# ldyken53/gaussian-splatting-wgpu

Measured on AMD Instinct MI355X. Metric: frames/sec, higher is better.
Workload: dtype f32; 1 GPU; bicycle-like synthetic 6.1M gaussians @1920x1080; gaussians=6100000, width=1920, height=1080, tile_size=16, parallelism=single GPU, visible=2430918, processed=15909895, block_evaluated=6068168, sort_passes=1, depth_ordered_emission=True, tight_binning=True, blend_mode=fused, camera=64-step orbit, moved every frame

## Files before the change

### gaussian-splatting-wgpu_amd/csrc/gs_context.hip

```cpp
#include <atomic>
#include <cmath>
#include <cstdarg>
#include <memory>
#include <new>

#include "gs_runtime.h"

thread_local char g_err[512] = "";
int32_t fail(int32_t code, const char* fmt, ...) {
    va_list ap;
    va_start(ap, fmt);
    vsnprintf(g_err, sizeof(g_err), fmt, ap);
    va_end(ap);
    return code;
}

static uint32_t tiles_f32(uint32_t extent, uint32_t ts) {
    return (uint32_t)std::ceil((float)extent / (float)ts);
}
static uint32_t bits_for(uint64_t v) {
    uint32_t b = 0;
    while (v) { ++b; v >>= 1; }
    return b ? b : 1;
}

GS_EXPORT const char* gs_last_error(void) { return g_err; }
GS_EXPORT int32_t gs_abi_version(void) { return GS_ABI_VERSION; }

int32_t alloc_kv(gs_ctx* c, uint64_t capacity, uint64_t row_cap) {
    if (capacity >= (1ull << 30)) return fail(GS_ERR_CAPACITY, "capacity %llu exceeds 2^30 intersections", (unsigned long long)capacity);
    if (row_cap >= (1ull << 31)) return fail(GS_ERR_CAPACITY, "%llu row items exceed the 2^31 limit", (unsigned long long)row_cap);
    c->gr.valid = false;
    c->keysA.reset(); c->valsA.reset(); c->keysB.reset(); c->valsB.reset(); c->keysU.reset(); c->valsU.reset();
    c->keysG.reset(); c->chunk_table.reset(); c->arena.reset(); c->rows_sorted.reset(); c->M3.reset(); c->ctl_mem.reset();
    c->valsG.reset();
    c->keysG_valid = c->valsG_valid = c->gdataG_valid = false;
    capacity = std::max<uint64_t>(capacity, 4096);
    row_cap = (std::max<uint64_t>(row_cap, 4096) + 15) & ~(uint64_t)15;
    const size_t kb = (size_t)capacity * 4;
    HIP_TRY(hipMalloc(c->keysA.out(), kb));
    HIP_TRY(hipMalloc(c->valsA.out(), kb));
    HIP_TRY(hipMalloc(c->keysB.out(), kb));
    HIP_TRY(hipMalloc(c->valsB.out(), kb));
    c->sort_index = GsSort{{c->keysA, c->valsA}, {c->keysB, c->valsB}, c->passes, 8, 0, false, false};
    c->sort_tile = GsSort{{c->keysA, c->valsA}, {c->keysB, c->valsB}, c->tile_passes, c->tile_bits, c->tile16 ? 0u : 1u, c->tile16, true};
    HIP_TRY(hipMalloc(c->chunk_table.out(), (size_t)gs_emit_chunks(std::max(capacity, row_cap)) * 4));
    if (c->tight_ok) {
        HIP_TRY(hipMalloc(c->arena.out(), (size_t)row_cap * 12));
        HIP_TRY(hipMalloc(c->rows_sorted.out(), (size_t)row_cap * 12));
        HIP_TRY(hipMalloc(c->M3.out(), (size_t)gs_rows_chunks(row_cap) * 256 * 4));
    }
    const size_t ctl_sz = (sizeof(GsControl) + 255) & ~(size_t)255;
    const size_t scan_sz = (((size_t)gs_scan_blocks(c->n ? c->n : 1) + 1) * 8 + 255) & ~(size_t)255;
    const size_t sort_sz = (size_t)std::max(c->passes, c->tile_passes) * gs_sort_tiles(capacity) * 256 * 4;
    const size_t rows_sz = c->tight_ok ? (size_t)gs_rows_sort_tiles(row_cap) * 256 * 4 : 0;
    const size_t depth_sz = ((size_t)c->T * 4 + 255) & ~(size_t)255;
    c->ctl_bytes = ctl_sz + depth_sz + rows_sz + scan_sz + sort_sz;
    c->ctl_bytes_tight = ctl_sz + depth_sz + rows_sz;
    HIP_TRY(hipMalloc(c->ctl_mem.out(), c->ctl_bytes));
    char* const base = (char*)c->ctl_mem.get();
    c->ctl = (GsControl*)base;
    c->tile_depth = (uint32_t*)(base + ctl_sz);
    c->rows_status = (uint32_t*)(base + ctl_sz + depth_sz);
    c->scan_status = (unsigned long long*)(base + ctl_sz + depth_sz + rows_sz);
    c->sort_status = (uint32_t*)(base + ctl_sz + depth_sz + rows_sz + scan_sz);
    c->capacity = capacity;
    c->row_cap = row_cap;
    c->frame.capacity = (uint32_t)capacity;
    c->frame.row_cap = (uint32_t)row_cap;
    return GS_OK;
}

GS_EXPORT int32_t gs_create(const gs_config* cfg, gs_ctx** out) {
    if (!cfg || !out) return fail(GS_ERR_INVALID_ARGUMENT, "gs_create: null argument");
    if (cfg->struct_size != sizeof(gs_config)) return fail(GS_ERR_INVALID_ARGUMENT, "gs_create: struct_size %u != %zu", cfg->struct_size, sizeof(gs_config));
    if (cfg->width == 0 || cfg->height == 0) return fail(GS_ERR_INVALID_ARGUMENT, "gs_create: empty canvas");
    if (cfg->tile_size != 8 && cfg->tile_size != 16 && cfg->tile_size != 32)
        return fail(GS_ERR_INVALID_ARGUMENT, "gs_create: tile_size must be 8, 16 or 32 (got %u)", cfg->tile_size);
    int ndev = 0;
    if (hipGetDeviceCount(&ndev) != hipSuccess || ndev == 0) return fail(GS_ERR_NO_DEVICE, "gs_create: no HIP device");
    if (cfg->device < 0 || cfg->device >= ndev) return fail(GS_ERR_INVALID_ARGUMENT, "gs_create: device %d of %d", cfg->device, ndev);
    HIP_TRY(hipSetDevice(cfg->device));

    std::unique_ptr<gs_ctx> c(new (std::nothrow) gs_ctx());
    if (!c) return fail(GS_ERR_OUT_OF_MEMORY, "gs_create: host allocation failed");
    c->cfg = *cfg;
    GsFrame& f = c->frame;
    f.width = cfg->width; f.height = cfg->height; f.tile_size = cfg->tile_size;
    f.ntx = tiles_f32(cfg->width, cfg->tile_size);
    f.nty = tiles_f32(cfg->height, cfg->tile_size);
    if (f.ntx >= 32768 || f.nty >= 65536) return fail(GS_ERR_INVALID_ARGUMENT, "gs_create: canvas too large");
    f.col0 = cfg->col_begin;
    f.col1 = cfg->col_end;
    if (f.col0 == 0 && f.col1 == 0) f.col1 = f.ntx;
    if (f.col1 > f.ntx || f.col0 >= f.col1) return fail(GS_ERR_INVALID_ARGUMENT, "gs_create: bad tile-column slab [%u,%u) of %u", f.col0, f.col1, f.ntx);
    f.full = (f.col0 == 0 && f.col1 == f.ntx) ? 1u : 0u;
    f.px0 = f.col0 * f.tile_size;
    f.slab_w = std::min(f.width, f.col1 * f.tile_size) - f.px0;
    c->T = f.ntx * f.nty;
    const uint64_t max_key = ((uint64_t)f.nty * f.ntx + f.ntx) * 1000ull + 999ull;
    if (max_key > 0xFFFFFFFFull) return fail(GS_ERR_INVALID_ARGUMENT, "gs_create: tile ids overflow the 32-bit key (write_tile_ids.wgsl:29)");
    c->key_bits = bits_for(max_key);
    c->passes = (c->key_bits + 7) / 8;
    const uint32_t tbits = bits_for((uint64_t)f.nty * f.ntx + f.ntx);
    c->tile_passes = (tbits + 7) / 8;
    c->tile_bits = (tbits + c->tile_passes - 1) / c->tile_passes;
    c->tile16 = ((uint64_t)f.nty * f.ntx + f.ntx) < 0xFFFFull;
    if ((uint64_t)(f.ntx + 1) * (f.nty + 1) > GS_COUNT_MASK) return fail(GS_ERR_INVALID_ARGUMENT, "gs_create: canvas has too many tiles");
    c->tight_ok = f.ntx <= 255u && f.nty <= 255u;

    hipDeviceProp_t prop;
    HIP_TRY(hipGetDeviceProperties(&prop, cfg->device));
    c->opt.grid_persist = (uint32_t)prop.multiProcessorCount * 4;
    if (cfg->stream) c->stream = (hipStream_t)cfg->stream;
    else { HIP_TRY(hipStreamCreateWithFlags(c->own_stream.out(), hipStreamNonBlocking)); c->stream = c->own_stream; }

    HIP_TRY(hipMalloc(c->ranges.out(), (size_t)c->T * 4));
    HIP_TRY(hipMemset(c->ranges, 0, (size_t)c->T * 4));
    const size_t px = (size_t)f.slab_w * f.height;
    HIP_TRY(hipMalloc(c->rgba8.out(), px * 4));
    HIP_TRY(hipMemset(c->rgba8, 0, px * 4));
    if (cfg->flags & GS_FLAG_F32_TAP) HIP_TRY(hipMalloc(c->rgbf.out(), px * 12));
    if (cfg->flags & GS_FLAG_AUX_OUTPUTS) {
        HIP_TRY(hipMalloc(c->alpha.out(), px * 4));
        HIP_TRY(hipMalloc(c->depth.out(), px * 4));
        HIP_TRY(hipMemset(c->alpha, 0, px * 4));
        HIP_TRY(hipMemset(c->depth, 0, px * 4));
    }
    HIP_TRY(hipHostMalloc(c->h_ctl.out(), sizeof(GsControl), hipHostMallocDefault));
    memset(c->h_ctl, 0, sizeof(GsControl));
    HIP_TRY(hipMalloc(c->d_pxb.out(), 65 * 4));
    HIP_TRY(hipMalloc(c->tileoff.out(), 256 * 256 * 4));
    HIP_TRY(hipMalloc(c->rowtot.out(), 256 * 4));
    HIP_TRY(hipMalloc(c->sticky.out(), 4 * 4));
    HIP_TRY(hipMemset(c->sticky, 0, 4 * 4));
    HIP_TRY(hipHostMalloc(c->h_rep.out(), sizeof(GsReport), hipHostMallocDefault));
    memset(c->h_rep, 0, sizeof(GsReport));
    if (cfg->flags & GS_FLAG_TIMING) {
        for (auto& row : c->ev)
            for (auto& e : row) HIP_TRY(hipEventCreate(e.out()));
        c->have_events = true;
    }
    c->fif = (c->own_stream && f.full) ? 3u : 1u;
    *out = c.release();
    return GS_OK;
}

gs_ctx::~gs_ctx() { drop_graph(this); }

GS_EXPORT int32_t gs_destroy(gs_ctx* c) {
    if (!c) return GS_OK;
    hipSetDevice(c->cfg.device);
    drop_shadows(c);
    if (c->stream) hipStreamSynchronize(c->stream);
    delete c;
    return GS_OK;
}

static int32_t alloc_per_gaussian(gs_ctx* c, uint64_t n, uint64_t min_capacity = 0, uint64_t min_rows = 0) {
    c->gr.valid = false;
    c->scene_own.reset();
    c->scene_mem = nullptr;
    c->n = (uint32_t)n;
    c->frame.n = (uint32_t)n;
    c->have_frame = false;
    c->cov.reset();
    c->ng = gs_ctx::Neigh{};
    c->cl = gs_ctx::Cluster{};
    c->counts.reset(); c->offsets.reset(); c->grec.reset(); c->rowptr.reset(); c->gsort_scratch.reset(); c->gdata.reset(); c->gdataG.reset();
    c->unit_off.reset(); c->unit_n.reset();
    const size_t np = ((size_t)n + 63) & ~(size_t)63;
    const size_t ne = (size_t)gs_gsort_tiles((uint32_t)(n ? n : 1)) * 2048, nu = ne / 1024 + 2;
    HIP_TRY(hipMalloc(c->counts.out(), ne * 4));
    HIP_TRY(hipMalloc(c->offsets.out(), std::max<size_t>(np * 4, 256)));
    HIP_TRY(hipMalloc(c->grec.out(), std::max<size_t>(np * 16, 256)));
    HIP_TRY(hipMalloc(c->rowptr.out(), ne * 4));
    HIP_TRY(hipMalloc(c->unit_off.out(), ne * 2));
    HIP_TRY(hipMalloc(c->unit_n.out(), nu * 4));
    HIP_TRY(hipMemsetAsync(c->unit_n, 0, nu * 4, c->stream));
    HIP_TRY(hipMalloc(c->gsort_scratch.out(), gs_gsort_scratch_bytes((uint32_t)n)));
    HIP_TRY(hipMalloc(c->gdata.out(), ((size_t)n + GS_RECORD_SLACK) * 64));
    HIP_TRY(hipMemsetAsync(c->gdata, 0, ((size_t)n + GS_RECORD_SLACK) * 64, c->stream));
    uint64_t cap = c->cfg.max_intersections ? c->cfg.max_intersections : std::max<uint64_t>(4 * n, 1u << 22);
    cap = std::max<uint64_t>(cap, min_capacity);
    cap = std::min<uint64_t>(cap, (1ull << 30) - 1);
    const uint64_t rows = std::max<uint64_t>(std::max<uint64_t>(2 * n, 1u << 20), min_rows);
    return alloc_kv(c, cap, rows);
}

GsSceneLayout scene_layout(void* base, uint64_t n, bool state) {
    GsSceneLayout L;
    const size_t np = ((size_t)n + 63) & ~(size_t)63;
    const size_t sh_end = np * 4 * 4 + np * 32 + (size_t)n * 192, state_at = (sh_end + 255) & ~(size_t)255;
    L.np = np;
    L.state_at = state_at;
    L.bytes = state ? state_at + np : sh_end;
    char* p = (char*)base;
    GsScene& s = L.scene;
    s.px = (float*)p; p += np * 4; s.py = (float*)p; p += np * 4; s.pz = (float*)p; p += np * 4;
    s.smax = (float*)p; p += np * 4;
    s.geo = (float4*)p; p += np * 32;
    s.sh = (float4*)p;
    s.state = state ? (const uint8_t*)base + state_at : nullptr;
    return L;
}
static void scene_views(gs_ctx* c, uint64_t n) {
    const GsSceneLayout L = scene_layout(c->scene_own.get(), n, has_state(c));
    c->scene_mem = c->scene_own;
    c->scene_bytes = L.bytes;
    c->scene = L.scene;
}

uint64_t scene_new_serial() {
    static std::atomic<uint64_t> next{1};
    return next.fetch_add(1, std::memory_order_relaxed);
}
int32_t scene_alloc(gs_ctx* c, uint64_t n, uint64_t min_capacity, uint64_t min_rows) {
    c->scene_serial = scene_new_serial();
    int32_t rc = alloc_per_gaussian(c, n, min_capacity, min_rows);
    if (rc != GS_OK) return rc;
    const GsSceneLayout L = scene_layout(nullptr, n, has_state(c));
    HIP_TRY(hipMalloc(c->scene_own.out(), std::max<size_t>(L.bytes, 256)));
    scene_views(c, n);
    if (has_state(c))
        HIP_TRY(hipMemsetAsync((char*)c->scene_mem + L.state_at, 0, std::max<size_t>(L.np, 4), c->stream));
    return GS_OK;
}

int32_t scene_install(gs_ctx* c, DevBuf<>&& mem, uint64_t n, uint64_t min_capacity, uint64_t min_rows) {
    const int32_t rc = alloc_per_gaussian(c, n, min_capacity, min_rows);
    if (rc != GS_OK) {
        c->scene = GsScene{};
        c->n = c->frame.n = 0;
        return rc;
    }
    c->scene_own = std::move(mem);
    scene_views(c, n);
    return GS_OK;
}

static int32_t upload_common(gs_ctx* c, const void* d_aos, uint64_t n) {
    int32_t rc = scene_alloc(c, n);
    if (rc != GS_OK) return rc;
    if (n) gs_launch_repack(d_aos, (uint32_t)n, 0, c->scene, c->stream);
    HIP_TRY(hipGetLastError());
    HIP_TRY(hipStreamSynchronize(c->stream));
    return GS_OK;
}

void drop_shadows(gs_ctx* c) {
    for (gs_ctx* s : c->shadows) gs_destroy(s);
    c->shadows.clear();
    c->last = c;
    c->rr = 0;
    c->cap_hint = 0;
    c->row_hint = 0;
}
GS_EXPORT int32_t gs_share_splats(gs_ctx* c, gs_ctx* owner) {
    if (!c || !owner || c == owner) return fail(GS_ERR_INVALID_ARGUMENT, "gs_share_splats: needs two distinct contexts");
    if (c->cfg.device != owner->cfg.device) return fail(GS_ERR_INVALID_ARGUMENT, "gs_share_splats: contexts are on different devices");
    if (!c->is_shadow) drop_shadows(c);
    if (!owner->scene_mem) return fail(GS_ERR_NO_SCENE, "gs_share_splats: the owner holds no splats");
    if (has_state(c) && !has_state(owner))
        return fail(GS_ERR_INVALID_ARGUMENT, "gs_share_splats: this context has GS_FLAG_SPLAT_STATE, the owner keeps no state plane");
    HIP_TRY(hipSetDevice(c->cfg.device));
    if (c->pending) { int32_t rc = wait_one(c); if (rc != GS_OK) return rc; }
    int32_t rc = alloc_per_gaussian(c, owner->n, c->cfg.max_intersections ? 0 : owner->capacity, owner->row_cap);
    if (rc != GS_OK) return rc;
    c->scene_mem = owner->scene_mem;
    c->scene_bytes = owner->scene_bytes;
    c->scene = owner->scene;
    c->scene_serial = scene_new_serial();
    HIP_TRY(hipStreamSynchronize(c->stream));
    return GS_OK;
}

GS_EXPORT int32_t gs_upload_splats_device(gs_ctx* c, const void* d_aos, uint64_t n) {
    if (!c || (!d_aos && n)) return fail(GS_ERR_INVALID_ARGUMENT, "gs_upload_splats_device: null argument");
    if (n >= (1ull << 31)) return fail(GS_ERR_INVALID_ARGUMENT, "gs_upload_splats: too many gaussians");
    HIP_TRY(hipSetDevice(c->cfg.device));
    drop_shadows(c);
    return upload_common(c, d_aos, n);
}

GS_EXPORT int32_t gs_upload_splats(gs_ctx* c, const void* aos, uint64_t n) {
    if (!c || (!aos && n)) return fail(GS_ERR_INVALID_ARGUMENT, "gs_upload_splats: null argument");
    if (n >= (1ull << 31)) return fail(GS_ERR_INVALID_ARGUMENT, "gs_upload_splats: too many gaussians");
    HIP_TRY(hipSetDevice(c->cfg.device));
    drop_shadows(c);
    DevBuf<> d;
    const size_t bytes = (size_t)n * GS_SPLAT_RECORD_BYTES;
    HIP_TRY(hipMalloc(d.out(), std::max<size_t>(bytes, 256)));
    if (bytes) {
        hipError_t e = hipMemcpy(d, aos, bytes, hipMemcpyHostToDevice);
        if (e != hipSuccess) return fail(GS_ERR_HIP, "upload memcpy: %s", hipGetErrorString(e));
    }
    return upload_common(c, d, n);
}

GS_EXPORT int32_t gs_host_alloc(uint64_t bytes, void** out) {
    if (!out) return fail(GS_ERR_INVALID_ARGUMENT, "gs_host_alloc: null argument");
    *out = nullptr;
    HIP_TRY(hipHostMalloc(out, std::max<size_t>((size_t)bytes, 256), hipHostMallocDefault));
    return GS_OK;
}
GS_EXPORT void gs_host_free(void* p) { if (p) hipHostFree(p); }

GS_EXPORT int32_t gs_slab_width(gs_ctx* c, uint32_t* px_begin, uint32_t* px_width) {
    if (!c) return fail(GS_ERR_INVALID_ARGUMENT, "gs_slab_width: null ctx");
    if (px_begin) *px_begin = c->frame.px0;
    if (px_width) *px_width = c->frame.slab_w;
    return GS_OK;
}

static int32_t set_option_one(gs_ctx* c, int32_t key, int64_t value) {
    c->gr.valid = false;
    GsOptions& o = c->opt;
    switch (key) {
    case GS_OPT_FRAME_GRAPH: o.frame_graph = (value != 0); return GS_OK;
    case GS_OPT_BLEND_ABLATION: o.blend_ablation = (uint32_t)value & 0x3FFFFu; return GS_OK;
    case GS_OPT_PERSISTENT_GRID: if (value <= 0) break; o.grid_persist = (uint32_t)value; return GS_OK;
    case GS_OPT_RESET_TIMING: c->timed_from = c->frames; c->max_I_seen = 0; c->truncated_frames = 0; return GS_OK;
    case GS_OPT_EMIT_ORDER: if (value < 0 || value > 2) break; o.emit_order = (int)value; return GS_OK;
    case GS_OPT_UNFUSED: return GS_OK;
    case GS_OPT_DEBUG_VIEW: if (value < 0 || value > 4) break; o.debug_view = (uint32_t)value; return GS_OK;
    case GS_OPT_TILE_CULL: o.tile_cull = (value != 0); return GS_OK;
    case GS_OPT_PROJ_CHUNKS: if (value != 0 && value != 2 && value != 4 && value != 8) break; o.tight_nb = (uint32_t)value; return GS_OK;
    case GS_OPT_SELECT_TINT:
        if (!has_state(c)) return fail(GS_ERR_INVALID_ARGUMENT, "gs_set_option: GS_OPT_SELECT_TINT needs GS_FLAG_SPLAT_STATE");
        if (value < 0 || value > 0xFFFFFFFFll) break;
        o.select_tint = (uint32_t)value;
        return GS_OK;
    default: break;
    }
    return fail(GS_ERR_INVALID_ARGUMENT, "gs_set_option: bad key/value %d/%lld", key, (long long)value);
}
GS_EXPORT int32_t gs_set_option(gs_ctx* c, int32_t key, int64_t value) {
    if (!c) return fail(GS_ERR_INVALID_ARGUMENT, "gs_set_option: null ctx");
    if (key == GS_OPT_FRAMES_IN_FLIGHT) {
        if (value < 1 || value > 4) return fail(GS_ERR_INVALID_ARGUMENT, "gs_set_option: frames in flight must be 1..4");
        if (!c->own_stream || !c->frame.full) value = 1;
        int32_t rc = gs_wait(c);
        if (rc != GS_OK && rc != GS_ERR_TRUNCATED) return rc;
        while (c->shadows.size() + 1 > (size_t)value) {
            if (c->last == c->shadows.back()) { c->last = c; }
            gs_destroy(c->shadows.back());
            c->shadows.pop_back();
        }
        c->fif = (uint32_t)value;
        c->rr = 0;
        return GS_OK;
    }
    int32_t rc = set_option_one(c, key, value);
    for (gs_ctx* s : c->shadows) if (rc == GS_OK) rc = set_option_one(s, key, value);
    return rc;
}
```

### gaussian-splatting-wgpu_amd/csrc/gs_device.h

```cpp
#pragma once
#include <hip/hip_runtime.h>
#include <stdint.h>

#define GS_WAVE 64

struct GsFrame {
    uint32_t n;
    uint32_t width, height, tile_size;
    uint32_t ntx, nty;
    uint32_t col0, col1;
    uint32_t px0, slab_w;
    uint32_t capacity;
    uint32_t full;
    uint32_t row_cap;
};

#define GS_COUNT_BITS 22
#define GS_COUNT_MASK 0x3FFFFFu

struct GsControl {
    uint32_t scan_ticket[2];
    uint32_t sort_ticket[4];
    uint32_t rows_ticket;
    uint32_t num_slots;
    uint32_t num_items;
    uint32_t fault;
    uint32_t overflow;
    uint32_t num_intersections;
    uint32_t num_visible;
    uint32_t pad0;
    uint32_t row_cursor[16];
    uint32_t rec_cursor[16];
    unsigned long long num_processed[64];
    unsigned long long num_evaluated[64];
    uint32_t hist[4][256];
    uint32_t rowhist[8][256];
};
__device__ __forceinline__ uint32_t gs_rowhist(const GsControl* ctl, uint32_t r) {
    uint32_t s = 0;
#pragma unroll
    for (int k = 0; k < 8; ++k) s += ctl->rowhist[k][r];
    return s;
}

struct GsReport {
    uint32_t fault, overflow, num_intersections, num_visible, num_slots, num_items, pad0, pad1;
    uint32_t row_cursor[16];
    uint32_t sticky[4];
};
__device__ __forceinline__ void gs_frame_report(const GsControl* ctl, uint32_t I, uint32_t num_items, uint32_t capacity, uint32_t* sticky,
                                                GsReport* rep) {
    uint32_t need = 0;
    for (int k = 0; k < 16; ++k) need = ctl->row_cursor[k] > need ? ctl->row_cursor[k] : need;
    need = need > 0x07FFFFFFu ? 0x7FFFFFFFu : need * 16u;
    const uint32_t over = (I > capacity || ctl->overflow) ? 1u : 0u;
    uint32_t s0 = 0, s1 = 0, s2 = 0, s3 = 0;
    if (sticky) {
        s0 = atomicAdd(&sticky[0], over) + over;
        s1 = atomicOr(&sticky[1], ctl->fault ? 1u : 0u) | (ctl->fault ? 1u : 0u);
        s2 = atomicMax(&sticky[2], I); s2 = s2 > I ? s2 : I;
        s3 = atomicMax(&sticky[3], need); s3 = s3 > need ? s3 : need;
    }
    if (rep) {
        rep->fault = ctl->fault; rep->overflow = over; rep->num_intersections = I; rep->num_visible = ctl->num_visible;
        rep->num_slots = ctl->num_slots; rep->num_items = num_items;
        for (int k = 0; k < 16; ++k) rep->row_cursor[k] = ctl->row_cursor[k];
        rep->sticky[0] = s0; rep->sticky[1] = s1; rep->sticky[2] = s2; rep->sticky[3] = s3;
    }
}

struct GsTightOut {
    uint32_t* arena; uint32_t* rowptr; GsControl* ctl;
    unsigned short* unit_off; uint32_t* unit_n;
    uint32_t rec_shard_cap;
};
#define GS_RECORD_SLACK (16u * 512u * 8u)

struct GsScene {
    const float* px; const float* py; const float* pz;
    const float* smax;
    const float4* geo;
    const float4* sh;
    const uint8_t* state;
};

#define GS_ST_HIDDEN 1u
#define GS_ST_SELECTED 2u
struct GsTint { float t[3]; float k; };
__device__ __forceinline__ uint32_t gs_state_apply(uint32_t s, uint32_t op, uint32_t bits) {
    return op == 1u ? (s | bits) : op == 2u ? (s & ~bits) : op == 3u ? (s ^ bits) : bits;
}
struct GsStateQuad { uint32_t w, valid; };
__device__ __forceinline__ GsStateQuad gs_state_quad(const uint8_t* __restrict__ state, uint32_t n, uint32_t q) {
    const uint64_t first = (uint64_t)q * 4u;
    uint32_t w = 0u, valid = 0u;
    if (first + 4u <= n) {
        valid = 4u;
        if (state) w = reinterpret_cast<const uint32_t*>(state)[q];
    } else if (first < n) {
        valid = (uint32_t)(n - first);
        if (state)
            for (uint32_t k = 0; k < valid; ++k) w |= (uint32_t)state[first + k] << (8u * k);
    }
    return GsStateQuad{w, valid};
}

struct GsPlyTable {
    uint32_t stride, nsrc, all_float;
    uint16_t soff[11 + 48];
    uint8_t stype[11 + 48], slot[11 + 48];
};

struct GsUniforms {
    float view[16];
    float proj[16];
    float cam[3];
    float tan_fovx, tan_fovy, focal_x, focal_y, scale_modifier;
};

__device__ __forceinline__ float wg_max(float a, float b) { return (a < b) ? b : a; }
__device__ __forceinline__ float wg_min(float a, float b) { return (b < a) ? b : a; }
__device__ __forceinline__ int wg_maxi(int a, int b) { return (a < b) ? b : a; }
__device__ __forceinline__ int wg_mini(int a, int b) { return (b < a) ? b : a; }

__device__ __forceinline__ int f2i_sat(float x) {
    if (x != x) return 0;
    if (x >= 2147483648.0f) return 2147483647;
    if (x <= -2147483648.0f) return (-2147483647 - 1);
    return (int)x;
}
__device__ __forceinline__ uint32_t f2u_sat(float x) {
    if (x != x) return 0u;
    if (x >= 4294967296.0f) return 0xFFFFFFFFu;
    if (x <= 0.0f) return 0u;
    return (uint32_t)x;
}

__device__ __forceinline__ float gs_exp(float x) {
    if (x != x) return x;
    if (x > 88.72283935546875f) return __builtin_inff();
    if (x < -103.97208404541015625f) return 0.0f;
    const float nf = __builtin_rintf(x * 1.44269502162933349609375f);
    float r = __builtin_fmaf(-nf, 0.693145751953125f, x);
    r = __builtin_fmaf(-nf, 1.42860677465796470642e-06f, r);
    float p = 1.9875691500e-4f;
    p = __builtin_fmaf(p, r, 1.3981999507e-3f);
    p = __builtin_fmaf(p, r, 8.3334519073e-3f);
    p = __builtin_fmaf(p, r, 4.1665795894e-2f);
    p = __builtin_fmaf(p, r, 1.6666665459e-1f);
    p = __builtin_fmaf(p, r, 5.0000001201e-1f);
    const float z = r * r;
    float y = __builtin_fmaf(p, z, r);
    y = y + 1.0f;
    const int n = (int)nf;
    const int a = n >> 1;
    const int b = n - a;
    const float sa = __uint_as_float((uint32_t)(a + 127) << 23);
    const float sb = __uint_as_float((uint32_t)(b + 127) << 23);
    return (y * sa) * sb;
}

__device__ __forceinline__ float gs_blend_power(float cx, float cy, float cz, float dx, float dy) {
    const float t1 = cx * dx * dx, t2 = cz * dy * dy, t3 = cy * dx * dy;
    return -0.5f * (t1 + t2) - t3;
}
__device__ __forceinline__ float gs_blend_alpha(float op, float power) { return wg_min(0.99f, op * gs_exp(power)); }
struct GsPixel { float T, cr, cg, cb, cd; };
template <bool AUX>
__device__ __forceinline__ GsPixel gs_blend_exact(GsPixel p, float4 p1, float4 p2, float dx, float dy) {
    const float power = gs_blend_power(p1.x, p1.y, p1.z, dx, dy);
    const float alpha = gs_blend_alpha(p2.w, power);
    const float test = p.T * (1.0f - alpha);
    const float cond = (power <= 0.0f && alpha >= (float)(1.0 / 255.0) && test >= 0.0001f) ? 1.0f : 0.0f;
    p.cr += cond * p2.x * alpha * p.T;
    p.cg += cond * p2.y * alpha * p.T;
    p.cb += cond * p2.z * alpha * p.T;
    if constexpr (AUX) p.cd += cond * p1.w * alpha * p.T;
    p.T = cond * test + (1.0f - cond) * p.T;
    return p;
}
template <bool EXACT>
__device__ __forceinline__ bool gs_pixel_final(float T) {
    const float c255 = (float)(1.0 / 255.0);
    return (EXACT ? T * (1.0f - c255) : __builtin_fmaf(-T, c255, T)) < 0.0001f;
}

__device__ __forceinline__ float block_qmin(float cx, float cy, float cz, float dxlo, float dxhi, float dylo, float dyhi,
                                            float& mag) {
    const float X = __builtin_fminf(__builtin_fmaxf(0.0f, dxlo), dxhi);
    const float Y = __builtin_fminf(__builtin_fmaxf(0.0f, dylo), dyhi);
    float q = 3.0e38f;
    mag = 0.0f;
    if (X == 0.0f && Y == 0.0f) return 0.0f;
    if (X != 0.0f) {
        const float dy = __builtin_fminf(__builtin_fmaxf(-cy * X * __builtin_amdgcn_rcpf(cz), dylo), dyhi);
        const float a = 0.5f * cx * X * X, b = 0.5f * cz * dy * dy, c = cy * X * dy;
        q = a + b + c;
        mag = __builtin_fabsf(a) + __builtin_fabsf(b) + __builtin_fabsf(c);
    }
    if (Y != 0.0f) {
        const float dx = __builtin_fminf(__builtin_fmaxf(-cy * Y * __builtin_amdgcn_rcpf(cx), dxlo), dxhi);
        const float a = 0.5f * cx * dx * dx, b = 0.5f * cz * Y * Y, c = cy * dx * Y;
        const float q2 = a + b + c;
        if (q2 < q) { q = q2; mag = __builtin_fabsf(a) + __builtin_fabsf(b) + __builtin_fabsf(c); }
    }
    return q;
}

__device__ __forceinline__ bool blend_tmax_cull(float cx, float cy, float cz, float op, float dxlo, float dxhi, float dylo, float dyhi, float Tmax) {
    const float ax0 = (0.5f * cx) * dxlo * dxlo, ax1 = (0.5f * cx) * dxhi * dxhi, by0 = (0.5f * cz) * dylo * dylo, by1 = (0.5f * cz) * dyhi * dyhi;
    const float c00 = cy * dxlo * dylo, c01 = cy * dxlo * dyhi, c10 = cy * dxhi * dylo, c11 = cy * dxhi * dyhi;
    const float qmax = __builtin_fmaxf(__builtin_fmaxf(ax0 + by0 + c00, ax0 + by1 + c01), __builtin_fmaxf(ax1 + by0 + c10, ax1 + by1 + c11));
    const float qmag = __builtin_fmaxf(ax0, ax1) + __builtin_fmaxf(by0, by1) +
                       __builtin_fmaxf(__builtin_fmaxf(__builtin_fabsf(c00), __builtin_fabsf(c01)), __builtin_fmaxf(__builtin_fabsf(c10), __builtin_fabsf(c11)));
    const float alo = 0.99f * __builtin_fminf(0.99f, op * __builtin_amdgcn_exp2f(-1.44269502162933349609375f * (qmax + 1.0e-5f * qmag)));
    return Tmax * (1.0f - alo) < 0.0000999f;
}

struct GsLiveBox { float c0, c1, r0, r1; };
template <bool EMPTY_OK>
__device__ __forceinline__ GsLiveBox gs_live_box(unsigned long long lv) {
    uint32_t lcm = (uint32_t)lv | (uint32_t)(lv >> 32);
    lcm |= lcm >> 16; lcm |= lcm >> 8; lcm &= 0xFFu;
    const unsigned long long lo = EMPTY_OK ? lv | (1ull << 63) : lv, hi = EMPTY_OK ? lv | 1ull : lv;
    return GsLiveBox{(float)__builtin_ctz(lcm | 0x100u), (float)(31 - __builtin_clz(lcm | 1u)), (float)(__builtin_ctzll(lo) >> 3),
                     (float)((63 - __builtin_clzll(hi)) >> 3)};
}

__device__ __forceinline__ uint2 gs_tile_range(const uint32_t* __restrict__ ranges, uint32_t tile, uint32_t capacity) {
    const uint32_t start = tile > 0 ? ranges[tile - 1] : 0u;
    uint32_t end = ranges[tile];
    if (end > capacity) end = capacity;
    return make_uint2(start, end);
}

struct GsListRec {
    float ux, uy, cx, cy, cz, z, op;
    uint32_t id;
    bool live;
};
__device__ __forceinline__ GsListRec gs_list_fetch(const uint4* __restrict__ gdata, const uint32_t* __restrict__ values, uint32_t i, uint32_t end,
                                                   uint32_t id_mask, uint32_t want, uint32_t nrec, uint32_t n) {
    GsListRec r;
    r.ux = r.uy = r.cx = r.cy = r.cz = r.z = r.op = 0.0f;
    r.id = 0u;
    r.live = false;
    if (i < end) {
        const uint32_t v = values[i];
        const uint32_t g = v & id_mask;
        if (g < nrec && (want == 0u || (v & want) != 0u)) {
            const uint4 p0 = gdata[(uint64_t)g * 4 + 0];
            const uint4 p1 = gdata[(uint64_t)g * 4 + 1];
            r.op = __uint_as_float(((const uint32_t*)gdata)[(uint64_t)g * 16 + 11]);
            r.ux = __uint_as_float(p0.x); r.uy = __uint_as_float(p0.y);
            r.cx = __uint_as_float(p1.x); r.cy = __uint_as_float(p1.y); r.cz = __uint_as_float(p1.z); r.z = __uint_as_float(p1.w);
            r.id = p0.z;
            r.live = p0.z < n;
        }
    }
    return r;
}
__device__ __forceinline__ uint32_t gs_bcast(uint32_t v, int l) { return (uint32_t)__builtin_amdgcn_readlane((int)v, l); }
__device__ __forceinline__ float gs_bcast(float v, int l) { return __uint_as_float((uint32_t)__builtin_amdgcn_readlane((int)__float_as_uint(v), l)); }

__device__ __forceinline__ void slab_cols(uint32_t rx0, uint32_t rx1, const GsFrame& f, uint32_t& xa, uint32_t& wmain,
                                          uint32_t& alias) {
    const uint32_t hi = rx1 < f.ntx ? rx1 : f.ntx;
    xa = rx0 > f.col0 ? rx0 : f.col0;
    const uint32_t xb = hi < f.col1 ? hi : f.col1;
    wmain = xb > xa ? xb - xa : 0u;
    alias = (rx1 == f.ntx + 1u && f.col0 == 0u) ? 1u : 0u;
}

__device__ __forceinline__ uint32_t lane_id() { return __builtin_amdgcn_mbcnt_hi(~0u, __builtin_amdgcn_mbcnt_lo(~0u, 0u)); }

#define GS_DPP(v, ctrl, rm) (uint32_t)__builtin_amdgcn_update_dpp(0, (int)(v), (ctrl), (rm), 0xf, false)
__device__ __forceinline__ uint32_t wave_incl_scan(uint32_t v, uint32_t) {
    v += GS_DPP(v, 0x111, 0xf);
    v += GS_DPP(v, 0x112, 0xf);
    v += GS_DPP(v, 0x114, 0xf);
    v += GS_DPP(v, 0x118, 0xf);
    v += GS_DPP(v, 0x142, 0xa);
    v += GS_DPP(v, 0x143, 0xc);
    return v;
}
__device__ __forceinline__ unsigned long long wave_incl_scan64(unsigned long long v, uint32_t lane) {
#pragma unroll
    for (int d = 1; d < 64; d <<= 1) {
        const uint32_t lo = __shfl_up((uint32_t)v, d, 64), hi = __shfl_up((uint32_t)(v >> 32), d, 64);
        if ((int)lane >= d) v += ((unsigned long long)hi << 32) | lo;
    }
    return v;
}
__device__ __forceinline__ uint32_t wave_incl_max(uint32_t v) {
    uint32_t t;
    t = GS_DPP(v, 0x111, 0xf); v = (t > v) ? t : v;
    t = GS_DPP(v, 0x112, 0xf); v = (t > v) ? t : v;
    t = GS_DPP(v, 0x114, 0xf); v = (t > v) ? t : v;
    t = GS_DPP(v, 0x118, 0xf); v = (t > v) ? t : v;
    t = GS_DPP(v, 0x142, 0xa); v = (t > v) ? t : v;
    t = GS_DPP(v, 0x143, 0xc); v = (t > v) ? t : v;
    return v;
}
__device__ __forceinline__ uint32_t wave_sum(uint32_t v) {
    return (uint32_t)__builtin_amdgcn_readlane((int)wave_incl_scan(v, 0u), 63);
}

__device__ __forceinline__ void st_agent(uint32_t* p, uint32_t v) {
    __hip_atomic_store(p, v, __ATOMIC_RELAXED, __HIP_MEMORY_SCOPE_AGENT);
}
__device__ __forceinline__ uint32_t ld_agent(const uint32_t* p) {
    return __hip_atomic_load(p, __ATOMIC_RELAXED, __HIP_MEMORY_SCOPE_AGENT);
}
__device__ __forceinline__ void st_agent64(unsigned long long* p, unsigned long long v) {
    __hip_atomic_store(p, v, __ATOMIC_RELAXED, __HIP_MEMORY_SCOPE_AGENT);
}
__device__ __forceinline__ unsigned long long ld_agent64(const unsigned long long* p) {
    return __hip_atomic_load(p, __ATOMIC_RELAXED, __HIP_MEMORY_SCOPE_AGENT);
}

#define GS_SPIN_LIMIT (1u << 22)
```

### gaussian-splatting-wgpu_amd/csrc/gs_frame.hip

```cpp
#include <dlfcn.h>

#include "gs_runtime.h"
#include "gs_tight.h"

namespace {
struct Roctx {
    int (*push)(const char*) = nullptr;
    int (*pop)() = nullptr;
    Roctx() {
        void* h = dlopen("librocprofiler-sdk-roctx.so.1", RTLD_LAZY | RTLD_LOCAL);
        if (!h) h = dlopen("libroctx64.so.4", RTLD_LAZY | RTLD_LOCAL);
        if (h) {
            push = (int (*)(const char*))dlsym(h, "roctxRangePushA");
            pop = (int (*)())dlsym(h, "roctxRangePop");
            if (!push || !pop) push = nullptr, pop = nullptr;
        }
    }
};
Roctx& roctx() { static Roctx r; return r; }
const char* const kStageRange[] = {"gsplat:process_gaussians", "gsplat:exclusive_scan", "gsplat:write_tile_ids", "gsplat:radix_sort",
                                   "gsplat:compute_ranges", "gsplat:compute_tiles"};
}

static inline void mark(gs_ctx* c, int i) {
    if (!c->have_events) return;
    hipEventRecord(c->ev[c->frames % GS_EV_RING][i], c->stream);
    Roctx& r = roctx();
    if (r.push) {
        if (i > 0) r.pop();
        if (i < GS_STAGE_COUNT) r.push(kStageRange[i]);
    }
}

static void mark_cb(void* p, int i) { mark((gs_ctx*)p, i); }

GsLists frame_lists(const gs_ctx* c) {
    return GsLists{c->gdata, c->notes.valsS, c->ranges, c->frame, c->notes.last_tight ? GS_ID_MASK : 0xFFFFFFFFu,
                   c->notes.last_tight ? c->n + GS_RECORD_SLACK : c->n};
}

static void prepare_projection(gs_ctx* c, const GsUniforms& u, bool tight) {
    gs_preprocess_prepare(c->pre, c->scene, u, c->frame, c->gdata, c->counts, tight, c->arena, c->rowptr, c->unit_off, c->unit_n, c->ctl, c->opt.tight_nb,
                          has_state(c), tint_of(c->opt.select_tint));
}


static FrameNotes bin_tight(gs_ctx* c) {
    hipStream_t st = c->stream;
    gs_launch_gsort(c->counts, c->rowptr, c->unit_off, c->unit_n, c->n, c->gsort_scratch, c->grec, c->chunk_table,
                    (uint32_t)gs_emit_chunks(std::max(c->capacity, c->row_cap)), &c->ctl->num_visible, &c->ctl->num_slots, c->opt.grid_persist, st);
    mark(c, 2);
    gs_launch_rows(c->arena, c->grec, c->chunk_table, c->rows_sorted, c->ctl, c->rows_status, (uint32_t)c->row_cap, c->M3, c->tileoff, c->rowtot, c->frame,
                   c->valsA, c->ranges, c->opt.grid_persist / 4u, c->sticky, c->h_rep, st, mark_cb, c);
    mark(c, 4);
    return FrameNotes{nullptr, c->valsA,  1u,  1u,  false,  false,  true};
}

static FrameNotes sort_to_ranges(gs_ctx* c, const GsSort& plan, bool by_index) {
    hipStream_t st = c->stream;
    mark(c, 3);
    const GsSortPair sorted = gs_launch_sort(plan, c->ctl, c->sort_status, (uint32_t)c->capacity, c->opt.grid_persist, st);
    mark(c, 4);
    const uint32_t grid = c->opt.grid_persist * 2;
    if (plan.keys16) gs_launch_ranges16((const uint16_t*)sorted.keys, c->ctl, (uint32_t)c->capacity, c->T, c->ranges, grid, c->sticky, c->h_rep, st);
    else gs_launch_ranges(sorted.keys, c->ctl, (uint32_t)c->capacity, c->T, c->ranges, grid, c->sticky, c->h_rep, st);
    return FrameNotes{sorted.keys, sorted.vals, plan.passes,  1u, by_index, plan.keys16,  false};
}

static int32_t bin_by_index(gs_ctx* c, bool debug, FrameNotes& nt) {
    hipStream_t st = c->stream;
    gs_launch_scan(c->counts, c->n, c->offsets, c->scan_status, &c->ctl->scan_ticket[0], c->ctl, st);
    mark(c, 2);
    gs_launch_emit(c->gdata, c->counts, c->offsets, c->frame, c->keysA, c->valsA, c->ctl, st);
    if (debug) {
        const size_t kb = (size_t)c->capacity * 4;
        if (!c->keysU) {
            HIP_TRY(hipMalloc(c->keysU.out(), kb));
            HIP_TRY(hipMalloc(c->valsU.out(), kb));
        }
        HIP_TRY(hipMemcpyAsync(c->keysU, c->keysA, kb, hipMemcpyDeviceToDevice, st));
        HIP_TRY(hipMemcpyAsync(c->valsU, c->valsA, kb, hipMemcpyDeviceToDevice, st));
    }
    nt = sort_to_ranges(c, c->sort_index, true);
    return GS_OK;
}

static FrameNotes bin_by_depth(gs_ctx* c) {
    gs_launch_gsort(c->counts, nullptr, nullptr, nullptr, c->n, c->gsort_scratch, c->grec, c->chunk_table, (uint32_t)gs_emit_chunks(std::max(c->capacity, c->row_cap)),
                    &c->ctl->num_visible, &c->ctl->num_intersections, c->opt.grid_persist, c->stream);
    mark(c, 2);
    gs_launch_emit_balanced(c->gdata, c->grec, c->chunk_table, c->frame, c->keysA, c->valsA, c->ctl, c->opt.grid_persist * 2, c->tile_bits, c->tile_passes,
                            c->tile16, c->stream);
    return sort_to_ranges(c, c->sort_tile, false);
}

static int32_t record_frame(gs_ctx* c, const GsUniforms& u, bool debug, void* ext_rgba8, bool tight, bool index_order) {
    hipStream_t st = c->stream;
    const GsOptions& o = c->opt;
    gs_launch_zero(c->ctl_mem, tight ? c->ctl_bytes_tight : c->ctl_bytes, st);
    c->h_ctl_valid = false;
    if (debug) HIP_TRY(hipMemsetAsync(c->gdata, 0, std::max<size_t>((size_t)c->n * 64, 256), st));
    mark(c, 0);
    prepare_projection(c, u, tight);
    gs_launch_preprocess(c->pre, st);
    mark(c, 1);
    FrameNotes& nt = c->notes;
    if (tight) nt = bin_tight(c);
    else if (!debug && !index_order) nt = bin_by_depth(c);
    else if (const int32_t rc = bin_by_index(c, debug, nt); rc != GS_OK) return rc;
    mark(c, 5);
    uint32_t* target = ext_rgba8 ? (uint32_t*)ext_rgba8 : c->rgba8.get();
    const bool prof = (o.blend_ablation & 0x10000u) != 0;
    if (prof && !c->blend_prof) HIP_TRY(hipMalloc(c->blend_prof.out(), (size_t)(1u << 20) * 16));
    const bool aux = (c->cfg.flags & GS_FLAG_AUX_OUTPUTS) != 0;
    const int walkers = gs_launch_blend(frame_lists(c), target, c->rgbf, aux, c->alpha, c->depth, c->ctl, c->tile_depth, (c->cfg.flags & GS_FLAG_EXACT_BLEND) != 0,
                                        o.blend_ablation & 0xFFFFu, st, prof ? c->blend_prof.get() : nullptr, &c->blend_prof_blocks);
    if (walkers == -2) return fail(GS_ERR_INVALID_ARGUMENT, "blend: GS_FLAG_AUX_OUTPUTS without its alpha / depth planes");
    if (walkers < 0) return fail(GS_ERR_INVALID_ARGUMENT, "unsupported tile size %u", c->frame.tile_size);
    nt.blend_walkers = (uint32_t)walkers;
    mark(c, 6);
    if (o.debug_view) gs_launch_debug_view(c->ranges, c->frame, o.debug_view, target, st);
    return GS_OK;
}

void drop_graph(gs_ctx* c) {
    if (c->gr.exec) hipGraphExecDestroy(c->gr.exec);
    if (c->gr.graph) hipGraphDestroy(c->gr.graph);
    c->gr.exec = nullptr; c->gr.graph = nullptr; c->gr.pre_node = nullptr;
    c->gr.valid = false;
}

static int32_t enqueue_frame(gs_ctx* c, const GsUniforms& u, bool debug, void* ext_rgba8) {
    hipStream_t st = c->stream;
    bool index_order = (c->opt.emit_order == 1);
    if (c->opt.emit_order == 2) {
        const uint64_t saved = c->passes > c->tile_passes ? c->passes - c->tile_passes : 0;
        index_order = !(c->have_frame && saved * (uint64_t)c->h_rep->num_intersections >= 1000000ull);
    }
    const bool tight = !debug && c->opt.tile_cull && c->tight_ok && (uint64_t)c->n + GS_RECORD_SLACK <= (1ull << GS_ID_BITS);
    const bool graphable = c->opt.frame_graph && !debug && !c->have_events && !(c->opt.blend_ablation & 0x10000u) && c->n;
    if (graphable) {
        const GraphKey key{index_order, tight, ext_rgba8, c->alpha, c->depth};
        if (!c->gr.exec || !c->gr.valid || !(c->gr.key == key)) {
            if (c->gr.exec) HIP_TRY(hipStreamSynchronize(st));
            drop_graph(c);
            HIP_TRY(hipStreamBeginCapture(st, hipStreamCaptureModeRelaxed));
            const int32_t rc = record_frame(c, u, debug, ext_rgba8, tight, index_order);
            const hipError_t e = hipStreamEndCapture(st, &c->gr.graph);
            if (rc != GS_OK) { drop_graph(c); return rc; }
            if (e != hipSuccess || !c->gr.graph) return fail(GS_ERR_HIP, "frame graph capture: %s", hipGetErrorString(e));
            hipGraph_t g = c->gr.graph;
            HIP_TRY(hipGraphInstantiate(&c->gr.exec, g, nullptr, nullptr, 0));
            size_t nn = 0;
            HIP_TRY(hipGraphGetNodes(g, nullptr, &nn));
            std::vector<hipGraphNode_t> nodes(nn);
            HIP_TRY(hipGraphGetNodes(g, nodes.data(), &nn));
            uint32_t found = 0;
            for (hipGraphNode_t nd : nodes) {
                hipGraphNodeType ty;
                if (hipGraphNodeGetType(nd, &ty) != hipSuccess || ty != hipGraphNodeTypeKernel) continue;
                hipKernelNodeParams kp;
                if (hipGraphKernelNodeGetParams(nd, &kp) == hipSuccess && kp.func == c->pre.func) { c->gr.pre_node = nd; ++found; }
            }
            if (found != 1) {
                c->opt.frame_graph = false;
                c->gr.pre_node = nullptr;
            }
            c->gr.key = key;
            c->gr.notes = c->notes;
            c->gr.valid = true;
        } else {
            c->notes = c->gr.notes;
            prepare_projection(c, u, tight);
            hipKernelNodeParams kp{};
            kp.func = const_cast<void*>(c->pre.func);
            kp.gridDim = dim3(c->pre.blocks); kp.blockDim = dim3(256); kp.sharedMemBytes = 0;
            kp.kernelParams = c->pre.args; kp.extra = nullptr;
            HIP_TRY(hipGraphExecKernelNodeSetParams(c->gr.exec, c->gr.pre_node, &kp));
        }
        HIP_TRY(hipGraphLaunch(c->gr.exec, st));
        c->gr.frames++;
    } else {
        const int32_t rc = record_frame(c, u, debug, ext_rgba8, tight, index_order);
        if (rc != GS_OK) return rc;
    }
    c->keysG_valid = c->valsG_valid = c->gdataG_valid = false;
    c->h_ctl_valid = false;
    HIP_TRY(hipGetLastError());
    c->pending = true;
    c->have_frame = true;
    c->last_debug = debug;
    c->last_ext = ext_rgba8;
    c->last_u = u;
    c->frames++;
    return GS_OK;
}

static int32_t render_common(gs_ctx* c, const void* uniforms, bool debug, void* ext) {
    if (!c || !uniforms) return fail(GS_ERR_INVALID_ARGUMENT, "gs_render: null argument");
    if (!c->scene_mem) return fail(GS_ERR_NO_SCENE, "gs_render: no splats uploaded");
    HIP_TRY(hipSetDevice(c->cfg.device));
    GsUniforms u;
    static_assert(sizeof(GsUniforms) == GS_UNIFORM_BYTES, "uniform block must be 160 bytes");
    memcpy(&u, uniforms, sizeof(u));
    return enqueue_frame(c, u, debug, ext);
}

int32_t wait_one(gs_ctx* c) {
    if (!c) return fail(GS_ERR_INVALID_ARGUMENT, "gs_wait: null ctx");
    HIP_TRY(hipSetDevice(c->cfg.device));
    uint32_t dropped = 0;
    for (int attempt = 0; attempt < 8; ++attempt) {
        HIP_TRY(hipStreamSynchronize(c->stream));
        c->pending = false;
        if (!c->have_frame) return GS_OK;
        const uint32_t over_frames = c->h_rep->sticky[0], fault_any = c->h_rep->sticky[1];
        const uint64_t max_I = c->h_rep->sticky[2], max_rows = c->h_rep->sticky[3];
        if (over_frames || fault_any || max_I || max_rows) HIP_TRY(hipMemset(c->sticky, 0, 4 * 4));
        c->h_rep->sticky[0] = c->h_rep->sticky[1] = c->h_rep->sticky[2] = c->h_rep->sticky[3] = 0;
        if (max_I > c->max_I_seen) c->max_I_seen = max_I;
        if (fault_any || c->h_rep->fault) return fail(GS_ERR_DEVICE_FAULT, "a look-back spin exceeded its bound (fault word set)");
        const uint64_t I = c->h_rep->num_intersections;
        uint64_t rows_last = 0;
        if (c->notes.last_tight)
            for (int k = 0; k < 16; ++k) rows_last = std::max<uint64_t>(rows_last, (uint64_t)c->h_rep->row_cursor[k] * 16);
        const bool last_over = I > c->capacity || c->h_rep->overflow;
        if (attempt == 0 && over_frames > (last_over ? 1u : 0u)) dropped = over_frames - (last_over ? 1u : 0u);
        const uint64_t need = std::max<uint64_t>(I, max_I), need_rows = std::max<uint64_t>(rows_last, max_rows);
        if (!last_over && need <= c->capacity && need_rows <= c->row_cap) break;
        if (need >= (1ull << 30)) return fail(GS_ERR_CAPACITY, "%llu intersections exceed the 2^30 limit", (unsigned long long)need);
        uint64_t want = c->capacity, want_rows = c->row_cap;
        if (need > c->capacity) want = std::min<uint64_t>(std::max<uint64_t>(need + need / 4, c->capacity * 2), (1ull << 30) - 1);
        if (need_rows > c->row_cap) want_rows = std::max<uint64_t>(need_rows + need_rows / 4, c->row_cap * 2);
        if (want == c->capacity && want_rows == c->row_cap) {
            if (last_over) return fail(GS_ERR_CAPACITY, "the frame reports an overflow that growing cannot fix (capacity %llu, rows %llu)",
                                       (unsigned long long)c->capacity, (unsigned long long)c->row_cap);
            break;
        }
        int32_t rc = alloc_kv(c, want, want_rows);
        if (rc != GS_OK) return rc;
        if (!last_over) break;
        if (attempt == 7) return fail(GS_ERR_CAPACITY, "capacity did not converge");
        c->frames--;
        rc = enqueue_frame(c, c->last_u, c->last_debug, c->last_ext);
        if (rc != GS_OK) return rc;
    }
    if (dropped) {
        c->truncated_frames += dropped;
        return fail(GS_ERR_TRUNCATED, "%u frame(s) enqueued before the last one overflowed the (key,value) capacity and were rendered from "
                    "truncated lists; the capacity has been grown to %llu -- wait after every frame, or pass gs_config.max_intersections",
                    dropped, (unsigned long long)c->capacity);
    }
    return GS_OK;
}

GS_EXPORT int32_t gs_wait(gs_ctx* c) {
    if (!c) return fail(GS_ERR_INVALID_ARGUMENT, "gs_wait: null ctx");
    int32_t first = wait_one(c);
    char msg[sizeof(g_err)];
    if (first != GS_OK) memcpy(msg, g_err, sizeof(msg));
    for (gs_ctx* s : c->shadows) {
        const int32_t rc = wait_one(s);
        if (rc != GS_OK && first == GS_OK) { first = rc; memcpy(msg, g_err, sizeof(msg)); }
    }
    c->cap_hint = std::max(c->cap_hint, over_ring(c, [](const gs_ctx* m) { return m->capacity; }, true));
    c->row_hint = std::max(c->row_hint, over_ring(c, [](const gs_ctx* m) { return m->row_cap; }, true));
    if (first != GS_OK) memcpy(g_err, msg, sizeof(msg));
    return first;
}

static int32_t add_shadow(gs_ctx* c) {
    gs_config cfg = c->cfg;
    cfg.stream = nullptr;
    cfg.max_intersections = 0;
    gs_ctx* s = nullptr;
    int32_t rc = gs_create(&cfg, &s);
    if (rc != GS_OK) return rc;
    s->fif = 1;
    s->is_shadow = true;
    rc = gs_share_splats(s, c);
    if (rc != GS_OK) { gs_destroy(s); return rc; }
    s->opt = c->opt;
    c->shadows.push_back(s);
    return GS_OK;
}

GS_EXPORT int32_t gs_render(gs_ctx* c, const void* uniforms) {
    if (!c || !uniforms) return fail(GS_ERR_INVALID_ARGUMENT, "gs_render: null argument");
    gs_ctx* t = c;
    if (c->fif > 1 && c->scene_mem) {
        if (c->pending && c->shadows.size() + 1 < c->fif) {
            int32_t rc = add_shadow(c);
            if (rc != GS_OK) return rc;
            c->rr = (uint32_t)c->shadows.size();
        }
        if (!c->shadows.empty()) {
            const uint32_t slot = c->rr++ % (uint32_t)(c->shadows.size() + 1);
            t = slot ? c->shadows[slot - 1] : c;
        }
        if (t->capacity < c->cap_hint || t->row_cap < c->row_hint) {
            HIP_TRY(hipSetDevice(t->cfg.device));
            if (t->pending) { int32_t rc = wait_one(t); if (rc != GS_OK && rc != GS_ERR_TRUNCATED) return rc; }
            int32_t rc = alloc_kv(t, std::max(t->capacity, c->cap_hint), std::max(t->row_cap, c->row_hint));
            if (rc != GS_OK) return rc;
            t->have_frame = false;
        }
    }
    const int32_t rc = render_common(t, uniforms, false, nullptr);
    if (rc == GS_OK) c->last = t;
    return rc;
}
GS_EXPORT int32_t gs_render_debug(gs_ctx* c, const void* uniforms) {
    const int32_t rc = render_common(c, uniforms, true, nullptr);
    if (rc == GS_OK && c) c->last = c;
    return rc;
}
GS_EXPORT int32_t gs_render_to(gs_ctx* c, const void* uniforms, void* d_rgba8) {
    if (!d_rgba8) return fail(GS_ERR_INVALID_ARGUMENT, "gs_render_to: null output");
    const int32_t rc = render_common(c, uniforms, false, d_rgba8);
    if (rc == GS_OK && c) c->last = c;
    return rc;
}

GS_EXPORT int32_t gs_render_host(gs_ctx* c, const void* uniforms, void* host_dst, uint64_t size, uint64_t* ticket) {
    if (!c || !uniforms || !host_dst || !ticket) return fail(GS_ERR_INVALID_ARGUMENT, "gs_render_host: null argument");
    const uint64_t bytes = (uint64_t)c->frame.slab_w * c->frame.height * 4;
    if (size < bytes) return fail(GS_ERR_INVALID_ARGUMENT, "gs_render_host: need %llu bytes, got %llu", (unsigned long long)bytes, (unsigned long long)size);
    int32_t rc = gs_render(c, uniforms);
    if (rc != GS_OK) return rc;
    gs_ctx* t = last_of(c);
    if (!t->ev_done) HIP_TRY(hipEventCreateWithFlags(t->ev_done.out(), hipEventDisableTiming));
    HIP_TRY(hipMemcpyAsync(host_dst, t->rgba8, bytes, hipMemcpyDeviceToHost, t->stream));
    std::lock_guard<std::mutex> lk(c->ticket_mu);
    HIP_TRY(hipEventRecord(t->ev_done, t->stream));
    const uint64_t k = c->next_ticket++;
    c->tickets[k & 63u].ticket = k;
    c->tickets[k & 63u].member = t;
    *ticket = k;
    return GS_OK;
}

GS_EXPORT int32_t gs_wait_ticket(gs_ctx* c, uint64_t ticket) {
    if (!c) return fail(GS_ERR_INVALID_ARGUMENT, "gs_wait_ticket: null ctx");
    gs_ctx* t = nullptr;
    {
        std::lock_guard<std::mutex> lk(c->ticket_mu);
        if (ticket == 0 || ticket >= c->next_ticket) return fail(GS_ERR_INVALID_ARGUMENT, "gs_wait_ticket: unknown ticket %llu", (unsigned long long)ticket);
        if (c->next_ticket - ticket > 64 || c->tickets[ticket & 63u].ticket != ticket) return GS_OK;
        t = c->tickets[ticket & 63u].member;
    }
    HIP_TRY(hipSetDevice(c->cfg.device));
    HIP_TRY(hipEventSynchronize(t->ev_done));
    return GS_OK;
}
```

### gaussian-splatting-wgpu_amd/csrc/gs_kernels.h

```cpp
#pragma once
#include "gs_device.h"

void gs_launch_repack(const void* d_aos, uint32_t n, uint32_t first, const GsScene& s, hipStream_t st);
void gs_launch_ply_chunk(const void* d_raw, uint32_t m, uint32_t first, const GsPlyTable& t, const GsScene& s, hipStream_t st);
struct GsPreprocessLaunch {
    const void* func;
    uint32_t blocks;
    GsScene s; GsUniforms u; GsFrame f;
    void* gdata; uint32_t* counts; GsTightOut to; GsTint tint;
    float w2;
    void* args[8];
};
float gs_view_norm2(const GsUniforms& u);
void gs_preprocess_prepare(GsPreprocessLaunch& L, const GsScene& s, const GsUniforms& u, const GsFrame& f, void* gdata, uint32_t* counts,
                           bool tight, uint32_t* arena, uint32_t* rowptr, unsigned short* unit_off, uint32_t* unit_n, GsControl* ctl,
                           uint32_t tight_nb = 0, bool state = false, GsTint tint = GsTint{});
void gs_launch_preprocess(GsPreprocessLaunch& L, hipStream_t st);
void gs_launch_zero(void* p, uint64_t bytes, hipStream_t st);
uint32_t gs_scan_blocks(uint32_t n);
void gs_launch_scan(const uint32_t* counts, uint32_t n, uint32_t* offsets, unsigned long long* status, uint32_t* ticket, GsControl* ctl,
                    hipStream_t st);
uint64_t gs_emit_chunks(uint64_t capacity);
void gs_launch_emit_balanced(const void* gdata, const void* grec, const uint32_t* chunk_table, const GsFrame& f, uint32_t* keys, uint32_t* values,
                             GsControl* ctl, uint32_t grid, uint32_t hist_bits, uint32_t hist_passes, bool keys16, hipStream_t st);
void gs_launch_emit(const void* gdata, const uint32_t* counts, const uint32_t* offsets, const GsFrame& f, uint32_t* keys, uint32_t* values,
                    GsControl* ctl, hipStream_t st);
void gs_launch_ranges16(const uint16_t* tiles, const GsControl* ctl, uint32_t capacity, uint32_t T, uint32_t* ranges, uint32_t grid,
                        uint32_t* sticky, GsReport* rep, hipStream_t st);
void gs_launch_rebuild_keys(const uint16_t* tiles, const uint32_t* vals, const uint32_t* counts, uint32_t count, uint32_t n, uint32_t* keys,
                            hipStream_t st);
void gs_launch_ranges(const uint32_t* keys, const GsControl* ctl, uint32_t capacity, uint32_t T, uint32_t* ranges, uint32_t grid,
                      uint32_t* sticky, GsReport* rep, hipStream_t st);
uint32_t gs_sort_tiles(uint64_t capacity);
struct GsSortPair { uint32_t *keys, *vals; };
struct GsSort {
    GsSortPair in, alt;
    uint32_t passes, bits, by_tile;
    bool keys16, have_hist;
};
GsSortPair gs_launch_sort(const GsSort& s, GsControl* ctl, uint32_t* status, uint32_t capacity, uint32_t grid, hipStream_t st);
struct GsLists {
    const void* gdata;
    const uint32_t* values;
    const uint32_t* ranges;
    GsFrame f;
    uint32_t id_mask;
    uint32_t nrec;
};
int gs_launch_blend(const GsLists& L, uint32_t* rgba8, float* rgbf, bool aux, float* alpha, float* depth, GsControl* ctl, uint32_t* tile_depth,
                    bool exact, uint32_t ablation, hipStream_t st, uint32_t* prof = nullptr, uint32_t* prof_blocks = nullptr);
void gs_launch_debug_view(const uint32_t* ranges, const GsFrame& f, uint32_t view, uint32_t* rgba8, hipStream_t st);
void gs_launch_assemble(const void* slabs, void* image, uint32_t width, uint32_t height, const uint32_t* d_px_bounds, uint32_t n_slabs,
                        uint64_t slab_stride_px, hipStream_t st);
uint32_t gs_gsort_tiles(uint32_t n);
uint64_t gs_gsort_scratch_bytes(uint32_t n);
void gs_launch_gsort(const uint32_t* words, const uint32_t* aux_in, const unsigned short* unit_off, const uint32_t* unit_n, uint32_t n, void* scratch,
                     void* grec, uint32_t* chunk_table, uint32_t chunk_cap, uint32_t* tot_visible, uint32_t* tot_quantity, uint32_t grid, hipStream_t st);
uint32_t gs_rows_sort_tiles(uint64_t row_cap);
uint32_t gs_rows_chunks(uint64_t row_cap);
void gs_launch_rows(const uint32_t* arena, const void* grec, const uint32_t* chunk_table, uint32_t* rows_sorted, GsControl* ctl, uint32_t* sort_status, uint32_t row_cap,
                    uint32_t* M3, uint32_t* tileoff, uint32_t* rowtot, const GsFrame& f, uint32_t* values, uint32_t* ranges, uint32_t cus,
                    uint32_t* sticky, GsReport* rep, hipStream_t st, void (*mark)(void*, int), void* mark_arg);
void gs_launch_rows_rebuild_keys(const uint32_t* ranges, uint32_t T, const uint32_t* vals, const void* gdata, uint32_t nrec, uint32_t count, uint32_t n,
                                 uint32_t* keys, hipStream_t st);
void gs_launch_rows_rebuild_taps(const uint32_t* vals, const void* gdata, uint32_t nrec, uint32_t count, uint32_t n, uint32_t* ids_out, void* gdata_out,
                                 hipStream_t st);
struct GsRegionDev {
    float a[3], b[3];
    float x0, y0, x1, y1;
    float W, H;
    uint32_t wi, hi;
    float proj[16];
    float viewz[4];
    const uint8_t* mask;
};
#define GS_STATE_SLOTS 32
#define GS_STATE_SLOT_STRIDE 32
void gs_launch_state_region(uint32_t kind, uint8_t* state, const GsScene& s, uint32_t n, const GsRegionDev& r, uint32_t op, uint32_t bits,
                            uint32_t where_mask, uint32_t where_value, unsigned long long* matched, hipStream_t st);
void gs_launch_state_ids(uint8_t* state, const uint32_t* ids, uint64_t n, uint32_t op, uint32_t bits, hipStream_t st);
void gs_launch_state_count(const uint8_t* state, uint32_t n, uint32_t mask, uint32_t value, unsigned long long* count, hipStream_t st);
void gs_launch_state_coverage(uint8_t* state, const void* planes, uint32_t n, uint32_t min_hits, float min_weight, uint32_t covered, uint32_t op,
                              uint32_t bits, uint32_t where_mask, uint32_t where_value, unsigned long long* matched, hipStream_t st);
struct GsAttrDev { float p[4]; };
void gs_launch_attr_state(uint32_t kind, uint8_t* state, const GsScene& s, const void* cov, uint32_t n, const GsAttrDev& a, float lo, float hi,
                          uint32_t inside, uint32_t op, uint32_t bits, uint32_t where_mask, uint32_t where_value, unsigned long long* matched,
                          hipStream_t st);
struct GsAttrSlot { unsigned long long matched, nan; uint32_t kmin, kmax; };
void gs_launch_attr_summary(uint32_t kind, const uint8_t* state, const GsScene& s, const void* cov, uint32_t n, const GsAttrDev& a, uint32_t mask,
                            uint32_t value, unsigned long long* slots, hipStream_t st);
void gs_launch_attr_histogram(uint32_t kind, const uint8_t* state, const GsScene& s, const void* cov, uint32_t n, const GsAttrDev& a, uint32_t mask,
                              uint32_t value, float lo, float hi, float scale, uint32_t bins, unsigned long long* counts, uint32_t grid, hipStream_t st);
void gs_launch_attr_values(uint32_t kind, const GsScene& s, const void* cov, uint32_t n, const GsAttrDev& a, const uint32_t* ids, uint32_t first,
                           uint32_t m, float* out, hipStream_t st);
struct GsNeighGrid { float lo[3]; float inv_h; uint32_t g[3]; uint32_t bx, bxy, shift, blocks, none; };
void gs_launch_neigh_bounds(const uint8_t* state, const GsScene& s, uint32_t n, uint32_t smask, uint32_t svalue, uint32_t qmask, uint32_t qvalue,
                            uint32_t* out, hipStream_t st);
void gs_launch_neigh_keys(const uint8_t* state, const GsScene& s, uint32_t n, uint32_t mask, uint32_t value, const GsNeighGrid& g, uint32_t* keys,
                          uint32_t* vals, hipStream_t st);
void gs_launch_neigh_records(const uint32_t* keys, const uint32_t* vals, uint32_t n, const GsNeighGrid& g, const GsScene& s, void* rec, uint32_t* skeys,
                             void* table, hipStream_t st);
void gs_launch_neigh_cands(const void* qrec, uint32_t nq, const void* srec, const uint32_t* skeys, const void* table, uint32_t nrec, const GsNeighGrid& g,
                           unsigned long long* sums, hipStream_t st);
void gs_launch_neigh_query(const void* qrec, uint32_t nq, uint32_t first_block, uint32_t blocks, const void* srec, const uint32_t* skeys, const void* table,
                           uint32_t nrec, const GsNeighGrid& g, float r2, uint32_t limit, uint32_t n, uint32_t* plane, hipStream_t st);
void gs_launch_state_neigh(uint8_t* state, const uint32_t* plane, uint32_t n, uint32_t min_count, uint32_t max_count, uint32_t inside, uint32_t op,
                           uint32_t bits, uint32_t where_mask, uint32_t where_value, unsigned long long* matched, hipStream_t st);
void gs_launch_cluster_init(const uint8_t* state, const GsScene& s, uint32_t n, uint32_t mask, uint32_t value, uint32_t* parent, uint32_t* count,
                            hipStream_t st);
void gs_launch_cluster_edges(const void* rec, uint32_t nrec, uint32_t first_block, uint32_t blocks, const uint32_t* skeys, const void* table,
                             const GsNeighGrid& g, float r2, uint32_t n, uint32_t* parent, uint32_t* changed, hipStream_t st);
void gs_launch_cluster_flatten(const void* rec, uint32_t nrec, uint32_t n, uint32_t* parent, hipStream_t st);
void gs_launch_cluster_sizes(const void* rec, uint32_t nrec, uint32_t n, const uint32_t* parent, uint32_t* count, bool fold, hipStream_t st);
void gs_launch_cluster_commit(const uint32_t* parent, const uint32_t* count, uint32_t n, uint32_t* labels, uint32_t* sizes, unsigned long long* slots,
                              hipStream_t st);
void gs_launch_cluster_seeds(const uint8_t* state, const uint32_t* labels, uint32_t n, uint32_t mask, uint32_t value, uint32_t* flag, hipStream_t st);
void gs_launch_state_cluster_linked(uint8_t* state, const uint32_t* labels, uint32_t n, const uint32_t* flag, uint32_t op, uint32_t bits, uint32_t where_mask,
                                    uint32_t where_value, unsigned long long* matched, hipStream_t st);
uint32_t gs_select_blocks(uint32_t n);
void gs_launch_select_count(const uint8_t* state, uint32_t n, uint32_t mask, uint32_t value, uint32_t* counts, hipStream_t st);
void gs_launch_select_scatter(const uint8_t* state, uint32_t n, uint32_t mask, uint32_t value, const uint32_t* offsets, uint32_t* ids, uint32_t cap,
                              hipStream_t st);
void gs_launch_unpack(const GsScene& s, uint32_t n, const uint32_t* ids, uint32_t first, uint32_t m, void* d_aos, uint32_t* out_ids, hipStream_t st);
void gs_launch_compact_planes(const GsScene& o, uint32_t n_old, const uint32_t* ids, uint32_t m, const GsScene& d, hipStream_t st, uint32_t first = 0,
                              bool with_state = true);
void gs_launch_grow(const GsScene& o, uint32_t n_old, const GsScene& d, uint32_t n_new, uint32_t new_state, uint32_t grid, hipStream_t st);
struct GsSnapshotDev {
    const uint32_t* ids;
    float *x, *y, *z;
    float4 *geo, *sh;
    uint32_t* state;
};
void gs_launch_snapshot(uint32_t mode, const GsScene& sc, uint32_t n, const GsSnapshotDev& s, uint32_t m, uint32_t parts, hipStream_t st);
void gs_launch_write(const void* d_aos, const uint8_t* d_states, uint32_t m, const uint32_t* ids, const GsScene& s, uint32_t n, uint32_t parts,
                     hipStream_t st);
void gs_launch_ids_ascending(const uint32_t* ids, uint64_t m, uint32_t n, unsigned long long* first_bad, hipStream_t st);
struct gs_xform;
void gs_launch_xform(const GsScene& s, uint32_t n, const uint32_t* ids, uint32_t m, const gs_xform& x, hipStream_t st);
struct gs_grade;
void gs_launch_grade(const GsScene& s, uint32_t n, const uint32_t* ids, uint32_t m, const gs_grade& x, hipStream_t st);
void gs_launch_pick(const GsLists& L, const void* d_queries, uint32_t n, void* d_results, uint32_t max_contrib, void* d_contrib, hipStream_t st);
struct GsCoverDev {
    uint32_t x0, y0, x1, y1;
    const uint8_t* mask;
};
void gs_launch_coverage(const GsLists& L, uint32_t bx0, uint32_t by0, uint32_t nbx, uint32_t nby, const GsCoverDev& r, void* planes, hipStream_t st);
```

### gaussian-splatting-wgpu_amd/csrc/gs_runtime.h

```cpp
#pragma once
#include <hip/hip_runtime.h>

#include <algorithm>
#include <cstdint>
#include <cstdio>
#include <cstring>
#include <mutex>
#include <vector>

#include "../../include/gsplat/gs_abi.h"
#include "gs_kernels.h"

#define GS_EXPORT extern "C" __attribute__((visibility("default")))

extern thread_local char g_err[512];
int32_t fail(int32_t code, const char* fmt, ...) __attribute__((format(printf, 2, 3)));
#define HIP_TRY(expr)                                                                                       \
    do {                                                                                                    \
        hipError_t e_ = (expr);                                                                             \
        if (e_ != hipSuccess)                                                                               \
            return fail(e_ == hipErrorOutOfMemory ? GS_ERR_OUT_OF_MEMORY : GS_ERR_HIP, "%s: %s", #expr,      \
                        hipGetErrorString(e_));                                                             \
    } while (0)

template <class P, auto Destroy>
struct Owned {
    P p = nullptr;
    Owned() = default;
    explicit Owned(P q) : p(q) {}
    Owned(const Owned&) = delete;
    Owned& operator=(const Owned&) = delete;
    Owned(Owned&& o) noexcept : p(o.p) { o.p = nullptr; }
    Owned& operator=(Owned&& o) noexcept { if (this != &o) { reset(); p = o.p; o.p = nullptr; } return *this; }
    ~Owned() { reset(); }
    void reset() { if (p) { (void)Destroy(p); p = nullptr; } }
    P* out() { reset(); return &p; }
    P get() const { return p; }
    operator P() const { return p; }
    P operator->() const { return p; }
};
template <class T = void> using DevBuf = Owned<T*, hipFree>;
template <class T = void> using PinnedBuf = Owned<T*, hipHostFree>;
template <class T>
struct Scratch : DevBuf<T> {
    uint64_t cap = 0;
    int32_t reserve(uint64_t count) {
        if (count <= cap) return GS_OK;
        cap = 0;
        HIP_TRY(hipMalloc(this->out(), (size_t)count * sizeof(T)));
        cap = count;
        return GS_OK;
    }
};
using Event = Owned<hipEvent_t, hipEventDestroy>;
using Stream = Owned<hipStream_t, hipStreamDestroy>;
using File = Owned<FILE*, fclose>;

struct FrameNotes {
    uint32_t *keysS = nullptr, *valsS = nullptr;
    uint32_t last_passes = 0;
    uint32_t blend_walkers = 1;
    bool last_by_index = true;
    bool last_keys16 = false;
    bool last_tight = false;
};

struct GraphKey {
    bool index = false, tight = false;
    void* ext = nullptr;
    float *alpha = nullptr, *depth = nullptr;
    bool operator==(const GraphKey& o) const { return index == o.index && tight == o.tight && ext == o.ext && alpha == o.alpha && depth == o.depth; }
};

struct GsOptions {
    int emit_order = 2;
    uint32_t debug_view = 0;
    bool tile_cull = true;
    uint32_t tight_nb = 0;
    uint32_t blend_ablation = 0;
    uint32_t select_tint = 0x80FFFF00u;
    uint32_t grid_persist = 0;
    bool frame_graph = false;
};

#define GS_EV_RING 256
struct gs_ctx {
    ~gs_ctx();
    gs_config cfg{};
    Stream own_stream;
    hipStream_t stream = nullptr;
    GsFrame frame{};
    uint32_t T = 0, passes = 0, key_bits = 0;
    uint32_t tile_passes = 0, tile_bits = 0;
    bool tile16 = false;
    bool tight_ok = false;
    GsOptions opt;
    DevBuf<uint32_t> blend_prof;
    uint32_t blend_prof_blocks = 0;
    uint32_t fif = 1;
    std::vector<gs_ctx*> shadows;
    bool is_shadow = false;
    gs_ctx* last = nullptr;
    uint32_t rr = 0;
    uint64_t cap_hint = 0, row_hint = 0;
    Event ev_done;
    uint64_t next_ticket = 1;
    struct { uint64_t ticket; gs_ctx* member; } tickets[64] = {};
    std::mutex ticket_mu;
    DevBuf<> scene_own;
    void* scene_mem = nullptr;
    size_t scene_bytes = 0;
    GsScene scene{};
    uint32_t n = 0;
    uint64_t scene_serial = 0;
    DevBuf<uint32_t> counts, offsets, rowptr;
    DevBuf<unsigned short> unit_off;
    DevBuf<uint32_t> unit_n;
    DevBuf<> gdata;
    DevBuf<> grec;
    DevBuf<> gsort_scratch;
    uint64_t capacity = 0;
    DevBuf<uint32_t> keysA, valsA, keysB, valsB;
    GsSort sort_index{}, sort_tile{};
    DevBuf<uint32_t> keysU, valsU;
    DevBuf<uint32_t> keysG;
    bool keysG_valid = false;
    DevBuf<uint32_t> valsG;
    DevBuf<> gdataG;
    bool valsG_valid = false, gdataG_valid = false;
    DevBuf<uint32_t> chunk_table;
    uint64_t row_cap = 0;
    DevBuf<uint32_t> arena, rows_sorted, M3;
    DevBuf<uint32_t> tileoff, rowtot;
    DevBuf<> ctl_mem;
    size_t ctl_bytes = 0;
    size_t ctl_bytes_tight = 0;
    GsControl* ctl = nullptr;
    uint32_t* tile_depth = nullptr;
    uint32_t* rows_status = nullptr;
    unsigned long long* scan_status = nullptr;
    uint32_t* sort_status = nullptr;
    PinnedBuf<GsControl> h_ctl;
    bool h_ctl_valid = false;
    PinnedBuf<GsReport> h_rep;
    DevBuf<uint32_t> sticky;
    uint64_t max_I_seen = 0;
    uint64_t truncated_frames = 0;
    DevBuf<uint32_t> ranges, rgba8;
    DevBuf<float> rgbf;
    DevBuf<float> alpha, depth;
    DevBuf<uint32_t> d_pxb;
    uint32_t pxb_host[65] = {};
    uint32_t pxb_n = 0;
    struct { DevBuf<> q, r; Scratch<uint8_t> c; } pick;
    struct { DevBuf<unsigned long long> counter; Scratch<uint32_t> ids; Scratch<uint8_t> mask; } st;
    struct { Scratch<uint32_t> counts, ids; } ex;
    struct { DevBuf<unsigned long long> slots; Scratch<unsigned long long> hist; Scratch<float> vals; } at;
    DevBuf<> cov;
    struct Neigh {
        DevBuf<uint32_t> plane;
        Scratch<uint32_t> keysA, valsA, keysB, valsB, skeys, bounds;
        Scratch<uint8_t> ctl, src, qry, table;
        Scratch<unsigned long long> sums;
        uint32_t n32 = 0;
    } ng;
    struct Cluster { DevBuf<uint32_t> label, size; } cl;
    Event ev[GS_EV_RING][GS_STAGE_COUNT + 1];
    bool have_events = false;
    uint64_t timed_from = 0;
    struct {
        bool valid = false;
        hipGraph_t graph = nullptr;
        hipGraphExec_t exec = nullptr;
        hipGraphNode_t pre_node = nullptr;
        GraphKey key;
        FrameNotes notes;
        uint64_t frames = 0;
    } gr;
    GsPreprocessLaunch pre{};
    FrameNotes notes;
    bool have_frame = false, pending = false, last_debug = false;
    void* last_ext = nullptr;
    GsUniforms last_u{};
    uint64_t frames = 0;
};

int32_t alloc_kv(gs_ctx* c, uint64_t capacity, uint64_t row_cap);
int32_t scene_alloc(gs_ctx* c, uint64_t n, uint64_t min_capacity = 0, uint64_t min_rows = 0);
struct GsSceneLayout {
    GsScene scene{};
    size_t np = 0, state_at = 0, bytes = 0;
};
GsSceneLayout scene_layout(void* base, uint64_t n, bool state);
int32_t scene_install(gs_ctx* c, DevBuf<>&& mem, uint64_t n, uint64_t min_capacity, uint64_t min_rows);
uint64_t scene_new_serial();
void drop_shadows(gs_ctx* c);
void drop_graph(gs_ctx* c);
int32_t wait_one(gs_ctx* c);
GsLists frame_lists(const gs_ctx* c);
template <class Get>
uint64_t over_ring(const gs_ctx* root, Get get, bool maximum = false) {
    uint64_t v = get(root);
    for (const gs_ctx* s : root->shadows) v = maximum ? std::max<uint64_t>(v, get(s)) : v + get(s);
    return v;
}
enum class Plane {
    none,
    filtered,
    always
};
int32_t resident_check(gs_ctx* c, const char* who, Plane need, uint32_t mask = 0, uint32_t value = 0);
int32_t resident_drain(gs_ctx* c, bool counter = false);
inline int32_t resident_begin(gs_ctx* c, const char* who, Plane need, uint32_t mask = 0, uint32_t value = 0) {
    const int32_t rc = resident_check(c, who, need, mask, value);
    return rc != GS_OK ? rc : resident_drain(c);
}
int32_t stage_mask(gs_ctx* root, const uint8_t* mask, hipStream_t st, const uint8_t** dev);
int32_t last_frame(gs_ctx* root, const char* who, gs_ctx** c);
int32_t cover_planes(gs_ctx* root, hipStream_t st);
int32_t neigh_plane(gs_ctx* c, hipStream_t st);
size_t plane_bytes(const gs_ctx* c);
struct NeighBuilt {
    GsNeighGrid g{};
    const uint8_t* state = nullptr;
    uint64_t sources = 0, queried = 0;
    uint32_t nsrc = 0, nqry = 0;
    bool grid = false;
    float cell_edge = 0.0f;
    const void* qrec = nullptr;
    std::vector<unsigned long long> sums;
    uint64_t candidates = 0;
};
int32_t neigh_check_radius(const char* who, float radius, float* r2);
int32_t neigh_build(gs_ctx* c, const char* who, float radius, uint32_t smask, uint32_t svalue, uint32_t qmask, uint32_t qvalue, NeighBuilt* b);
int32_t neigh_budget(const char* who, uint64_t candidates, uint64_t max_candidates, float radius);
template <class Launch>
void neigh_slices(const std::vector<unsigned long long>& sums, Launch launch) {
    const uint32_t nblocks = (uint32_t)sums.size();
    for (uint32_t b0 = 0; b0 < nblocks;) {
        uint64_t sum = sums[b0];
        uint32_t b1 = b0 + 1u;
        while (b1 < nblocks && sum + sums[b1] <= GS_NEIGH_SLICE_CANDIDATES) sum += sums[b1++];
        launch(b0, b1 - b0);
        b0 = b1;
    }
}
int32_t cluster_planes(gs_ctx* c, hipStream_t st);
int32_t edit_select(gs_ctx* c, uint32_t mask, uint32_t value, bool want_ids, uint64_t* total);
static constexpr uint64_t kBounceRecords = 1ull << 20;
struct PlyLayout {
    uint64_t data_off = 0, vertex_count = 0;
    uint32_t stride = 0;
    int degree = 0, nsrc = 0;
    uint32_t soff[11 + 48], stype[11 + 48], slot[11 + 48];
    bool all_float = true;
};
struct PlySource { File fp; PlyLayout L; };
int32_t ply_open(const char* who, const char* path, PlySource* src);
int32_t ply_stream(const char* who, gs_ctx* c, PlySource& src, const GsScene& dst, uint64_t first);
int32_t attr_check(const char* who, const gs_attr* a, GsAttrDev* dev);
inline bool attr_needs_cover(const gs_attr* a) { return a->kind >= GS_ATTR_COVER_HITS; }
inline gs_ctx* last_of(gs_ctx* c) { return (c && c->last) ? c->last : c; }
inline bool has_state(const gs_ctx* c) { return (c->cfg.flags & GS_FLAG_SPLAT_STATE) != 0; }
inline GsTint tint_of(uint32_t argb) {
    return GsTint{{(float)((argb >> 16) & 255u) / 255.0f, (float)((argb >> 8) & 255u) / 255.0f, (float)(argb & 255u) / 255.0f},
                  (float)(argb >> 24) / 255.0f};
}
```

### gaussian-splatting-wgpu_amd/csrc/k_gsort.hip

```cpp
#include "gs_binning.h"

#define GC_ITEMS 8
#define GC_THREADS 256
#define GC (GC_THREADS * GC_ITEMS)
#define GBINS 1024
#ifndef GS_GSORT_RUNS_Q
#define GS_GSORT_RUNS_Q 4
#endif
__device__ __forceinline__ uint64_t m_index(uint32_t b, uint32_t col, uint32_t ncol) { return ((uint64_t)(b >> 3) * ncol + col) * 8u + (b & 7u); }

#define GU (GC / 2)
__device__ __forceinline__ uint2 unit_pair(const uint2* __restrict__ unit_n, uint32_t c) {
    const uint2 v = unit_n[c];
    return make_uint2(v.x < GU ? v.x : GU, v.y < GU ? v.y : GU);
}
template <bool DENSE>
__global__ __launch_bounds__(GC_THREADS) void gs_gsort_hist_kernel(const uint32_t* __restrict__ words, const uint2* __restrict__ unit_n, uint32_t n,
                                                                   uint2* __restrict__ M, uint32_t ncol, uint32_t cpr, uint32_t NT) {
    __shared__ uint32_t s_cnt[GBINS];
    __shared__ unsigned long long s_sum[GBINS];
    const uint32_t run = blockIdx.x, tid = threadIdx.x;
    const uint32_t c0 = run * cpr, c1 = c0 + cpr < NT ? c0 + cpr : NT;
    for (uint32_t b = tid; b < GBINS; b += GC_THREADS) { s_cnt[b] = 0u; s_sum[b] = 0ull; }
    uint32_t wv[GC_ITEMS];
    uint2 un = make_uint2(0u, 0u);
    auto load = [&](uint32_t c, uint32_t (&o)[GC_ITEMS]) {
#pragma unroll
        for (int j = 0; j < GC_ITEMS; ++j) {
            if (DENSE) {
                const uint32_t e = (uint32_t)(j & 3) * GC_THREADS + tid;
                o[j] = (e < (j < 4 ? un.x : un.y)) ? words[c * GC + (uint32_t)(j >> 2) * GU + e] : 0u;
            } else {
                const uint32_t k = c * GC + j * GC_THREADS + tid;
                o[j] = (k < n) ? words[k] : 0u;
            }
        }
    };
    if (DENSE) un = unit_pair(unit_n, c0);
    load(c0, wv);
    if (DENSE) un = c0 + 1u < c1 ? unit_pair(unit_n, c0 + 1u) : make_uint2(0u, 0u);
    __syncthreads();
    for (uint32_t c = c0; c < c1; ++c) {
        uint32_t nx[GC_ITEMS];
        if (c + 1u < c1) load(c + 1u, nx);
        else {
#pragma unroll
            for (int j = 0; j < GC_ITEMS; ++j) nx[j] = 0u;
        }
        if (DENSE) un = c + 2u < c1 ? unit_pair(unit_n, c + 2u) : make_uint2(0u, 0u);
#pragma unroll
        for (int j = 0; j < GC_ITEMS; ++j) {
            const uint32_t w = wv[j];
            if (w & GS_COUNT_MASK) {
                const uint32_t b = w >> GS_COUNT_BITS;
                atomicAdd(&s_cnt[b], 1u);
                atomicAdd(&s_sum[b], (unsigned long long)(w & GS_COUNT_MASK));
            }
        }
#pragma unroll
        for (int j = 0; j < GC_ITEMS; ++j) wv[j] = nx[j];
    }
    __syncthreads();
#pragma unroll
    for (uint32_t i = 0; i < GBINS / GC_THREADS; ++i) {
        const uint32_t b = tid * (GBINS / GC_THREADS) + i;
        M[m_index(b, run, ncol)] = make_uint2(s_cnt[b], sat32(s_sum[b]));
    }
}

#define GR_THREADS 1024
__device__ __forceinline__ void scan_stride8(uint32_t& x, unsigned long long& y, uint32_t lane) {
#pragma unroll
    for (int d = 8; d < 64; d <<= 1) {
        const uint32_t ox = __shfl_up(x, d, 64), lo = __shfl_up((uint32_t)y, d, 64), hi = __shfl_up((uint32_t)(y >> 32), d, 64);
        if ((int)lane >= d) { x += ox; y += ((unsigned long long)hi << 32) | lo; }
    }
}
__global__ __launch_bounds__(GR_THREADS) void gs_gsort_rowscan_kernel(uint2* __restrict__ M, uint32_t ncol, uint2* __restrict__ rowtot) {
    __shared__ uint32_t s_x[GR_THREADS / 64][8];
    __shared__ unsigned long long s_y[GR_THREADS / 64][8];
    const uint32_t nt = ncol, tid = threadIdx.x, lane = tid & 63, w = tid >> 6, cl = tid >> 3, sub = tid & 7u;
    const uint32_t per = (nt + GR_THREADS / 8 - 1u) / (GR_THREADS / 8);
    const uint32_t c0 = cl * per < nt ? cl * per : nt, c1 = (cl + 1u) * per < nt ? (cl + 1u) * per : nt;
    uint2* row = M + (uint64_t)blockIdx.x * ncol * 8u + sub;
    uint32_t ax = 0;
    unsigned long long ay = 0;
    for (uint32_t c = c0; c < c1; c += 8u) {
        uint2 v[8];
#pragma unroll
        for (int k = 0; k < 8; ++k) v[k] = (c + k < c1) ? row[(uint64_t)(c + k) * 8u] : make_uint2(0u, 0u);
#pragma unroll
        for (int k = 0; k < 8; ++k) { ax += v[k].x; ay += v[k].y; }
    }
    uint32_t ix = ax;
    unsigned long long iy = ay;
    scan_stride8(ix, iy, lane);
    if (lane >= 56u) { s_x[w][sub] = ix; s_y[w][sub] = iy; }
    __syncthreads();
    uint32_t rx = ix - ax, tx = 0;
    unsigned long long ry = iy - ay, ty = 0;
#pragma unroll
    for (uint32_t k = 0; k < GR_THREADS / 64; ++k) {
        const uint32_t vx = s_x[k][sub];
        const unsigned long long vy = s_y[k][sub];
        if (k < w) { rx += vx; ry += vy; }
        tx += vx; ty += vy;
    }
    for (uint32_t c = c0; c < c1; c += 8u) {
        uint2 v[8];
#pragma unroll
        for (int k = 0; k < 8; ++k) v[k] = (c + k < c1) ? row[(uint64_t)(c + k) * 8u] : make_uint2(0u, 0u);
#pragma unroll
        for (int k = 0; k < 8; ++k) {
            if (c + k < c1) row[(uint64_t)(c + k) * 8u] = make_uint2(rx, sat32(ry));
            rx += v[k].x; ry += v[k].y;
        }
    }
    if (tid < 8u) rowtot[blockIdx.x * 8u + sub] = make_uint2(tx, sat32(ty));
}

struct alignas(16) GsortShared {
    uint2 base[GBINS];
    unsigned short binstart[GBINS];
    union {
        unsigned short whist[GC_THREADS / 64][GBINS];
        uint32_t P[GC];
        uint4 zero[GC / 4];
    } u;
    unsigned short id[GC];
    uint32_t word[GC], aux[GC];
    GsPair w2[GC_THREADS / 64];
    uint32_t w1[GC_THREADS / 64];
    uint32_t ptot;
};
static_assert(sizeof(unsigned short) * (GC_THREADS / 64) * GBINS == sizeof(uint32_t) * GC, "the ranking counters and the prefix share their storage");
static_assert(sizeof(GsortShared) <= 40 * 1024, "four workgroups per CU");

template <bool DENSE>
__global__ __launch_bounds__(GC_THREADS) void gs_gsort_scatter_kernel(const uint32_t* __restrict__ words, const uint32_t* __restrict__ aux_in,
                                                                      const unsigned short* __restrict__ unit_off, const uint2* __restrict__ unit_n, uint32_t n,
                                                                      const uint2* __restrict__ M, uint32_t ncol, uint32_t cpr, uint32_t NT,
                                                                      const uint2* __restrict__ rowtot, uint4* __restrict__ grec,
                                                                      uint32_t* __restrict__ chunk_table, uint32_t chunk_cap,
                                                                      uint32_t* __restrict__ tot_visible, uint32_t* __restrict__ tot_quantity) {
    __shared__ GsortShared S;
    const uint32_t run_id = blockIdx.x;
    const uint32_t chunk0 = run_id * cpr, chunk1 = chunk0 + cpr < NT ? chunk0 + cpr : NT;
    const uint32_t tid = threadIdx.x, lane = tid & 63, w = tid >> 6;
    const unsigned long long lt_mask = (1ull << lane) - 1ull;
    constexpr uint32_t BPT = GBINS / GC_THREADS;

    uint32_t nwv[GC_ITEMS], nav[GC_ITEMS];
    uint32_t nid[GC_ITEMS];
    uint2 un = make_uint2(0u, 0u);
    uint2 unx = make_uint2(0u, 0u);
#pragma unroll
    for (int j = 0; j < GC_ITEMS; ++j) nwv[j] = nav[j] = nid[j] = 0u;
    const uint32_t whole = n / GC;
    auto load_chunk = [&](uint32_t c) {
        if (DENSE) {
            const uint32_t T = un.x + un.y;
            const uint32_t R = (T + 255u) >> 8;
            const uint32_t p0 = w * (R << 6) + lane;
#pragma unroll
            for (int j = 0; j < GC_ITEMS; ++j) {
                if ((uint32_t)j < R) {
                    const uint32_t p = p0 + j * 64 < T ? p0 + j * 64 : 0u;
                    const uint32_t e = c * GC + (p >= un.x ? GU + (p - un.x) : p);
                    nwv[j] = words[e];
                    nav[j] = aux_in[e];
                    nid[j] = (uint32_t)unit_off[e];
                }
            }
            unx = un;
            return;
        }
        const uint32_t k0 = c * GC + w * (64 * GC_ITEMS) + lane;
        if (c < whole) {
#pragma unroll
            for (int j = 0; j < GC_ITEMS; ++j) nwv[j] = words[k0 + j * 64];
#pragma unroll
            for (int j = 0; j < GC_ITEMS; ++j) nav[j] = aux_in ? aux_in[k0 + j * 64] : 0u;
        } else {
#pragma unroll
            for (int j = 0; j < GC_ITEMS; ++j) {
                const uint32_t k = k0 + j * 64;
                nwv[j] = (k < n) ? words[k] : 0u;
                nav[j] = (aux_in && k < n) ? aux_in[k] : 0u;
            }
        }
    };
    if (DENSE) un = unit_pair(unit_n, chunk0);
    load_chunk(chunk0);
    if (DENSE) un = chunk0 + 1u < chunk1 ? unit_pair(unit_n, chunk0 + 1u) : make_uint2(0u, 0u);
    {
        uint2 t[BPT], mm[BPT];
#pragma unroll
        for (uint32_t i = 0; i < BPT; ++i) { t[i] = rowtot[tid * BPT + i]; mm[i] = M[m_index(tid * BPT + i, run_id, ncol)]; }

        GsPair acc; acc.x = 0u; acc.y = 0ull;
#pragma unroll
        for (uint32_t i = 0; i < BPT; ++i) { acc.x += t[i].x; acc.y += t[i].y; }
        GsPair total;
        GsPair run = block_excl2<GC_THREADS / 64>(acc, tid, S.w2, total);
#pragma unroll
        for (uint32_t i = 0; i < BPT; ++i) {
            S.base[tid * BPT + i] = make_uint2(run.x + mm[i].x, sat32(run.y + mm[i].y));
            run.x += t[i].x; run.y += t[i].y;
        }
        if (run_id == 0 && tid == 0) { *tot_visible = total.x; *tot_quantity = sat32(total.y); }
    }

    for (uint32_t chunk = chunk0; chunk < chunk1; ++chunk) {
        uint32_t wv[GC_ITEMS], av[GC_ITEMS];
#pragma unroll
        for (int j = 0; j < GC_ITEMS; ++j) { wv[j] = nwv[j]; av[j] = nav[j]; }
        uint32_t idv[GC_ITEMS];
#pragma unroll
        for (int j = 0; j < GC_ITEMS; ++j) idv[j] = 0u;
        if (DENSE) {
            const uint32_t T = unx.x + unx.y, R = (T + 255u) >> 8, p0 = w * (R << 6) + lane;
#pragma unroll
            for (int j = 0; j < GC_ITEMS; ++j) {
                const uint32_t p = p0 + j * 64;
                if (!((uint32_t)j < R && p < T)) wv[j] = 0u;
                idv[j] = (p >= unx.x ? GU : 0u) + nid[j];
            }
        }
        if (chunk + 1u < chunk1) load_chunk(chunk + 1u);
        if (DENSE) un = chunk + 2u < chunk1 ? unit_pair(unit_n, chunk + 2u) : make_uint2(0u, 0u);
        {
            S.u.zero[w * (GBINS / 8) + lane] = make_uint4(0u, 0u, 0u, 0u);
            S.u.zero[w * (GBINS / 8) + 64 + lane] = make_uint4(0u, 0u, 0u, 0u);
        }
        uint32_t rank2[GC_ITEMS / 2];
#pragma unroll
        for (int j = 0; j < GC_ITEMS; ++j) {
            if (!(wv[j] & GS_COUNT_MASK)) wv[j] = 0u;
            const unsigned long long vis = __ballot(wv[j] != 0u);
            uint32_t r = 0;
            if (vis) {
                const uint32_t d = wv[j] >> GS_COUNT_BITS;
                uint32_t plo = (uint32_t)vis, phi = (uint32_t)(vis >> 32);
#pragma unroll
                for (int b = 0; b < 10; ++b) {
                    const uint32_t bit = (d >> b) & 1u;
                    const unsigned long long bal = __ballot(bit != 0u);
                    const uint32_t inv = bit - 1u;
                    plo &= (uint32_t)bal ^ inv;
                    phi &= (uint32_t)(bal >> 32) ^ inv;
                }
                r = wave_rank_peers(S.u.whist[w], d, plo, phi, wv[j] != 0u, lt_mask);
            }
            rank2_put(rank2, j, r);
        }
        __syncthreads();
        uint32_t nc;
        {
            uint32_t tot[BPT], acc = 0;
#pragma unroll
            for (uint32_t i = 0; i < BPT; ++i) {
                const uint32_t b = tid * BPT + i;
                uint32_t run = 0;
#pragma unroll
                for (int k = 0; k < GC_THREADS / 64; ++k) { const uint32_t c = S.u.whist[k][b]; S.u.whist[k][b] = (unsigned short)run; run += c; }
                tot[i] = run;
                acc += run;
            }
            uint32_t run = block_excl_u32<GC_THREADS / 64, uint32_t>(acc, tid, S.w1, nc);
#pragma unroll
            for (uint32_t i = 0; i < BPT; ++i) { S.binstart[tid * BPT + i] = (unsigned short)run; run += tot[i]; }
        }
        if (nc == 0) continue;
        __syncthreads();
#pragma unroll
        for (int j = 0; j < GC_ITEMS; ++j) {
            if (wv[j]) {
                const uint32_t d = wv[j] >> GS_COUNT_BITS;
                const uint32_t r = rank2_get(rank2, j);
                const uint32_t pos = (uint32_t)S.binstart[d] + (uint32_t)S.u.whist[w][d] + r;
                S.id[pos] = (unsigned short)(DENSE ? idv[j] : w * (64 * GC_ITEMS) + j * 64 + lane);
                S.word[pos] = wv[j];
                S.aux[pos] = av[j];
            }
        }
        __syncthreads();
        {
            uint32_t c[GC_ITEMS], acc = 0;
#pragma unroll
            for (int j = 0; j < GC_ITEMS; ++j) {
                const uint32_t p = tid * GC_ITEMS + j;
                c[j] = (p < nc) ? (S.word[p] & GS_COUNT_MASK) : 0u;
                acc += c[j];
            }
            unsigned long long total;
            unsigned long long run = block_excl_u32<GC_THREADS / 64, unsigned long long>(acc, tid, S.w1, total);
#pragma unroll
            for (int j = 0; j < GC_ITEMS; ++j) { S.u.P[tid * GC_ITEMS + j] = sat32(run); run += c[j]; }
            if (tid == 0) S.ptot = sat32(total);
        }
        __syncthreads();
#pragma unroll
        for (int j = 0; j < GC_ITEMS; ++j) {
            const uint32_t pos = j * GC_THREADS + tid;
            if (pos >= nc) continue;
            const uint32_t x = S.word[pos];
            const uint32_t b = x >> GS_COUNT_BITS, first = S.binstart[b];
            const uint2 base = S.base[b];
            const uint32_t g = base.x + (pos - first);
            const unsigned long long off64 = (unsigned long long)base.y + (S.u.P[pos] - S.u.P[first]);
            const uint32_t off = sat32(off64);
            grec[g] = make_uint4(chunk * GC + (uint32_t)S.id[pos], x, off, S.aux[pos]);
            const uint32_t cnt = x & GS_COUNT_MASK;
            if (off != 0xFFFFFFFFu) {
                const unsigned long long lastq = (off64 + cnt - 1ull) >> GS_EMIT_CHUNK_SHIFT;
                const uint32_t last = lastq > 0xFFFFFFFFull ? 0xFFFFFFFFu : (uint32_t)lastq;
                for (uint32_t c = (uint32_t)((off64 + (1u << GS_EMIT_CHUNK_SHIFT) - 1ull) >> GS_EMIT_CHUNK_SHIFT); c <= last && c < chunk_cap; ++c) chunk_table[c] = g;
            }
        }
        if (chunk + 1u < chunk1) {
            uint32_t dx[BPT], py[BPT + 1];
            uint32_t s = S.binstart[tid * BPT];
            py[0] = s < GC ? S.u.P[s] : S.ptot;
#pragma unroll
            for (uint32_t i = 0; i < BPT; ++i) {
                const uint32_t b = tid * BPT + i;
                const uint32_t e = (b + 1u < GBINS) ? (uint32_t)S.binstart[b + 1u] : nc;
                dx[i] = e - s;
                py[i + 1] = e < GC ? S.u.P[e] : S.ptot;
                s = e;
            }
            __syncthreads();
#pragma unroll
            for (uint32_t i = 0; i < BPT; ++i) {
                uint2 v = S.base[tid * BPT + i];
                v.x += dx[i];
                v.y = py[i + 1] == 0xFFFFFFFFu ? 0xFFFFFFFFu : sat32((unsigned long long)v.y + (py[i + 1] - py[i]));
                S.base[tid * BPT + i] = v;
            }
        }
    }
}

uint32_t gs_gsort_tiles(uint32_t n) { return (n + GC - 1) / GC; }
uint64_t gs_gsort_scratch_bytes(uint32_t n) { return ((uint64_t)GBINS * gs_gsort_tiles(n ? n : 1) + GBINS) * sizeof(uint2); }
void gs_launch_gsort(const uint32_t* words, const uint32_t* aux_in, const unsigned short* unit_off, const uint32_t* unit_n, uint32_t n, void* scratch,
                     void* grec, uint32_t* chunk_table, uint32_t chunk_cap, uint32_t* tot_visible, uint32_t* tot_quantity, uint32_t grid, hipStream_t st) {
    if (!n) return;
    const uint32_t NT = gs_gsort_tiles(n);
    uint64_t want = (uint64_t)grid * GS_GSORT_RUNS_Q / 4u;
    if (!want) want = 1;
    const uint32_t cpr = (uint32_t)((NT + want - 1) / want);
    const uint32_t G = (NT + cpr - 1) / cpr;
    uint2* M = (uint2*)scratch;
    uint2* rowtot = M + (uint64_t)GBINS * G;
    const uint2* un = (const uint2*)unit_n;
    if (un) hipLaunchKernelGGL(gs_gsort_hist_kernel<true>, dim3(G), dim3(GC_THREADS), 0, st, words, un, n, M, G, cpr, NT);
    else hipLaunchKernelGGL(gs_gsort_hist_kernel<false>, dim3(G), dim3(GC_THREADS), 0, st, words, un, n, M, G, cpr, NT);
    hipLaunchKernelGGL(gs_gsort_rowscan_kernel, dim3(GBINS / 8), dim3(GR_THREADS), 0, st, M, G, rowtot);
    if (un) hipLaunchKernelGGL(gs_gsort_scatter_kernel<true>, dim3(G), dim3(GC_THREADS), 0, st, words, aux_in, unit_off, un, n, (const uint2*)M, G, cpr, NT,
                               (const uint2*)rowtot, (uint4*)grec, chunk_table, chunk_cap, tot_visible, tot_quantity);
    else hipLaunchKernelGGL(gs_gsort_scatter_kernel<false>, dim3(G), dim3(GC_THREADS), 0, st, words, aux_in, unit_off, un, n, (const uint2*)M, G, cpr, NT,
                            (const uint2*)rowtot, (uint4*)grec, chunk_table, chunk_cap, tot_visible, tot_quantity);
}
```

### gaussian-splatting-wgpu_amd/csrc/k_preprocess.hip

```cpp
#include "gs_device.h"
#include "gs_kernels.h"
#include "gs_tight.h"

__global__ __launch_bounds__(256) void gs_repack_kernel(const float4* __restrict__ aos, uint32_t n, uint32_t first, float* px, float* py,
                                                         float* pz, float* smax, float* geo, float* sh) {
    const uint64_t t = (uint64_t)blockIdx.x * 256 + threadIdx.x;
    const uint64_t total = (uint64_t)n * 20;
    if (t >= total) return;
    const uint32_t g = first + (uint32_t)(t / 20), c = (uint32_t)(t % 20);
    const float4 v = aos[t];
    float* r = geo + (uint64_t)g * 8;
    if (c == 0) { px[g] = v.x; py[g] = v.y; pz[g] = v.z; }
    else if (c == 1) { r[0] = v.x; r[1] = v.y; r[2] = v.z; smax[g] = __builtin_fmaxf(v.x, __builtin_fmaxf(v.y, v.z)); }
    else if (c == 2) { r[4] = v.x; r[5] = v.y; r[6] = v.z; r[7] = v.w; }
    else if (c == 3) { r[3] = v.x; }
    else {
        const uint32_t k = c - 4;
        float* q = sh + (uint64_t)g * 48 + 3 * k;
        q[0] = v.x;
        q[1] = v.y;
        q[2] = v.z;
    }
}

__global__ __launch_bounds__(256) void gs_ply_chunk_kernel(const unsigned char* __restrict__ raw, uint32_t m, uint32_t first, GsPlyTable t,
                                                            float* px, float* py, float* pz, float* smax, float* geo, float* sh) {
    const uint64_t id = (uint64_t)blockIdx.x * 256 + threadIdx.x;
    if (id >= (uint64_t)m * t.nsrc) return;
    const uint32_t v = (uint32_t)(id / t.nsrc), k = (uint32_t)(id % t.nsrc);
    const unsigned char* src = raw + (uint64_t)v * t.stride;
    auto rd = [&](uint32_t kk) {
        const unsigned char* q = src + t.soff[kk];
        if (t.stype[kk] == 1u) {
            uint32_t w;
            if (t.all_float) w = *reinterpret_cast<const uint32_t*>(q);
            else w = (uint32_t)q[0] | ((uint32_t)q[1] << 8) | ((uint32_t)q[2] << 16) | ((uint32_t)q[3] << 24);
            return __uint_as_float(w);
        }
        if (t.stype[kk] == 2u) return (float)((double)q[0] / 255.0);
        return 0.0f;
    };
    const uint64_t g = (uint64_t)first + v;
    const uint32_t slot = t.slot[k];
    const float val = rd(k);
    if (slot == 0u) px[g] = val;
    else if (slot == 1u) py[g] = val;
    else if (slot == 2u) pz[g] = val;
    else if (slot >= 4u && slot <= 6u) {
        geo[g * 8 + (slot - 4u)] = val;
        if (slot == 4u) smax[g] = __builtin_fmaxf(val, __builtin_fmaxf(rd(4), rd(5)));
    } else if (slot >= 8u && slot <= 11u) geo[g * 8 + 4u + (slot - 8u)] = val;
    else if (slot == 12u) geo[g * 8 + 3u] = val;
    else {
        const uint32_t kk = (slot - 16u) >> 2, ch = (slot - 16u) & 3u;
        sh[g * 48 + 3u * kk + ch] = val;
    }
}
void gs_launch_ply_chunk(const void* d_raw, uint32_t m, uint32_t first, const GsPlyTable& t, const GsScene& s, hipStream_t st) {
    const uint64_t total = (uint64_t)m * t.nsrc;
    if (!total) return;
    hipLaunchKernelGGL(gs_ply_chunk_kernel, dim3((uint32_t)((total + 255) / 256)), dim3(256), 0, st, (const unsigned char*)d_raw, m, first, t,
                       (float*)s.px, (float*)s.py, (float*)s.pz, (float*)s.smax, (float*)s.geo, (float*)s.sh);
}

struct M3 { float m[3][3]; };
__device__ __forceinline__ M3 m3_mul(const M3& A, const M3& B) {
    M3 o;
#pragma unroll
    for (int c = 0; c < 3; ++c)
#pragma unroll
        for (int r = 0; r < 3; ++r) o.m[c][r] = (A.m[0][r] * B.m[c][0] + A.m[1][r] * B.m[c][1]) + A.m[2][r] * B.m[c][2];
    return o;
}
__device__ __forceinline__ M3 m3_t(const M3& A) {
    M3 o;
#pragma unroll
    for (int c = 0; c < 3; ++c)
#pragma unroll
        for (int r = 0; r < 3; ++r) o.m[c][r] = A.m[r][c];
    return o;
}
__device__ __forceinline__ void m4_mulv(const float* m, float x, float y, float z, float* o) {
#pragma unroll
    for (int r = 0; r < 4; ++r) o[r] = ((m[0 + r] * x + m[4 + r] * y) + m[8 + r] * z) + m[12 + r] * 1.0f;
}

__device__ __forceinline__ float sigmoid_ref(float o) {
    const float ez = gs_exp(o);
    const float cond = (o >= 0.0f) ? 1.0f : 0.0f;
    return (cond * (1.0f / (1.0f + gs_exp(-o)))) + ((1.0f - cond) * (ez / (1.0f + ez)));
}

__device__ __forceinline__ void sh_colour(const float4* __restrict__ sh, float x, float y, float z, const GsUniforms& u, float col[3]) {
    const float dx = x - u.cam[0], dy = y - u.cam[1], dz = z - u.cam[2];
    const float dl = __builtin_sqrtf((dx * dx + dy * dy) + dz * dz);
    const float X = dx / dl, Y = dy / dl, Z = dz / dl;
    const float xx = X * X, yy = Y * Y, zz = Z * Z, xy = X * Y, xz = X * Z, yz = Y * Z;
    float k[16];
    k[4] = 1.0925484305920792f * xy;
    k[5] = -1.0925484305920792f * yz;
    k[6] = 0.31539156525252005f * ((2.f * zz - xx) - yy);
    k[7] = -1.0925484305920792f * xz;
    k[8] = 0.5462742152960396f * (xx - yy);
    k[9] = (-0.5900435899266435f * Y) * (3.f * xx - yy);
    k[10] = (2.890611442640554f * xy) * Z;
    k[11] = (-0.4570457994644658f * Y) * ((4.f * zz - xx) - yy);
    k[12] = (0.3731763325901154f * Z) * ((2.f * zz - 3.f * xx) - 3.f * yy);
    k[13] = (-0.4570457994644658f * X) * ((4.f * zz - xx) - yy);
    k[14] = (1.445305721320277f * Z) * (xx - yy);
    k[15] = (-0.5900435899266435f * X) * (xx - 3.f * yy);
    float shv[48];
#pragma unroll
    for (int p = 0; p < 12; ++p) {
#ifdef PRE_ABLATE_SH
        const float4 vv = make_float4(X, Y, Z, 0.5f);
#else
        const float4 vv = sh[p];
#endif
        shv[4 * p + 0] = vv.x; shv[4 * p + 1] = vv.y; shv[4 * p + 2] = vv.z; shv[4 * p + 3] = vv.w;
    }
#pragma unroll
    for (int c = 0; c < 3; ++c) {
        float res = 0.28209479177387814f * shv[c];
        res = res + 0.4886025119029199f * ((((-Y) * shv[3 + c]) + Z * shv[6 + c]) - X * shv[9 + c]);
#pragma unroll
        for (int j = 4; j < 16; ++j) res = res + k[j] * shv[3 * j + c];
        res = res + 0.5f;
        col[c] = wg_max(res, 0.0f);
    }
}

__device__ __forceinline__ bool in_frustum_slab(const GsUniforms& u, const GsFrame& f, float w2, float x, float y, float z, float smax_log) {
    float ph[4], pv[4];
    m4_mulv(u.proj, x, y, z, ph);
    const float pw = 1.0f / (ph[3] + 0.0000001f);
    const float ndx = ph[0] * pw, ndy = ph[1] * pw;
    m4_mulv(u.view, x, y, z, pv);
    if ((pv[2] <= 0.2f) || (ndx <= -1.1f || ndx >= 1.1f || ndy <= -1.1f || ndy >= 1.1f)) return false;
    if (f.full) return true;
    const float sm = __expf(smax_log) * u.scale_modifier * 1.001f;
    const float limx = 1.3f * u.tan_fovx, limy = 1.3f * u.tan_fovy;
    const float iz = 1.0f / pv[2];
    const float jf2 = ((u.focal_x * iz) * (u.focal_x * iz) * (1.0f + limx * limx) + (u.focal_y * iz) * (u.focal_y * iz) * (1.0f + limy * limy)) * w2;
    const float rb = 3.0f * __builtin_sqrtf(2.0f * jf2 * sm * sm + 0.92f) * 1.001f + 2.0f;
    const float pxs = ((ndx * 0.5f) + 0.5f) * (float)f.width;
    const float ts = (float)f.tile_size;
    const float lo = pxs - rb, hi = pxs + rb;
    const bool reach = (lo < (float)f.col1 * ts) && (f.col0 == 0u || hi >= (float)f.col0 * ts);
    const bool alias = (f.col0 == 0u) && (hi >= (float)f.ntx * ts);
    return (reach || alias) || !(rb == rb);
}

#ifdef GS_PROFILING
__device__ unsigned long long gs_pre_prof[256][16];
extern "C" __attribute__((visibility("default"))) int gs_prof_preprocess(unsigned long long* out8, int reset) {
    static unsigned long long h[256][16];
    if (out8) {
        if (hipMemcpyFromSymbol(h, HIP_SYMBOL(gs_pre_prof), sizeof(h)) != hipSuccess) return -1;
        for (int k = 0; k < 8; ++k) { out8[k] = 0; for (int c = 0; c < 256; ++c) out8[k] += h[c][k]; }
    }
    if (reset) { for (auto& r : h) for (auto& v : r) v = 0; if (hipMemcpyToSymbol(HIP_SYMBOL(gs_pre_prof), h, sizeof(h)) != hipSuccess) return -1; }
    return 0;
}
#define PRE_STAMP(k) do { const uint32_t t_ = (uint32_t)__builtin_amdgcn_readfirstlane((int)(uint32_t)__builtin_amdgcn_s_memtime()); \
                          pacc[k] = (uint32_t)__builtin_amdgcn_readfirstlane((int)(pacc[k] + (t_ - tprev))); tprev = t_; } while (0)
#else
#define PRE_STAMP(k) do { } while (0)
#endif
#define PRE_G 512
#ifndef PRE_WAVES
#define PRE_WAVES 4
#endif
typedef uint32_t gs_row_u32x3 __attribute__((ext_vector_type(3), aligned(4)));


template <bool TIGHT, int NB, bool STATE>
__global__ __launch_bounds__(256, PRE_WAVES) void gs_preprocess_kernel(GsScene s, GsUniforms u, GsFrame f, uint4* __restrict__ gdata,
                                                             uint32_t* __restrict__ tile_counts, GsTightOut to, GsTint tint, float w2) {
    __shared__ uint32_t s_ids[PRE_G * NB];
    constexpr bool KEEP_POS = NB == 2;
    __shared__ float s_pos[3][KEEP_POS ? PRE_G * NB : 1];
    __shared__ uint32_t s_cnt[2][4];
    __shared__ uint32_t s_misc[8];
    __shared__ alignas(16) uint32_t s_rc[TIGHT ? 2 * NB : 1][4];
    __shared__ uint32_t s_ust[TIGHT ? 4 : 1];
    __shared__ float4 s_tA[TIGHT ? 256 : 1], s_tB[TIGHT ? 256 : 1], s_tC[TIGHT ? 256 : 1];
    __shared__ uint32_t s_mark[TIGHT ? 256 : 1], s_tcnt[TIGHT ? 256 : 1], s_tgid[TIGHT ? 256 : 1];
    __shared__ uint32_t s_tw[4];
    __shared__ uint32_t s_rowhist[TIGHT ? 256 : 1];
    const uint32_t tid = threadIdx.x, lane = tid & 63, w = tid >> 6;
    const uint32_t bid = blockIdx.x;
    const uint32_t base = bid * (PRE_G * NB);
    if (TIGHT) s_rowhist[tid] = 0u;
#ifdef GS_PROFILING
    uint32_t pacc[5] = {0, 0, 0, 0, 0};
    uint32_t tprev = (uint32_t)__builtin_amdgcn_readfirstlane((int)(uint32_t)__builtin_amdgcn_s_memtime());
#endif

    uint32_t nvis = 0;
    if (NB > 1) {
        if (!TIGHT) {
            if (tid == 0) s_misc[1] = 0u;
            __syncthreads();
        }
        uint32_t carried = 0;
        constexpr int GRP = 2 * NB < 8 ? 2 * NB : 8;
#pragma unroll 1
        for (int h = 0; h < 2 * NB / GRP; ++h) {
            float X[GRP], Y[GRP], Z[GRP], S[GRP];
            uint32_t B[GRP];
#pragma unroll
            for (int k = 0; k < GRP; ++k) {
                const uint32_t i = base + (uint32_t)(h * GRP + k) * 256u + tid;
                const uint32_t ic = i < f.n ? i : f.n - 1u;
                X[k] = s.px[ic]; Y[k] = s.py[ic]; Z[k] = s.pz[ic];
                S[k] = 0.0f;
                B[k] = STATE ? (uint32_t)s.state[ic] : 0u;
            }
            if (!f.full) {
#pragma unroll
                for (int k = 0; k < GRP; ++k) {
                    const uint32_t i = base + (uint32_t)(h * GRP + k) * 256u + tid;
                    S[k] = s.smax[i < f.n ? i : f.n - 1u];
                }
            }
            __builtin_amdgcn_sched_barrier(0);
            if (TIGHT) {
                uint32_t vm = 0;
#pragma unroll
                for (int k = 0; k < GRP; ++k) {
                    const uint32_t i = base + (uint32_t)(h * GRP + k) * 256u + tid;
                    bool v = false;
                    if (i < f.n) {
                        v = in_frustum_slab(u, f, w2, X[k], Y[k], Z[k], S[k]);
                        if (STATE && (B[k] & GS_ST_HIDDEN)) v = false;
                    }
                    vm |= (v ? 1u : 0u) << k;
                    const uint32_t c = (uint32_t)__popcll(__ballot(v));
                    if (lane == 0) s_rc[h * GRP + k][w] = c;
                }
                __syncthreads();
#pragma unroll
                for (int k = 0; k < GRP; ++k) {
                    const uint4 c = make_uint4(s_rc[h * GRP + k][0], s_rc[h * GRP + k][1], s_rc[h * GRP + k][2], s_rc[h * GRP + k][3]);
                    const bool v = (vm >> k) & 1u;
                    const unsigned long long b = __ballot(v);
                    if (v) {
                        const uint32_t off = (uint32_t)(h * GRP + k) * 256u + tid;
                        const uint32_t slot = carried + (w > 0 ? c.x : 0u) + (w > 1 ? c.y : 0u) + (w > 2 ? c.z : 0u) + (uint32_t)__popcll(b & ((1ull << lane) - 1ull));
                        s_ids[slot] = STATE ? (off | (B[k] << 16)) : off;
                        if (KEEP_POS) { s_pos[0][slot] = X[k]; s_pos[1][slot] = Y[k]; s_pos[2][slot] = Z[k]; }
                    }
                    carried += (c.x + c.y) + (c.z + c.w);
                }
                continue;
            }
#pragma unroll
            for (int k = 0; k < GRP; ++k) {
                const uint32_t off = (uint32_t)(h * GRP + k) * 256u + tid;
                const uint32_t i = base + off;
                bool v = false;
                if (i < f.n) {
                    v = in_frustum_slab(u, f, w2, X[k], Y[k], Z[k], S[k]);
                    if (STATE && (B[k] & GS_ST_HIDDEN)) v = false;
                    if (!v) tile_counts[i] = 0u;
                }
                const unsigned long long b = __ballot(v);
                if (b) {
                    uint32_t at = 0;
                    if (lane == (uint32_t)__builtin_ctzll(b)) at = atomicAdd(&s_misc[1], (uint32_t)__popcll(b));
                    at = (uint32_t)__builtin_amdgcn_readlane((int)at, __builtin_ctzll(b));
                    if (v) {
                        const uint32_t slot = at + (uint32_t)__popcll(b & ((1ull << lane) - 1ull));
                        s_ids[slot] = STATE ? (off | (B[k] << 16)) : off;
                        if (KEEP_POS) { s_pos[0][slot] = X[k]; s_pos[1][slot] = Y[k]; s_pos[2][slot] = Z[k]; }
                    }
                }
            }
        }
        if (TIGHT && tid < NB / 2) {
            uint32_t first = 0, cnt = 0;
#pragma unroll
            for (int r = 0; r < 2 * NB; ++r) {
                const uint4 c = make_uint4(s_rc[r][0], s_rc[r][1], s_rc[r][2], s_rc[r][3]);
                const uint32_t t = (c.x + c.y) + (c.z + c.w);
                if (r < 4 * (int)tid) first += t;
                else if (r < 4 * (int)tid + 4) cnt += t;
            }
            s_ust[tid] = first;
            const uint32_t un = bid * (NB / 2) + tid;
            if (un < ((f.n + 1023u) >> 10)) to.unit_n[un] = cnt;
        }
        __syncthreads();
        nvis = TIGHT ? carried : s_misc[1];
    } else {
        bool vis[2];
        uint32_t sb[2] = {0u, 0u};
        unsigned long long bal[2];
#pragma unroll
        for (int k = 0; k < 2; ++k) {
            const uint32_t i = base + k * 256 + tid;
            vis[k] = false;
            if (i < f.n) {
                vis[k] = in_frustum_slab(u, f, w2, s.px[i], s.py[i], s.pz[i], f.full ? 0.0f : s.smax[i]);
                if (STATE) {
                    sb[k] = (uint32_t)s.state[i];
                    if (sb[k] & GS_ST_HIDDEN) vis[k] = false;
                }
                if (!vis[k]) tile_counts[i] = 0u;
            }
            bal[k] = __ballot(vis[k]);
            if (lane == 0) s_cnt[k][w] = (uint32_t)__popcll(bal[k]);
        }
        __syncthreads();
#pragma unroll
        for (int k = 0; k < 2; ++k) {
            uint32_t before = 0;
#pragma unroll
            for (int ww = 0; ww < 4; ++ww) {
                const uint32_t c = s_cnt[k][ww];
                if (ww < (int)w) before += c;
                nvis += c;
            }
            if (k == 1) before += s_cnt[0][0] + s_cnt[0][1] + s_cnt[0][2] + s_cnt[0][3];
            if (vis[k]) s_ids[before + (uint32_t)__popcll(bal[k] & ((1ull << lane) - 1ull))] = (k * 256 + tid) | (STATE ? sb[k] << 16 : 0u);
        }
        __syncthreads();
    }

    PRE_STAMP(0);
    const uint32_t trips = (nvis + 255u) / 256u;
    const uint32_t ts_ = f.tile_size, sub = ts_ >= 16u ? ts_ / 2u : ts_, ns = ts_ / sub;
    const float inv_ts = 1.0f / (float)ts_, inv_sub = 1.0f / (float)sub;
    const uint32_t shard = bid & 15u, shard_cap = f.row_cap >> 4;
    for (uint32_t v = tid, trip = 0; TIGHT ? trip < trips : v < nvis; v += 256, ++trip) {
        const bool active = v < nvis;
        const uint32_t sid = s_ids[active ? v : nvis - 1u];
        const uint32_t i = base + (STATE ? (sid & 0xFFFFu) : sid);
        const float4* geo = s.geo + (uint64_t)i * 2;
        const float x = KEEP_POS ? s_pos[0][v < nvis ? v : nvis - 1u] : s.px[i], y = KEEP_POS ? s_pos[1][v < nvis ? v : nvis - 1u] : s.py[i],
                    z = KEEP_POS ? s_pos[2][v < nvis ? v : nvis - 1u] : s.pz[i];
        float ph[4], pv[4];
        m4_mulv(u.proj, x, y, z, ph);
        const float pw = 1.0f / (ph[3] + 0.0000001f);
        const float ndx = ph[0] * pw, ndy = ph[1] * pw;
        m4_mulv(u.view, x, y, z, pv);
        const float uvx = (ndx * 0.5f) + 0.5f, uvy = (ndy * 0.5f) + 0.5f;
        const float4 so = geo[0];
        const float4 q = geo[1];
        const float mod = u.scale_modifier;
        const float sc[3] = {gs_exp(so.x) * mod, gs_exp(so.y) * mod, gs_exp(so.z) * mod};
        const float len = __builtin_sqrtf(((q.x * q.x + q.y * q.y) + q.z * q.z) + q.w * q.w);
        const float qr = q.x / len, qx = q.y / len, qy = q.z / len, qz = q.w / len;
        M3 R;
        R.m[0][0] = 1.f - 2.f * (qy * qy + qz * qz); R.m[0][1] = 2.f * (qx * qy - qr * qz); R.m[0][2] = 2.f * (qx * qz + qr * qy);
        R.m[1][0] = 2.f * (qx * qy + qr * qz); R.m[1][1] = 1.f - 2.f * (qx * qx + qz * qz); R.m[1][2] = 2.f * (qy * qz - qr * qx);
        R.m[2][0] = 2.f * (qx * qz - qr * qy); R.m[2][1] = 2.f * (qy * qz + qr * qx); R.m[2][2] = 1.f - 2.f * (qx * qx + qy * qy);
        M3 M;
#pragma unroll
        for (int c = 0; c < 3; ++c)
#pragma unroll
            for (int r = 0; r < 3; ++r) M.m[c][r] = sc[r] * R.m[c][r];
        const M3 Sig = m3_mul(m3_t(M), M);
        float t0 = pv[0], t1 = pv[1];
        const float t2 = pv[2];
        const float limx = 1.3f * u.tan_fovx, limy = 1.3f * u.tan_fovy;
        t0 = wg_min(limx, wg_max(-limx, t0 / t2)) * t2;
        t1 = wg_min(limy, wg_max(-limy, t1 / t2)) * t2;
        M3 J;
        J.m[0][0] = u.focal_x / t2; J.m[0][1] = 0.f; J.m[0][2] = -(u.focal_x * t0) / (t2 * t2);
        J.m[1][0] = 0.f; J.m[1][1] = u.focal_y / t2; J.m[1][2] = -(u.focal_y * t1) / (t2 * t2);
        J.m[2][0] = 0.f; J.m[2][1] = 0.f; J.m[2][2] = 0.f;
        M3 Wm;
#pragma unroll
        for (int c = 0; c < 3; ++c)
#pragma unroll
            for (int r = 0; r < 3; ++r) Wm.m[c][r] = u.view[r * 4 + c];
        const M3 Tm = m3_mul(Wm, J);
        M3 Vrk;
        Vrk.m[0][0] = Sig.m[0][0]; Vrk.m[0][1] = Sig.m[0][1]; Vrk.m[0][2] = Sig.m[0][2];
        Vrk.m[1][0] = Sig.m[0][1]; Vrk.m[1][1] = Sig.m[1][1]; Vrk.m[1][2] = Sig.m[1][2];
        Vrk.m[2][0] = Sig.m[0][2]; Vrk.m[2][1] = Sig.m[1][2]; Vrk.m[2][2] = Sig.m[2][2];
        const M3 cov = m3_mul(m3_mul(m3_t(Tm), m3_t(Vrk)), Tm);
        const float ca = cov.m[0][0] + 0.3f, cb = cov.m[0][1], cc = cov.m[1][1] + 0.3f;
        const float det = ca * cc - cb * cb;
        uint32_t count = 0;
        uint32_t rminx = 0, rminy = 0, rmaxx = 0, rmaxy = 0;
        uint32_t t_xa = 0, t_wmain = 0, t_alias = 0;
        float conx = 0.f, cony = 0.f, conz = 0.f, opacity = 0.f;
        if (det != 0.0f) {
            const float det_inv = 1.0f / det;
            conx = cc * det_inv; cony = (-cb) * det_inv; conz = ca * det_inv;
            const float mid = 0.5f * (ca + cc);
            const float sq = __builtin_sqrtf(wg_max(0.1f, mid * mid - det));
            const float l1 = mid + sq, l2 = mid - sq;
            const float radius = __builtin_ceilf(3.f * __builtin_sqrtf(wg_max(l1, l2)));
            const float pxs = uvx * (float)f.width, pys = uvy * (float)f.height;
            const int ts = (int)f.tile_size, ntx = (int)f.ntx, nty = (int)f.nty;
            rminx = (uint32_t)wg_mini(ntx, wg_maxi(0, f2i_sat(pxs - radius) / ts));
            rminy = (uint32_t)wg_mini(nty, wg_maxi(0, f2i_sat(pys - radius) / ts));
            rmaxx = (uint32_t)(wg_mini(ntx, wg_maxi(0, f2i_sat(pxs + radius) / ts)) + 1);
            rmaxy = (uint32_t)(wg_mini(nty, wg_maxi(0, f2i_sat(pys + radius) / ts)) + 1);
            uint32_t xa, wmain, alias;
            slab_cols(rminx, rmaxx, f, xa, wmain, alias);
            count = f.full ? (rmaxy - rminy) * (rmaxx - rminx)  : (rmaxy - rminy) * (wmain + alias);
            if (TIGHT) { t_xa = xa; t_wmain = wmain; t_alias = alias; }
        }
        uint32_t nslots = 0, rowptr = 0;
        if (TIGHT) {
            uint32_t ra = 0, nrows = 0;
            if (active && count) {
                opacity = sigmoid_ref(so.w);
                const TightG tg = tight_setup(uvx, uvy, conx, cony, conz, opacity, (float)f.width, (float)f.height);
                if (tg.mode == 0u) count = 0u;
                else {
                    uint32_t rb;
                    tight_rows(tg, rminy, rmaxy, f.tile_size, inv_ts, f.nty, t_alias, ra, rb);
                    nrows = rb - ra;
                    nslots = nrows * (1u + t_alias);
                    if (!nslots) count = 0u;
                    s_tA[tid] = make_float4(tg.gx, tg.gy, tg.kc, tg.qa);
                    s_tB[tid] = make_float4(tg.qb, tg.rcx, tg.xmax, tg.dyR);
                    s_tC[tid] = make_float4(tg.eR, __uint_as_float(tg.mode), __uint_as_float(ra | (nrows << 16)),
                                            __uint_as_float(t_xa | (t_wmain << 16) | (t_alias << 31)));
                }
            } else {
                count = 0u;
            }
            s_tcnt[tid] = 0u;
            PRE_STAMP(1);
            const uint32_t rincl = wave_incl_scan(nslots, lane);
            const uint32_t Rw = (uint32_t)__builtin_amdgcn_readlane((int)rincl, 63);
            const uint32_t myrp = rincl - nslots;
            const unsigned long long recb = __ballot(nslots != 0u);
            const uint32_t recrank = (uint32_t)__popcll(recb & ((1ull << lane) - 1ull));
            if (lane == 63) s_tw[w] = rincl | ((uint32_t)__popcll(recb) << 16);
            __syncthreads();
            uint32_t wbase = 0, R = 0, cbase = 0, C = 0;
#pragma unroll
            for (int k = 0; k < 4; ++k) {
                const uint32_t t = s_tw[k];
                if (k < (int)w) { wbase += t & 0xFFFFu; cbase += t >> 16; }
                R += t & 0xFFFFu; C += t >> 16;
            }
            if (tid == 0) {
                uint32_t at = 0, rat = 0, ok = 1u;
                if (R) {
                    at = atomicAdd(&to.ctl->row_cursor[shard], R);
                    rat = atomicAdd(&to.ctl->rec_cursor[shard], C);
                    if (at > shard_cap || R > shard_cap - at) { ok = 0u; to.ctl->overflow = 1u; }
                }
                s_misc[2] = at; s_misc[3] = ok; s_misc[4] = rat;
            }
            __syncthreads();
            const uint32_t abase = shard * shard_cap + s_misc[2] + wbase;
            const bool ok = s_misc[3] != 0u;
            if (nslots) s_tgid[tid] = shard * to.rec_shard_cap + s_misc[4] + cbase + recrank;
            PRE_STAMP(2);
            uint32_t jcarry = 0u;
            for (uint32_t rb0 = 0; rb0 < Rw; rb0 += 64u) {
                s_mark[tid] = 0u;
                __builtin_amdgcn_fence(__ATOMIC_RELEASE, "wavefront");
                if (nslots && myrp >= rb0 && myrp < rb0 + 64u) s_mark[(w << 6) + (myrp - rb0)] = lane + 1u;
                __builtin_amdgcn_fence(__ATOMIC_RELEASE, "wavefront");
                __builtin_amdgcn_fence(__ATOMIC_ACQUIRE, "wavefront");
                uint32_t m = wave_incl_max(s_mark[tid]);
                m = m > jcarry ? m : jcarry;
                jcarry = (uint32_t)__builtin_amdgcn_readlane((int)m, 63);
                const uint32_t ri = rb0 + lane;
                const uint32_t rpj = (uint32_t)__shfl((int)myrp, (int)(m ? m - 1u : 0u), 64);
                if (ri < Rw) {
                    const uint32_t j = (w << 6) + (m - 1u);
                    const float4 a = s_tA[j], b = s_tB[j], c4 = s_tC[j];
                    TightG g;
                    g.gx = a.x; g.gy = a.y; g.kc = a.z; g.qa = a.w; g.qb = b.x; g.rcx = b.y; g.xmax = b.z; g.dyR = b.w;
                    g.eR = c4.x; g.mode = __float_as_uint(c4.y);
                    g.cx = g.cy = g.cz = g.cxz = g.lim2 = g.ymax = 0.0f;
                    const uint32_t rw = __float_as_uint(c4.z), cw = __float_as_uint(c4.w);
                    uint32_t w1, w2;
                    const uint32_t ilen = tight_slot_item(g, ri - rpj, rw & 0xFFFFu, rw >> 16, f.tile_size, inv_ts, sub, inv_sub, ns, f.nty, cw & 0xFFFFu,
                                                          (cw >> 16) & 0x7FFFu, cw >> 31, w1, w2);
                    if (ilen) {
                        atomicAdd(&s_tcnt[j], ilen);
                        atomicAdd(&s_rowhist[w1 & 0xFFu], 1u);
                    }
                    if (ok) {
                        gs_row_u32x3 it;
                        it.x = ilen ? s_tgid[j] : GS_ROW_HOLE; it.y = w1; it.z = w2;
                        *reinterpret_cast<gs_row_u32x3*>(to.arena + (uint64_t)(abase + ri) * 3u) = it;
                    }
                }
            }
            __builtin_amdgcn_fence(__ATOMIC_RELEASE, "wavefront");
            __builtin_amdgcn_fence(__ATOMIC_ACQUIRE, "wavefront");
            if (count) count = ok ? s_tcnt[tid] : 0u;
            rowptr = abase + myrp;
            PRE_STAMP(3);
            if (!active) continue;
        }
        const uint32_t bucket = f2u_sat(wg_min(50.0f * pv[2], 999.0f));
        const uint32_t word = count ? ((TIGHT ? nslots : count) | (bucket << GS_COUNT_BITS)) : 0u;
        if (TIGHT) {
            const uint32_t off = STATE ? (sid & 0xFFFFu) : sid, uk = off >> 10;
            const uint32_t e = ((bid * (NB / 2) + uk) << 10) + (v - (NB == 2 ? 0u : s_ust[uk]));
            tile_counts[e] = word;
            to.rowptr[e] = rowptr;
            to.unit_off[e] = (unsigned short)(off & 1023u);
        } else tile_counts[i] = word;
        if (count == 0) continue;

        float col[3];
        sh_colour(s.sh + (uint64_t)i * 12, x, y, z, u, col);
        if (STATE && ((sid >> 16) & GS_ST_SELECTED) && tint.k != 0.0f) {
#pragma unroll
            for (int c = 0; c < 3; ++c) col[c] = col[c] + tint.k * (tint.t[c] - col[c]);
        }
        if (!TIGHT) opacity = sigmoid_ref(so.w);
        uint4* o4 = gdata + (uint64_t)(TIGHT ? s_tgid[tid] : i) * 4;
        o4[0] = make_uint4(__float_as_uint(uvx), __float_as_uint(uvy), i, 0u);
        o4[1] = make_uint4(__float_as_uint(conx), __float_as_uint(cony), __float_as_uint(conz), __float_as_uint(pv[2]));
        o4[2] = make_uint4(__float_as_uint(col[0]), __float_as_uint(col[1]), __float_as_uint(col[2]), __float_as_uint(opacity));
        o4[3] = make_uint4(rminx, rminy, rmaxx, rmaxy);
    }
    PRE_STAMP(4);
#ifdef GS_PROFILING
    if (TIGHT && lane == 0) {
        unsigned long long* pp = gs_pre_prof[(bid * 4u + w) & 255u];
        for (int k = 0; k < 5; ++k) atomicAdd(&pp[k], (unsigned long long)pacc[k]);
        atomicAdd(&pp[5], 1ull);
    }
#endif
    if (TIGHT) {
        __syncthreads();
        const uint32_t c = s_rowhist[tid];
        if (c) atomicAdd(&to.ctl->rowhist[bid & 7u][tid], c);
    }
}

void gs_launch_repack(const void* d_aos, uint32_t n, uint32_t first, const GsScene& s, hipStream_t st) {
    const uint64_t total = (uint64_t)n * 20;
    const uint32_t blocks = (uint32_t)((total + 255) / 256);
    if (!blocks) return;
    hipLaunchKernelGGL(gs_repack_kernel, dim3(blocks), dim3(256), 0, st, (const float4*)d_aos, n, first, (float*)s.px, (float*)s.py,
                       (float*)s.pz, (float*)s.smax, (float*)s.geo, (float*)s.sh);
}
float gs_view_norm2(const GsUniforms& u) {
    double A[3][3];
    for (int i = 0; i < 3; ++i)
        for (int j = 0; j < 3; ++j) {
            A[i][j] = 0.0;
            for (int r = 0; r < 3; ++r) A[i][j] += (double)u.view[4 * i + r] * (double)u.view[4 * j + r];
        }
    const double q = (A[0][0] + A[1][1] + A[2][2]) / 3.0;
    const double d0 = A[0][0] - q, d1 = A[1][1] - q, d2 = A[2][2] - q;
    const double p2 = (d0 * d0 + d1 * d1 + d2 * d2 + 2.0 * (A[0][1] * A[0][1] + A[0][2] * A[0][2] + A[1][2] * A[1][2])) / 6.0;
    const double p = sqrt(p2);
    double lam = q;
    if (!(p <= 1e-14 * fabs(q))) {
        const double b01 = A[0][1] / p, b02 = A[0][2] / p, b12 = A[1][2] / p, b0 = d0 / p, b1 = d1 / p, b2 = d2 / p;
        double r = 0.5 * (b0 * (b1 * b2 - b12 * b12) - b01 * (b01 * b2 - b12 * b02) + b02 * (b01 * b12 - b1 * b02));
        r = r < -1.0 ? -1.0 : (r > 1.0 ? 1.0 : r);
        lam = q + 2.0 * p * cos(acos(r) / 3.0);
    }
    return (float)(lam * (1.0 + 1e-7));
}
void gs_preprocess_prepare(GsPreprocessLaunch& L, const GsScene& s, const GsUniforms& u, const GsFrame& f, void* gdata, uint32_t* counts,
                           bool tight, uint32_t* arena, uint32_t* rowptr, unsigned short* unit_off, uint32_t* unit_n, GsControl* ctl,
                           uint32_t tight_nb, bool state, GsTint tint) {
    const uint32_t wcols = f.col1 - f.col0;
    uint32_t nb = f.full || wcols * 4u > f.ntx * 3u ? 1u : (wcols * 10u > f.ntx * 3u ? 4u : 8u);
    if (tight) nb = tight_nb ? tight_nb : (nb == 1u ? 2u : nb);
    L.blocks = (f.n + PRE_G * nb - 1) / (PRE_G * nb);
    if (state) {
        if (tight) L.func = nb == 8u ? (const void*)&gs_preprocess_kernel<true, 8, true> : nb == 4u ? (const void*)&gs_preprocess_kernel<true, 4, true>
                                                                                                     : (const void*)&gs_preprocess_kernel<true, 2, true>;
        else L.func = nb == 8u ? (const void*)&gs_preprocess_kernel<false, 8, true> : nb == 4u ? (const void*)&gs_preprocess_kernel<false, 4, true>
                                                                                                  : (const void*)&gs_preprocess_kernel<false, 1, true>;
    } else {
        if (tight) L.func = nb == 8u ? (const void*)&gs_preprocess_kernel<true, 8, false> : nb == 4u ? (const void*)&gs_preprocess_kernel<true, 4, false>
                                                                                                      : (const void*)&gs_preprocess_kernel<true, 2, false>;
        else L.func = nb == 8u ? (const void*)&gs_preprocess_kernel<false, 8, false> : nb == 4u ? (const void*)&gs_preprocess_kernel<false, 4, false>
                                                                                                   : (const void*)&gs_preprocess_kernel<false, 1, false>;
    }
    L.s = s; L.u = u; L.f = f; L.gdata = gdata; L.counts = counts; L.tint = tint;
    L.w2 = f.full ? 1.0f : gs_view_norm2(u);
    L.to.arena = arena; L.to.rowptr = rowptr; L.to.unit_off = unit_off; L.to.unit_n = unit_n; L.to.ctl = ctl;
    L.to.rec_shard_cap = ((L.blocks + 15u) / 16u) * (PRE_G * nb);
    L.args[0] = &L.s; L.args[1] = &L.u; L.args[2] = &L.f; L.args[3] = &L.gdata; L.args[4] = &L.counts; L.args[5] = &L.to; L.args[6] = &L.tint; L.args[7] = &L.w2;
}
void gs_launch_preprocess(GsPreprocessLaunch& L, hipStream_t st) {
    if (!L.f.n) return;
    (void)hipLaunchKernel(L.func, dim3(L.blocks), dim3(256), L.args, 0, st);
}
```

### gaussian-splatting-wgpu_amd/csrc/k_rows.hip

```cpp
#include "gs_binning.h"
#include "gs_tight.h"

typedef uint32_t gs_item3 __attribute__((ext_vector_type(3), aligned(4)));

#ifndef RA_ITEMS
#define RA_ITEMS 8
#endif
#ifndef RA_WAVES
#define RA_WAVES 8
#endif
#define RA_THREADS (RA_WAVES * 64)
#define RA_TILE (RA_THREADS * RA_ITEMS)

#ifndef RB_CH
#define RB_CH 512u
#endif
#define RB_IT (RB_CH / 256u)
#ifndef RB_SB
#define RB_SB 2048u
#endif
#define RB_PER (RB_SB / 256u)
#define RB_WSL (RB_SB / 4u)

struct RowSortShared {
    uint32_t hist[RA_WAVES][256];
    uint32_t gbase[256];
    uint32_t tot[256];
    uint32_t dbase[256];
    uint32_t wsum[RA_WAVES];
    uint32_t tile, nvalid;
    union {
        uint32_t it[RA_TILE * 3];
        struct {
            uint32_t goff[RA_TILE + 8], gptr[RA_TILE + 8];
            unsigned short mark[RA_TILE];
        } g;
    } u;
};

__global__ __launch_bounds__(RA_THREADS) void gs_rows_sort_kernel(const uint32_t* __restrict__ arena, const uint4* __restrict__ grec,
                                                                  const uint32_t* __restrict__ chunk_table, uint32_t* __restrict__ rows_out,
                                                                  GsControl* ctl, uint32_t* __restrict__ status, uint32_t row_cap, uint32_t ndig) {
    __shared__ RowSortShared sh;
    const GsDigits dg = gs_digits(ndig);
    const uint32_t tid = threadIdx.x, lane = tid & 63, w = tid >> 6;
    const unsigned long long lt_mask = (1ull << lane) - 1ull;
    uint32_t n = ctl->num_slots;
    if (n > row_cap) n = row_cap;
    const uint32_t ntiles = (n + RA_TILE - 1) / RA_TILE;
    const uint32_t nvis = ctl->num_visible;
    {
        const uint32_t c = tid < 256u ? gs_rowhist(ctl, tid) : 0u;
        const uint32_t incl = wave_scan_publish(c, lane, w, sh.wsum);
        __syncthreads();
        const uint32_t b = waves_before<uint32_t>(sh.wsum, w);
        if (tid < 256u) sh.dbase[tid] = b + incl - c;
        __syncthreads();
    }
    for (;;) {
        if (tid == 0) sh.tile = atomicAdd(&ctl->rows_ticket, 1u);
        __syncthreads();
        const uint32_t tile = sh.tile;
        if (tile >= ntiles) break;
        const uint32_t s0 = tile * RA_TILE, s_end = (s0 + RA_TILE < n) ? s0 + RA_TILE : n;
        const uint32_t g0 = chunk_table[s0 >> 10];
        const uint32_t g1 = (s_end < n) ? chunk_table[s_end >> 10] : nvis - 1u;
        uint32_t K = (g1 >= g0) ? g1 - g0 + 1u : 1u;
        if (K > RA_TILE + 8u) K = RA_TILE + 8u;
        for (uint32_t k = tid; k < RA_TILE / 2u; k += RA_THREADS) reinterpret_cast<uint32_t*>(sh.u.g.mark)[k] = 0u;
        __syncthreads();
        for (uint32_t k = tid; k < K; k += RA_THREADS) {
            const uint4 rec = (g0 + k < nvis) ? grec[g0 + k] : make_uint4(0u, 0u, 0xFFFFFFFFu, 0u);
            sh.u.g.goff[k] = rec.z;
            sh.u.g.gptr[k] = rec.w;
            if (rec.z >= s0 && rec.z < s_end) sh.u.g.mark[rec.z - s0] = (unsigned short)(k + 1u);
        }
        __syncthreads();
        uint32_t carry;
        {
            constexpr uint32_t RA_STR = (RA_TILE + 8u + 63u) / 64u;
            static_assert(RA_STR * 64u >= RA_TILE + 8u && RA_STR <= 128u, "the two-level owner search covers the tile's gaussians");
            const uint32_t x0 = s0 + w * (64 * RA_ITEMS);
            const uint32_t m1 = lane * RA_STR;
            const uint32_t c1 = (uint32_t)__popcll(__ballot(m1 < K && sh.u.g.goff[m1 < K ? m1 : 0u] <= x0));
            const uint32_t b1 = (c1 ? c1 - 1u : 0u) * RA_STR;
            uint32_t c2 = 0;
#pragma unroll
            for (uint32_t t2 = 0; t2 < (RA_STR + 63u) / 64u; ++t2) {
                const uint32_t o2 = t2 * 64u + lane, m2 = b1 + o2;
                c2 += (uint32_t)__popcll(__ballot(o2 < RA_STR && m2 < K && sh.u.g.goff[m2 < K ? m2 : 0u] <= x0));
            }
            const uint32_t e = b1 + (c2 ? c2 - 1u : 0u);
            carry = e + 1u;
        }
        uint32_t ix[RA_ITEMS], iy[RA_ITEMS], iz[RA_ITEMS];
        uint32_t rank2[RA_ITEMS / 2];
#pragma unroll
        for (int j = 0; j < RA_ITEMS; ++j) {
            const uint32_t sp = w * (64 * RA_ITEMS) + j * 64 + lane, slot = s0 + sp;
            const uint32_t m = owner_walk((uint32_t)sh.u.g.mark[sp], carry);
            ix[j] = GS_ROW_HOLE; iy[j] = 0u; iz[j] = 0u;
            if (slot < n) {
                const uint32_t k = m - 1u;
                const uint32_t src = sh.u.g.gptr[k] + (slot - sh.u.g.goff[k]);
                if (src < row_cap) {
                    const gs_item3 v = *reinterpret_cast<const gs_item3*>(arena + (uint64_t)src * 3u);
                    ix[j] = v.x; iy[j] = v.y; iz[j] = v.z;
                }
            }
        }
        for (uint32_t k = lane; k < 256; k += 64) sh.hist[w][k] = 0;
        if (tid < 256u) sh.tot[tid] = 0u;
        __syncthreads();
#pragma unroll
        for (int j = 0; j < RA_ITEMS; ++j) atomicAdd(&sh.tot[ix[j] == GS_ROW_HOLE ? dg.hole : (iy[j] & 0xFFu)], 1u);
        __syncthreads();
        if (tid < ndig) st_agent(status + (uint64_t)tile * 256 + tid, (tile == 0 ? GS_LB_PREFIX : GS_LB_AGG) | sh.tot[tid]);
#pragma unroll
        for (int j = 0; j < RA_ITEMS; ++j) {
            const uint32_t d = ix[j] == GS_ROW_HOLE ? dg.hole : (iy[j] & 0xFFu);
            uint32_t plo = 0xFFFFFFFFu, phi = 0xFFFFFFFFu;
#pragma unroll
            for (int b = 0; b < 8; ++b) {
                if (b < dg.nbits) {
                    const uint32_t bit = (d >> b) & 1u;
                    const unsigned long long bal = __ballot(bit != 0u);
                    const uint32_t inv = bit - 1u;
                    plo &= (uint32_t)bal ^ inv;
                    phi &= (uint32_t)(bal >> 32) ^ inv;
                }
            }
            const uint32_t below = __popc(plo & (uint32_t)lt_mask) + __popc(phi & (uint32_t)(lt_mask >> 32));
            const uint32_t cnt = __popc(plo) + __popc(phi);
            const uint32_t pre = sh.hist[w][d];
            __builtin_amdgcn_fence(__ATOMIC_RELEASE, "wavefront");
            if (below == 0) sh.hist[w][d] = pre + cnt;
            __builtin_amdgcn_fence(__ATOMIC_ACQUIRE, "wavefront");
            const uint32_t r = pre + below;
            rank2_put(rank2, j, r);
        }
        __syncthreads();
        uint32_t cw[RA_WAVES], total = 0, excl = 0, incl = 0;
        if (tid < 256u) {
#pragma unroll
            for (int k = 0; k < RA_WAVES; ++k) { cw[k] = sh.hist[k][tid]; total += cw[k]; }
            incl = wave_scan_publish(total, lane, w, sh.wsum);
            if (tile > 0 && tid < ndig) {
                constexpr int LB = 8;
                bool found = false;
                for (int t = (int)tile - 1; t >= 0 && !found; t -= LB) {
                    uint32_t sv[LB];
#pragma unroll
                    for (int k = 0; k < LB; ++k) sv[k] = (t - k >= 0) ? ld_agent(status + (uint64_t)(t - k) * 256 + tid) : GS_LB_PREFIX;
#pragma unroll
                    for (int k = 0; k < LB; ++k) {
                        if (found) break;
                        uint32_t v = sv[k], spins = 0;
                        while ((v & GS_LB_FLAGS) == 0 && ++spins < GS_SPIN_LIMIT) {
                            __builtin_amdgcn_s_sleep(1);
                            v = ld_agent(status + (uint64_t)(t - k) * 256 + tid);
                        }
                        if ((v & GS_LB_FLAGS) == 0) { ctl->fault = 1u; found = true; break; }
                        excl += v & GS_LB_VALUE;
                        if ((v & GS_LB_FLAGS) == GS_LB_PREFIX) found = true;
                    }
                }
                st_agent(status + (uint64_t)tile * 256 + tid, GS_LB_PREFIX | ((excl + total) & GS_LB_VALUE));
            }
        }
        __syncthreads();
        if (tid < 256u) {
            uint32_t run = waves_before<uint32_t>(sh.wsum, w) + incl - total;
            if (tid == dg.hole) sh.nvalid = run;
            sh.gbase[tid] = sh.dbase[tid] + excl - run;
#pragma unroll
            for (int k = 0; k < RA_WAVES; ++k) { sh.hist[k][tid] = run; run += cw[k]; }
        }
        __syncthreads();
#pragma unroll
        for (int j = 0; j < RA_ITEMS; ++j) {
            const uint32_t d = ix[j] == GS_ROW_HOLE ? dg.hole : (iy[j] & 0xFFu);
            const uint32_t r = rank2_get(rank2, j);
            const uint32_t pos = sh.hist[w][d] + r;
            sh.u.it[pos * 3 + 0] = ix[j];
            sh.u.it[pos * 3 + 1] = iy[j];
            sh.u.it[pos * 3 + 2] = iz[j];
        }
        __syncthreads();
        const uint32_t nvalid = sh.nvalid;
#pragma unroll
        for (int j = 0; j < RA_ITEMS; ++j) {
            const uint32_t pos = j * RA_THREADS + tid;
            if (pos < nvalid) {
                gs_item3 v;
                v.x = sh.u.it[pos * 3 + 0]; v.y = sh.u.it[pos * 3 + 1]; v.z = sh.u.it[pos * 3 + 2];
                const uint32_t g = sh.gbase[v.y & 0xFFu] + pos;
                if (g < row_cap) *reinterpret_cast<gs_item3*>(rows_out + (uint64_t)g * 3u) = v;
            }
        }
        __syncthreads();
    }
}

struct RowTables {
    uint32_t ibase[257];
    uint32_t cbase[257];
    uint32_t w4[8];
};
__device__ __forceinline__ void row_tables(RowTables& T, const GsControl* ctl, uint32_t row_cap, uint32_t tid) {
    const uint32_t lane = tid & 63, w = tid >> 6;
    const bool on = tid < 256u;
    const uint32_t c = on ? gs_rowhist(ctl, tid) : 0u;
    const unsigned long long ic = wave_incl_scan64(c, lane);
    if (on && lane == 63) T.w4[w] = sat32(ic);
    __syncthreads();
    uint32_t i0 = 0, cc = 0;
    if (on) {
        const unsigned long long b = waves_before<unsigned long long>(T.w4, w, ic - c);
        const unsigned long long e = b + c;
        i0 = b > row_cap ? row_cap : (uint32_t)b;
        const uint32_t i1 = e > row_cap ? row_cap : (uint32_t)e;
        cc = i1 - i0;
        T.ibase[tid] = i0;
        if (tid == 255u) T.ibase[256] = i1;
    }
    const uint32_t ch = (cc + RB_CH - 1u) / RB_CH;
    const uint32_t ih = wave_incl_scan(ch, lane);
    if (on && lane == 63) T.w4[4 + w] = ih;
    __syncthreads();
    if (on) {
        const uint32_t bh = waves_before<uint32_t>(T.w4 + 4, w);
        T.cbase[tid] = bh + ih - ch;
        if (tid == 255u) T.cbase[256] = bh + ih;
    }
    __syncthreads();
}
__device__ __forceinline__ uint32_t row_of_chunk(const RowTables& T, uint32_t c) {
    const uint32_t lane = threadIdx.x & 63u;
    uint32_t v[4];
#pragma unroll
    for (int k = 0; k < 4; ++k) v[k] = T.cbase[lane + 64u * k];
    uint32_t r = 0;
#pragma unroll
    for (int k = 0; k < 4; ++k) r += (uint32_t)__popcll(__ballot(v[k] <= c && (lane + 64u * k) != 0u));
    return r;
}
__device__ __forceinline__ uint2 chunk_items(const RowTables& T, uint32_t r, uint32_t c) {
    const uint32_t i0 = T.ibase[r] + (c - T.cbase[r]) * RB_CH;
    return make_uint2(i0, (i0 + RB_CH < T.ibase[r + 1]) ? i0 + RB_CH : T.ibase[r + 1]);
}

__global__ __launch_bounds__(256) void gs_rows_count_kernel(const uint32_t* __restrict__ rows, const GsControl* ctl, uint32_t* __restrict__ M3,
                                                            uint32_t chunk_cap, uint32_t row_cap) {
    __shared__ RowTables T;
    __shared__ int s_diff[257];
    __shared__ uint32_t s_w[4];
    const uint32_t tid = threadIdx.x, lane = tid & 63, w = tid >> 6;
    row_tables(T, ctl, row_cap, tid);
    uint32_t nch = T.cbase[256];
    if (nch > chunk_cap) nch = chunk_cap;
    for (uint32_t c = blockIdx.x; c < nch; c += gridDim.x) {
        const uint2 ext = chunk_items(T, row_of_chunk(T, c), c);
        const uint32_t i0 = ext.x, i1 = ext.y;
        s_diff[tid] = 0;
        if (tid == 0) s_diff[256] = 0;
        __syncthreads();
#pragma unroll
        for (int k = 0; k < (int)(RB_CH / 256u); ++k) {
            const uint32_t i = i0 + k * 256u + tid;
            if (i < i1) {
                const uint32_t w1 = rows[(uint64_t)i * 3u + 1u];
                const uint32_t tlo = (w1 >> 8) & 0xFFu, len = ((w1 >> 16) & 0xFFu) + 1u;
                atomicAdd(&s_diff[tlo], 1);
                atomicAdd(&s_diff[tlo + len > 256u ? 256u : tlo + len], -1);
            }
        }
        __syncthreads();
        const uint32_t v = (uint32_t)s_diff[tid];
        const uint32_t incl = wave_incl_scan(v, lane);
        if (lane == 63) s_w[w] = incl;
        __syncthreads();
        M3[(uint64_t)c * 256u + tid] = waves_before<uint32_t>(s_w, w) + incl;
        __syncthreads();
    }
}

__global__ __launch_bounds__(1024) void gs_rows_scan_kernel(const GsControl* ctl, uint32_t* __restrict__ M3, uint32_t* __restrict__ tileoff,
                                                            uint32_t* __restrict__ rowtot, uint32_t chunk_cap, uint32_t row_cap) {
    __shared__ RowTables T;
    __shared__ unsigned long long s_part[4][256];
    __shared__ unsigned long long s_ex[256];
    __shared__ unsigned long long s_w[4];
    const uint32_t tid = threadIdx.x, c = tid & 255u, p = tid >> 8, r = blockIdx.x;
    row_tables(T, ctl, row_cap, tid);
    uint32_t c0 = T.cbase[r], c1 = T.cbase[r + 1];
    if (c0 > chunk_cap) c0 = chunk_cap;
    if (c1 > chunk_cap) c1 = chunk_cap;
    const uint32_t nch = c1 - c0, per = (nch + 3u) / 4u;
    const uint32_t j0 = c0 + (p * per < nch ? p * per : nch), j1 = c0 + ((p + 1u) * per < nch ? (p + 1u) * per : nch);
    unsigned long long sum = 0;
    for (uint32_t j = j0; j < j1; j += 8u) {
        uint32_t v[8];
#pragma unroll
        for (int k = 0; k < 8; ++k) v[k] = (j + k < j1) ? M3[(uint64_t)(j + k) * 256u + c] : 0u;
#pragma unroll
        for (int k = 0; k < 8; ++k) sum += v[k];
    }
    s_part[p][c] = sum;
    __syncthreads();
    unsigned long long run = 0, tot = 0;
#pragma unroll
    for (int k = 0; k < 4; ++k) { const unsigned long long t = s_part[k][c]; if (k < (int)p) run += t; tot += t; }
    for (uint32_t j = j0; j < j1; j += 8u) {
        uint32_t v[8];
#pragma unroll
        for (int k = 0; k < 8; ++k) v[k] = (j + k < j1) ? M3[(uint64_t)(j + k) * 256u + c] : 0u;
#pragma unroll
        for (int k = 0; k < 8; ++k) {
            if (j + k < j1) M3[(uint64_t)(j + k) * 256u + c] = sat32(run);
            run += v[k];
        }
    }
    if (p == 0) {
        const uint32_t lane = tid & 63, w = tid >> 6;
        const unsigned long long incl = wave_incl_scan64(tot, lane);
        if (lane == 63) s_w[w] = incl;
        s_ex[c] = incl - tot;
    }
    __syncthreads();
    if (p == 0) {
        const uint32_t w = tid >> 6;
        unsigned long long b = 0, all = 0;
#pragma unroll
        for (int k = 0; k < 4; ++k) { if (k < (int)w) b += s_w[k]; all += s_w[k]; }
        const unsigned long long ex = b + s_ex[c];
        tileoff[r * 256u + c] = sat32(ex);
        if (c == 0) rowtot[r] = sat32(all);
    }
}

struct ExpandShared {
    RowTables T;
    uint32_t rbase[257];
    uint32_t w0[RB_CH], w1[RB_CH], w2[RB_CH];
    uint32_t hist[4][256];
    uint32_t gbase[256];
    uint32_t wsum[8];
    uint32_t nvalid, total;
    unsigned char cols[RB_SB];
    union {
        struct { uint32_t P[RB_CH + 1]; unsigned short mark[RB_SB]; } e;
        uint32_t vals[RB_SB];
    } x;
};

__global__ __launch_bounds__(256) void gs_rows_expand_kernel(const uint32_t* __restrict__ rows, GsControl* ctl, const uint32_t* __restrict__ M3,
                                                             const uint32_t* __restrict__ tileoff, const uint32_t* __restrict__ rowtot, GsFrame f,
                                                             uint32_t* __restrict__ values, uint32_t* __restrict__ ranges, uint32_t chunk_cap,
                                                             uint32_t row_cap, uint32_t* sticky, GsReport* rep) {
    __shared__ ExpandShared S;
    const uint32_t tid = threadIdx.x, lane = tid & 63, w = tid >> 6;
    const unsigned long long lt_mask = (1ull << lane) - 1ull;
    const uint32_t ns = f.tile_size >= 16u ? 2u : 1u;
    const GsDigits dg = gs_digits(f.ntx);
    row_tables(S.T, ctl, row_cap, tid);
    {
        const uint32_t v = tid < f.nty ? rowtot[tid] : 0u;
        const unsigned long long incl = wave_incl_scan64(v, lane);
        __shared__ unsigned long long s_r[4];
        if (lane == 63) s_r[w] = incl;
        __syncthreads();
        const unsigned long long b = waves_before<unsigned long long>(s_r, w);
        S.rbase[tid] = sat32(b + incl - v);
        if (tid == 255u) S.rbase[256] = sat32(b + incl);
        __syncthreads();
    }
    if (blockIdx.x == 0 && tid == 0) {
        const uint32_t I = S.rbase[256];
        ctl->num_intersections = I;
        ctl->num_items = S.T.ibase[256];
        if (I > f.capacity) ctl->overflow = 1u;
        gs_frame_report(ctl, I, S.T.ibase[256], f.capacity, sticky, rep);
    }
    for (uint32_t r = blockIdx.x; r < f.nty; r += gridDim.x) {
        if (tid < f.ntx) {
            const uint32_t endoff = (tid + 1u < 256u) ? tileoff[r * 256u + tid + 1u] : rowtot[r];
            const unsigned long long e = (unsigned long long)S.rbase[r] + endoff;
            ranges[r * f.ntx + tid] = sat32(e);
        }
    }
    uint32_t nch = S.T.cbase[256];
    if (nch > chunk_cap) nch = chunk_cap;
    gs_item3 nit[RB_IT];
    uint32_t n_r = 0, n_ni = 0, n_tstart = 0, n_done = 0;
    auto prefetch = [&](uint32_t c) {
        n_r = row_of_chunk(S.T, c);
        const uint2 ext = chunk_items(S.T, n_r, c);
        const uint32_t i0 = ext.x;
        n_ni = ext.y - i0;
#pragma unroll
        for (int k = 0; k < (int)RB_IT; ++k) {
            const uint32_t e = tid * RB_IT + k;
            nit[k] = *reinterpret_cast<const gs_item3*>(rows + (uint64_t)(i0 + (e < n_ni ? e : 0u)) * 3u);
        }
        n_tstart = S.rbase[n_r] + tileoff[n_r * 256u + tid];
        n_done = M3[(uint64_t)c * 256u + tid];
    };
    if (blockIdx.x < nch) prefetch(blockIdx.x);
    for (uint32_t c = blockIdx.x; c < nch; c += gridDim.x) {
        const uint32_t ni = n_ni;
        uint32_t len[RB_IT], lsum = 0;
#pragma unroll
        for (int k = 0; k < (int)RB_IT; ++k) {
            const uint32_t e = tid * RB_IT + k;
            len[k] = 0u;
            if (e < ni) {
                S.w0[e] = nit[k].x; S.w1[e] = nit[k].y; S.w2[e] = nit[k].z;
                len[k] = ((nit[k].y >> 16) & 0xFFu) + 1u;
            }
            lsum += len[k];
        }
        const uint32_t tstart = n_tstart;
        uint32_t done = n_done;
        if (c + gridDim.x < nch) prefetch(c + gridDim.x);
        {
            const uint32_t incl = wave_incl_scan(lsum, lane);
            if (lane == 63) S.wsum[w] = incl;
            __syncthreads();
            uint32_t b = 0, all = 0;
#pragma unroll
            for (int k = 0; k < 4; ++k) { if (k < (int)w) b += S.wsum[k]; all += S.wsum[k]; }
            uint32_t run = b + incl - lsum;
#pragma unroll
            for (int k = 0; k < (int)RB_IT; ++k) { S.x.e.P[tid * RB_IT + k] = run; run += len[k]; }
            if (tid == 0) { S.x.e.P[RB_CH] = all; S.total = all; }
        }
        __syncthreads();
        const uint32_t ninst = S.total;
        for (uint32_t s0 = 0; s0 < ninst; s0 += RB_SB) {
            if (s0) {
                __syncthreads();
                uint32_t l2[RB_IT], ls = 0;
#pragma unroll
                for (int k = 0; k < (int)RB_IT; ++k) { const uint32_t e = tid * RB_IT + k; l2[k] = e < ni ? ((S.w1[e] >> 16) & 0xFFu) + 1u : 0u; ls += l2[k]; }
                const uint32_t incl = wave_incl_scan(ls, lane);
                if (lane == 63) S.wsum[w] = incl;
                __syncthreads();
                uint32_t b = 0;
#pragma unroll
                for (int k = 0; k < 4; ++k) if (k < (int)w) b += S.wsum[k];
                uint32_t run = b + incl - ls;
#pragma unroll
                for (int k = 0; k < (int)RB_IT; ++k) { S.x.e.P[tid * RB_IT + k] = run; run += l2[k]; }
                if (tid == 0) S.x.e.P[RB_CH] = ninst;
            }
            for (uint32_t k = tid; k < RB_SB / 2u; k += 256u) reinterpret_cast<uint32_t*>(S.x.e.mark)[k] = 0u;
            for (uint32_t k = lane; k < 256; k += 64) S.hist[w][k] = 0u;
            __syncthreads();
#pragma unroll
            for (int k = 0; k < (int)RB_IT; ++k) {
                const uint32_t e = tid * RB_IT + k;
                if (e < ni) {
                    const uint32_t p0 = S.x.e.P[e];
                    if (p0 >= s0 && p0 < s0 + RB_SB) S.x.e.mark[p0 - s0] = (unsigned short)(e + 1u);
                }
            }
            __syncthreads();
            uint32_t carry;
            {
                const uint32_t x0 = s0 + w * RB_WSL;
                uint32_t pv[RB_CH / 64u];
#pragma unroll
                for (int k = 0; k < (int)(RB_CH / 64u); ++k) pv[k] = S.x.e.P[lane + 64u * k];
                uint32_t e = 0;
#pragma unroll
                for (int k = 0; k < (int)(RB_CH / 64u); ++k) {
                    const uint32_t m = lane + 64u * k;
                    e += (uint32_t)__popcll(__ballot(m != 0u && m < ni && pv[k] <= x0));
                }
                carry = e + 1u;
            }
            uint32_t val[RB_PER], col4[RB_PER / 4u];
            uint32_t rank2[RB_PER / 2u];
#pragma unroll
            for (int j = 0; j < (int)(RB_PER / 4u); ++j) col4[j] = 0u;
            const uint32_t wfirst = s0 + w * RB_WSL;
            const uint32_t jn = wfirst >= ninst ? 0u : ((ninst - wfirst + 63u) / 64u < RB_PER ? (ninst - wfirst + 63u) / 64u : RB_PER);
#pragma unroll
            for (int j = 0; j < (int)RB_PER; ++j) {
                if ((uint32_t)j >= jn) break;
                const uint32_t sp = w * RB_WSL + j * 64u + lane, x = s0 + sp;
                const uint32_t m = owner_walk((uint32_t)S.x.e.mark[sp], carry);
                uint32_t d = dg.hole;
                val[j] = 0u;
                if (x < ninst) {
                    const uint32_t e = m - 1u;
                    const uint32_t q = x - S.x.e.P[e], i1w = S.w1[e];
                    d = ((i1w >> 8) & 0xFFu) + q;
                    val[j] = (S.w0[e] & GS_ID_MASK) | (tight_item_mask(S.w2[e], q, ns) << GS_ID_BITS);
                }
                col4[j >> 2] |= d << (8 * (j & 3));
            }
#pragma unroll
            for (int j = 0; j < (int)RB_PER; ++j) {
                if ((uint32_t)j >= jn) break;
                const uint32_t d = (col4[j >> 2] >> (8 * (j & 3))) & 0xFFu;
                uint32_t plo = 0xFFFFFFFFu, phi = 0xFFFFFFFFu;
#pragma unroll
                for (int b = 0; b < 8; ++b) {
                    if (b < dg.nbits) {
                        const uint32_t bit = (d >> b) & 1u;
                        const unsigned long long bal = __ballot(bit != 0u);
                        const uint32_t inv = bit - 1u;
                        plo &= (uint32_t)bal ^ inv;
                        phi &= (uint32_t)(bal >> 32) ^ inv;
                    }
                }
                const uint32_t below = __popc(plo & (uint32_t)lt_mask) + __popc(phi & (uint32_t)(lt_mask >> 32));
                const uint32_t cnt = __popc(plo) + __popc(phi);
                const uint32_t pre = S.hist[w][d];
                __builtin_amdgcn_fence(__ATOMIC_RELEASE, "wavefront");
                if (below == 0) S.hist[w][d] = pre + cnt;
                __builtin_amdgcn_fence(__ATOMIC_ACQUIRE, "wavefront");
                const uint32_t rr = pre + below;
                rank2_put(rank2, j, rr);
            }
            __syncthreads();
            {
                uint32_t cw[4], total = 0;
#pragma unroll
                for (int k = 0; k < 4; ++k) { cw[k] = S.hist[k][tid]; total += cw[k]; }
                const uint32_t incl = wave_incl_scan(total, lane);
                if (lane == 63) S.wsum[4 + w] = incl;
                __syncthreads();
                uint32_t b = 0;
#pragma unroll
                for (int k = 0; k < 4; ++k) if (k < (int)w) b += S.wsum[4 + k];
                uint32_t run = b + incl - total;
                if (tid == dg.hole) S.nvalid = run;
                S.gbase[tid] = tstart + done - run;
                done += total;
#pragma unroll
                for (int k = 0; k < 4; ++k) { S.hist[k][tid] = run; run += cw[k]; }
            }
            __syncthreads();
#pragma unroll
            for (int j = 0; j < (int)RB_PER; ++j) {
                if ((uint32_t)j >= jn) break;
                const uint32_t d = (col4[j >> 2] >> (8 * (j & 3))) & 0xFFu;
                const uint32_t rr = rank2_get(rank2, j);
                const uint32_t pos = S.hist[w][d] + rr;
                S.x.vals[pos] = val[j];
                S.cols[pos] = (unsigned char)d;
            }
            __syncthreads();
            const uint32_t nvalid = S.nvalid;
#pragma unroll
            for (int j = 0; j < (int)RB_PER; ++j) {
                const uint32_t pos = j * 256u + tid;
                if (pos < nvalid) {
                    const uint32_t dst = S.gbase[S.cols[pos]] + pos;
                    if (dst < f.capacity) values[dst] = S.x.vals[pos];
                }
            }
        }
        __syncthreads();
    }
}

__device__ __forceinline__ uint32_t rows_entry_id(const uint32_t* __restrict__ gdata, uint32_t nrec, uint32_t v, uint32_t n) {
    const uint32_t slot = v & GS_ID_MASK;
    if (slot >= nrec) return n;
    const uint32_t g = gdata[(uint64_t)slot * 16u + 2u];
    return g < n ? g : n;
}
__global__ __launch_bounds__(256) void gs_rows_rebuild_keys_kernel(const uint32_t* __restrict__ ranges, uint32_t T, const uint32_t* __restrict__ vals,
                                                                   const uint32_t* __restrict__ gdata, uint32_t nrec, uint32_t count, uint32_t n,
                                                                   uint32_t* __restrict__ keys) {
    for (uint32_t i = blockIdx.x * 256u + threadIdx.x; i < count; i += gridDim.x * 256u) {
        uint32_t lo = 0, hi = T;
        while (lo < hi) {
            const uint32_t mid = (lo + hi) >> 1;
            if (ranges[mid] > i) hi = mid; else lo = mid + 1u;
        }
        const uint32_t v = vals[i];
        const uint32_t g = rows_entry_id(gdata, nrec, v, n);
        const uint32_t bucket = g < n ? f2u_sat(wg_min(50.0f * __uint_as_float(gdata[(uint64_t)(v & GS_ID_MASK) * 16u + 7u]), 999.0f)) : 0u;
        keys[i] = lo * 1000u + bucket;
    }
}
__global__ __launch_bounds__(256) void gs_rows_rebuild_taps_kernel(const uint32_t* __restrict__ vals, const uint32_t* __restrict__ gdata, uint32_t nrec,
                                                                   uint32_t count, uint32_t n, uint32_t* __restrict__ ids_out,
                                                                   uint4* __restrict__ gdata_out) {
    for (uint32_t i = blockIdx.x * 256u + threadIdx.x; i < count; i += gridDim.x * 256u) {
        const uint32_t v = vals[i];
        const uint32_t g = rows_entry_id(gdata, nrec, v, n);
        if (ids_out) ids_out[i] = (g < n ? g : GS_ID_MASK) | (v & ~GS_ID_MASK);
        if (gdata_out && g < n) {
            const uint4* src = reinterpret_cast<const uint4*>(gdata) + (uint64_t)(v & GS_ID_MASK) * 4u;
            uint4 p0 = src[0];
            p0.z = 0u;
            uint4* dst = gdata_out + (uint64_t)g * 4u;
            dst[0] = p0; dst[1] = src[1]; dst[2] = src[2]; dst[3] = src[3];
        }
    }
}

#ifndef RB_CNT_WG
#define RB_CNT_WG 8u
#endif
#ifndef RB_EXP_WG
#define RB_EXP_WG 6u
#endif
uint32_t gs_rows_sort_tiles(uint64_t row_cap) { return (uint32_t)((row_cap + RA_TILE - 1) / RA_TILE); }
uint32_t gs_rows_chunks(uint64_t row_cap) { return (uint32_t)(row_cap / RB_CH + 256u); }
void gs_launch_rows(const uint32_t* arena, const void* grec, const uint32_t* chunk_table, uint32_t* rows_sorted, GsControl* ctl, uint32_t* sort_status, uint32_t row_cap,
                    uint32_t* M3, uint32_t* tileoff, uint32_t* rowtot, const GsFrame& f, uint32_t* values, uint32_t* ranges, uint32_t cus,
                    uint32_t* sticky, GsReport* rep, hipStream_t st, void (*mark)(void*, int), void* mark_arg) {
    const uint32_t chunk_cap = gs_rows_chunks(row_cap);
    if (!cus) cus = 1;
    hipLaunchKernelGGL(gs_rows_sort_kernel, dim3(cus * 3u), dim3(RA_THREADS), 0, st, arena, (const uint4*)grec, chunk_table, rows_sorted, ctl, sort_status,
                       row_cap, f.nty);
    if (mark) mark(mark_arg, 3);
    hipLaunchKernelGGL(gs_rows_count_kernel, dim3(cus * RB_CNT_WG), dim3(256), 0, st, (const uint32_t*)rows_sorted, (const GsControl*)ctl, M3, chunk_cap, row_cap);
    hipLaunchKernelGGL(gs_rows_scan_kernel, dim3(f.nty), dim3(1024), 0, st, (const GsControl*)ctl, M3, tileoff, rowtot, chunk_cap, row_cap);
    hipLaunchKernelGGL(gs_rows_expand_kernel, dim3(cus * RB_EXP_WG), dim3(256), 0, st, (const uint32_t*)rows_sorted, ctl, (const uint32_t*)M3,
                       (const uint32_t*)tileoff, (const uint32_t*)rowtot, f, values, ranges, chunk_cap, row_cap, sticky, rep);
}
void gs_launch_rows_rebuild_keys(const uint32_t* ranges, uint32_t T, const uint32_t* vals, const void* gdata, uint32_t nrec, uint32_t count, uint32_t n,
                                 uint32_t* keys, hipStream_t st) {
    if (!count) return;
    const uint32_t blocks = (count + 255u) / 256u;
    hipLaunchKernelGGL(gs_rows_rebuild_keys_kernel, dim3(blocks < 4096u ? blocks : 4096u), dim3(256), 0, st, ranges, T, vals, (const uint32_t*)gdata, nrec,
                       count, n, keys);
}
void gs_launch_rows_rebuild_taps(const uint32_t* vals, const void* gdata, uint32_t nrec, uint32_t count, uint32_t n, uint32_t* ids_out, void* gdata_out,
                                 hipStream_t st) {
    if (!count) return;
    const uint32_t blocks = (count + 255u) / 256u;
    hipLaunchKernelGGL(gs_rows_rebuild_taps_kernel, dim3(blocks < 4096u ? blocks : 4096u), dim3(256), 0, st, vals, (const uint32_t*)gdata, nrec, count, n,
                       ids_out, (uint4*)gdata_out);
}
```

Measured before the change: 1444 frames/s.

## Shrink arena row items to 8 bytes by moving record slot into gsort record

Row items in the arena previously stored three words (record slot, w1, w2). The record slot is now split across the tile-count word's spare bits and a 16-bit side array, carried through the gaussian sort into grec.x. The rows sort kernel reconstructs it per gaussian from shared memory. This cuts arena write and read traffic by a third, at the cost of extra shared memory in the rows kernel (67 KB vs 59 KB) and tighter bit packing in the count word.

```diff
diff --git a/gaussian-splatting-wgpu_amd/csrc/gs_context.hip b/gaussian-splatting-wgpu_amd/csrc/gs_context.hip
--- a/gaussian-splatting-wgpu_amd/csrc/gs_context.hip
+++ b/gaussian-splatting-wgpu_amd/csrc/gs_context.hip
@@ -46,7 +46,7 @@
     c->sort_tile = GsSort{{c->keysA, c->valsA}, {c->keysB, c->valsB}, c->tile_passes, c->tile_bits, c->tile16 ? 0u : 1u, c->tile16, true};
     HIP_TRY(hipMalloc(c->chunk_table.out(), (size_t)gs_emit_chunks(std::max(capacity, row_cap)) * 4));
     if (c->tight_ok) {
-        HIP_TRY(hipMalloc(c->arena.out(), (size_t)row_cap * 12));
+        HIP_TRY(hipMalloc(c->arena.out(), (size_t)row_cap * 8));
         HIP_TRY(hipMalloc(c->rows_sorted.out(), (size_t)row_cap * 12));
         HIP_TRY(hipMalloc(c->M3.out(), (size_t)gs_rows_chunks(row_cap) * 256 * 4));
     }
@@ -168,14 +168,14 @@
     c->ng = gs_ctx::Neigh{};
     c->cl = gs_ctx::Cluster{};
     c->counts.reset(); c->offsets.reset(); c->grec.reset(); c->rowptr.reset(); c->gsort_scratch.reset(); c->gdata.reset(); c->gdataG.reset();
-    c->unit_off.reset(); c->unit_n.reset();
+    c->rec_lo.reset(); c->unit_n.reset();
     const size_t np = ((size_t)n + 63) & ~(size_t)63;
     const size_t ne = (size_t)gs_gsort_tiles((uint32_t)(n ? n : 1)) * 2048, nu = ne / 1024 + 2;
     HIP_TRY(hipMalloc(c->counts.out(), ne * 4));
     HIP_TRY(hipMalloc(c->offsets.out(), std::max<size_t>(np * 4, 256)));
     HIP_TRY(hipMalloc(c->grec.out(), std::max<size_t>(np * 16, 256)));
     HIP_TRY(hipMalloc(c->rowptr.out(), ne * 4));
-    HIP_TRY(hipMalloc(c->unit_off.out(), ne * 2));
+    HIP_TRY(hipMalloc(c->rec_lo.out(), ne * 2));
     HIP_TRY(hipMalloc(c->unit_n.out(), nu * 4));
     HIP_TRY(hipMemsetAsync(c->unit_n, 0, nu * 4, c->stream));
     HIP_TRY(hipMalloc(c->gsort_scratch.out(), gs_gsort_scratch_bytes((uint32_t)n)));
diff --git a/gaussian-splatting-wgpu_amd/csrc/gs_device.h b/gaussian-splatting-wgpu_amd/csrc/gs_device.h
--- a/gaussian-splatting-wgpu_amd/csrc/gs_device.h
+++ b/gaussian-splatting-wgpu_amd/csrc/gs_device.h
@@ -17,6 +17,8 @@
 
 #define GS_COUNT_BITS 22
 #define GS_COUNT_MASK 0x3FFFFFu
+#define GS_TSLOT_BITS 10
+#define GS_TSLOT_MASK 0x3FFu
 
 struct GsControl {
     uint32_t scan_ticket[2];
@@ -71,7 +73,7 @@
 
 struct GsTightOut {
     uint32_t* arena; uint32_t* rowptr; GsControl* ctl;
-    unsigned short* unit_off; uint32_t* unit_n;
+    unsigned short* rec_lo; uint32_t* unit_n;
     uint32_t rec_shard_cap;
 };
 #define GS_RECORD_SLACK (16u * 512u * 8u)
diff --git a/gaussian-splatting-wgpu_amd/csrc/gs_frame.hip b/gaussian-splatting-wgpu_amd/csrc/gs_frame.hip
--- a/gaussian-splatting-wgpu_amd/csrc/gs_frame.hip
+++ b/gaussian-splatting-wgpu_amd/csrc/gs_frame.hip
@@ -40,14 +40,14 @@
 }
 
 static void prepare_projection(gs_ctx* c, const GsUniforms& u, bool tight) {
-    gs_preprocess_prepare(c->pre, c->scene, u, c->frame, c->gdata, c->counts, tight, c->arena, c->rowptr, c->unit_off, c->unit_n, c->ctl, c->opt.tight_nb,
+    gs_preprocess_prepare(c->pre, c->scene, u, c->frame, c->gdata, c->counts, tight, c->arena, c->rowptr, c->rec_lo, c->unit_n, c->ctl, c->opt.tight_nb,
                           has_state(c), tint_of(c->opt.select_tint));
 }
 
 
 static FrameNotes bin_tight(gs_ctx* c) {
     hipStream_t st = c->stream;
-    gs_launch_gsort(c->counts, c->rowptr, c->unit_off, c->unit_n, c->n, c->gsort_scratch, c->grec, c->chunk_table,
+    gs_launch_gsort(c->counts, c->rowptr, c->rec_lo, c->unit_n, c->n, c->gsort_scratch, c->grec, c->chunk_table,
                     (uint32_t)gs_emit_chunks(std::max(c->capacity, c->row_cap)), &c->ctl->num_visible, &c->ctl->num_slots, c->opt.grid_persist, st);
     mark(c, 2);
     gs_launch_rows(c->arena, c->grec, c->chunk_table, c->rows_sorted, c->ctl, c->rows_status, (uint32_t)c->row_cap, c->M3, c->tileoff, c->rowtot, c->frame,
diff --git a/gaussian-splatting-wgpu_amd/csrc/gs_kernels.h b/gaussian-splatting-wgpu_amd/csrc/gs_kernels.h
--- a/gaussian-splatting-wgpu_amd/csrc/gs_kernels.h
+++ b/gaussian-splatting-wgpu_amd/csrc/gs_kernels.h
@@ -13,7 +13,7 @@
 };
 float gs_view_norm2(const GsUniforms& u);
 void gs_preprocess_prepare(GsPreprocessLaunch& L, const GsScene& s, const GsUniforms& u, const GsFrame& f, void* gdata, uint32_t* counts,
-                           bool tight, uint32_t* arena, uint32_t* rowptr, unsigned short* unit_off, uint32_t* unit_n, GsControl* ctl,
+                           bool tight, uint32_t* arena, uint32_t* rowptr, unsigned short* rec_lo, uint32_t* unit_n, GsControl* ctl,
                            uint32_t tight_nb = 0, bool state = false, GsTint tint = GsTint{});
 void gs_launch_preprocess(GsPreprocessLaunch& L, hipStream_t st);
 void gs_launch_zero(void* p, uint64_t bytes, hipStream_t st);
@@ -54,7 +54,7 @@
                         uint64_t slab_stride_px, hipStream_t st);
 uint32_t gs_gsort_tiles(uint32_t n);
 uint64_t gs_gsort_scratch_bytes(uint32_t n);
-void gs_launch_gsort(const uint32_t* words, const uint32_t* aux_in, const unsigned short* unit_off, const uint32_t* unit_n, uint32_t n, void* scratch,
+void gs_launch_gsort(const uint32_t* words, const uint32_t* aux_in, const unsigned short* rec_lo, const uint32_t* unit_n, uint32_t n, void* scratch,
                      void* grec, uint32_t* chunk_table, uint32_t chunk_cap, uint32_t* tot_visible, uint32_t* tot_quantity, uint32_t grid, hipStream_t st);
 uint32_t gs_rows_sort_tiles(uint64_t row_cap);
 uint32_t gs_rows_chunks(uint64_t row_cap);
diff --git a/gaussian-splatting-wgpu_amd/csrc/gs_runtime.h b/gaussian-splatting-wgpu_amd/csrc/gs_runtime.h
--- a/gaussian-splatting-wgpu_amd/csrc/gs_runtime.h
+++ b/gaussian-splatting-wgpu_amd/csrc/gs_runtime.h
@@ -114,7 +114,7 @@
     uint32_t n = 0;
     uint64_t scene_serial = 0;
     DevBuf<uint32_t> counts, offsets, rowptr;
-    DevBuf<unsigned short> unit_off;
+    DevBuf<unsigned short> rec_lo;
     DevBuf<uint32_t> unit_n;
     DevBuf<> gdata;
     DevBuf<> grec;
diff --git a/gaussian-splatting-wgpu_amd/csrc/k_gsort.hip b/gaussian-splatting-wgpu_amd/csrc/k_gsort.hip
--- a/gaussian-splatting-wgpu_amd/csrc/k_gsort.hip
+++ b/gaussian-splatting-wgpu_amd/csrc/k_gsort.hip
@@ -14,11 +14,13 @@
     const uint2 v = unit_n[c];
     return make_uint2(v.x < GU ? v.x : GU, v.y < GU ? v.y : GU);
 }
+__host__ __device__ constexpr uint32_t gsort_qmask(bool dense) { return dense ? GS_TSLOT_MASK : GS_COUNT_MASK; }
 template <bool DENSE>
 __global__ __launch_bounds__(GC_THREADS) void gs_gsort_hist_kernel(const uint32_t* __restrict__ words, const uint2* __restrict__ unit_n, uint32_t n,
                                                                    uint2* __restrict__ M, uint32_t ncol, uint32_t cpr, uint32_t NT) {
     __shared__ uint32_t s_cnt[GBINS];
     __shared__ unsigned long long s_sum[GBINS];
+    constexpr uint32_t QMASK = gsort_qmask(DENSE);
     const uint32_t run = blockIdx.x, tid = threadIdx.x;
     const uint32_t c0 = run * cpr, c1 = c0 + cpr < NT ? c0 + cpr : NT;
     for (uint32_t b = tid; b < GBINS; b += GC_THREADS) { s_cnt[b] = 0u; s_sum[b] = 0ull; }
@@ -51,10 +53,10 @@
 #pragma unroll
         for (int j = 0; j < GC_ITEMS; ++j) {
             const uint32_t w = wv[j];
-            if (w & GS_COUNT_MASK) {
+            if (w & QMASK) {
                 const uint32_t b = w >> GS_COUNT_BITS;
                 atomicAdd(&s_cnt[b], 1u);
-                atomicAdd(&s_sum[b], (unsigned long long)(w & GS_COUNT_MASK));
+                atomicAdd(&s_sum[b], (unsigned long long)(w & QMASK));
             }
         }
 #pragma unroll
@@ -138,12 +140,13 @@
 
 template <bool DENSE>
 __global__ __launch_bounds__(GC_THREADS) void gs_gsort_scatter_kernel(const uint32_t* __restrict__ words, const uint32_t* __restrict__ aux_in,
-                                                                      const unsigned short* __restrict__ unit_off, const uint2* __restrict__ unit_n, uint32_t n,
+                                                                      const unsigned short* __restrict__ rec_lo, const uint2* __restrict__ unit_n, uint32_t n,
                                                                       const uint2* __restrict__ M, uint32_t ncol, uint32_t cpr, uint32_t NT,
                                                                       const uint2* __restrict__ rowtot, uint4* __restrict__ grec,
                                                                       uint32_t* __restrict__ chunk_table, uint32_t chunk_cap,
                                                                       uint32_t* __restrict__ tot_visible, uint32_t* __restrict__ tot_quantity) {
     __shared__ GsortShared S;
+    constexpr uint32_t QMASK = gsort_qmask(DENSE);
     const uint32_t run_id = blockIdx.x;
     const uint32_t chunk0 = run_id * cpr, chunk1 = chunk0 + cpr < NT ? chunk0 + cpr : NT;
     const uint32_t tid = threadIdx.x, lane = tid & 63, w = tid >> 6;
@@ -169,7 +172,7 @@
                     const uint32_t e = c * GC + (p >= un.x ? GU + (p - un.x) : p);
                     nwv[j] = words[e];
                     nav[j] = aux_in[e];
-                    nid[j] = (uint32_t)unit_off[e];
+                    nid[j] = (uint32_t)rec_lo[e];
                 }
             }
             unx = un;
@@ -224,7 +227,7 @@
             for (int j = 0; j < GC_ITEMS; ++j) {
                 const uint32_t p = p0 + j * 64;
                 if (!((uint32_t)j < R && p < T)) wv[j] = 0u;
-                idv[j] = (p >= unx.x ? GU : 0u) + nid[j];
+                idv[j] = nid[j];
             }
         }
         if (chunk + 1u < chunk1) load_chunk(chunk + 1u);
@@ -236,7 +239,7 @@
         uint32_t rank2[GC_ITEMS / 2];
 #pragma unroll
         for (int j = 0; j < GC_ITEMS; ++j) {
-            if (!(wv[j] & GS_COUNT_MASK)) wv[j] = 0u;
+            if (!(wv[j] & QMASK)) wv[j] = 0u;
             const unsigned long long vis = __ballot(wv[j] != 0u);
             uint32_t r = 0;
             if (vis) {
@@ -290,7 +293,7 @@
 #pragma unroll
             for (int j = 0; j < GC_ITEMS; ++j) {
                 const uint32_t p = tid * GC_ITEMS + j;
-                c[j] = (p < nc) ? (S.word[p] & GS_COUNT_MASK) : 0u;
+                c[j] = (p < nc) ? (S.word[p] & QMASK) : 0u;
                 acc += c[j];
             }
             unsigned long long total;
@@ -310,8 +313,10 @@
             const uint32_t g = base.x + (pos - first);
             const unsigned long long off64 = (unsigned long long)base.y + (S.u.P[pos] - S.u.P[first]);
             const uint32_t off = sat32(off64);
-            grec[g] = make_uint4(chunk * GC + (uint32_t)S.id[pos], x, off, S.aux[pos]);
-            const uint32_t cnt = x & GS_COUNT_MASK;
+            const uint32_t x0 = DENSE ? (uint32_t)S.id[pos] | (((x >> GS_TSLOT_BITS) & ((1u << (GS_COUNT_BITS - GS_TSLOT_BITS)) - 1u)) << 16)
+                                      : chunk * GC + (uint32_t)S.id[pos];
+            grec[g] = make_uint4(x0, x, off, S.aux[pos]);
+            const uint32_t cnt = x & QMASK;
             if (off != 0xFFFFFFFFu) {
                 const unsigned long long lastq = (off64 + cnt - 1ull) >> GS_EMIT_CHUNK_SHIFT;
                 const uint32_t last = lastq > 0xFFFFFFFFull ? 0xFFFFFFFFu : (uint32_t)lastq;
@@ -344,7 +349,7 @@
 
 uint32_t gs_gsort_tiles(uint32_t n) { return (n + GC - 1) / GC; }
 uint64_t gs_gsort_scratch_bytes(uint32_t n) { return ((uint64_t)GBINS * gs_gsort_tiles(n ? n : 1) + GBINS) * sizeof(uint2); }
-void gs_launch_gsort(const uint32_t* words, const uint32_t* aux_in, const unsigned short* unit_off, const uint32_t* unit_n, uint32_t n, void* scratch,
+void gs_launch_gsort(const uint32_t* words, const uint32_t* aux_in, const unsigned short* rec_lo, const uint32_t* unit_n, uint32_t n, void* scratch,
                      void* grec, uint32_t* chunk_table, uint32_t chunk_cap, uint32_t* tot_visible, uint32_t* tot_quantity, uint32_t grid, hipStream_t st) {
     if (!n) return;
     const uint32_t NT = gs_gsort_tiles(n);
@@ -358,8 +363,8 @@
     if (un) hipLaunchKernelGGL(gs_gsort_hist_kernel<true>, dim3(G), dim3(GC_THREADS), 0, st, words, un, n, M, G, cpr, NT);
     else hipLaunchKernelGGL(gs_gsort_hist_kernel<false>, dim3(G), dim3(GC_THREADS), 0, st, words, un, n, M, G, cpr, NT);
     hipLaunchKernelGGL(gs_gsort_rowscan_kernel, dim3(GBINS / 8), dim3(GR_THREADS), 0, st, M, G, rowtot);
-    if (un) hipLaunchKernelGGL(gs_gsort_scatter_kernel<true>, dim3(G), dim3(GC_THREADS), 0, st, words, aux_in, unit_off, un, n, (const uint2*)M, G, cpr, NT,
+    if (un) hipLaunchKernelGGL(gs_gsort_scatter_kernel<true>, dim3(G), dim3(GC_THREADS), 0, st, words, aux_in, rec_lo, un, n, (const uint2*)M, G, cpr, NT,
                                (const uint2*)rowtot, (uint4*)grec, chunk_table, chunk_cap, tot_visible, tot_quantity);
-    else hipLaunchKernelGGL(gs_gsort_scatter_kernel<false>, dim3(G), dim3(GC_THREADS), 0, st, words, aux_in, unit_off, un, n, (const uint2*)M, G, cpr, NT,
+    else hipLaunchKernelGGL(gs_gsort_scatter_kernel<false>, dim3(G), dim3(GC_THREADS), 0, st, words, aux_in, rec_lo, un, n, (const uint2*)M, G, cpr, NT,
                             (const uint2*)rowtot, (uint4*)grec, chunk_table, chunk_cap, tot_visible, tot_quantity);
 }
diff --git a/gaussian-splatting-wgpu_amd/csrc/k_preprocess.hip b/gaussian-splatting-wgpu_amd/csrc/k_preprocess.hip
--- a/gaussian-splatting-wgpu_amd/csrc/k_preprocess.hip
+++ b/gaussian-splatting-wgpu_amd/csrc/k_preprocess.hip
@@ -167,11 +167,12 @@
 #else
 #define PRE_STAMP(k) do { } while (0)
 #endif
+static_assert(2 * GS_ROW_MAX_DIM < 1024 && (1u << GS_TSLOT_BITS) == 1024, "a gaussian's slots (its rows, twice that with the aliased column) fit the slot field");
+static_assert(GS_ID_BITS == 28 && GS_TSLOT_BITS + (GS_ID_BITS - 16) == GS_COUNT_BITS, "the record slot's high half fills the word between the slots and the bucket");
 #define PRE_G 512
 #ifndef PRE_WAVES
 #define PRE_WAVES 4
 #endif
-typedef uint32_t gs_row_u32x3 __attribute__((ext_vector_type(3), aligned(4)));
 
 
 template <bool TIGHT, int NB, bool STATE>
@@ -484,11 +485,7 @@
                         atomicAdd(&s_tcnt[j], ilen);
                         atomicAdd(&s_rowhist[w1 & 0xFFu], 1u);
                     }
-                    if (ok) {
-                        gs_row_u32x3 it;
-                        it.x = ilen ? s_tgid[j] : GS_ROW_HOLE; it.y = w1; it.z = w2;
-                        *reinterpret_cast<gs_row_u32x3*>(to.arena + (uint64_t)(abase + ri) * 3u) = it;
-                    }
+                    if (ok) reinterpret_cast<uint2*>(to.arena)[abase + ri] = make_uint2(ilen ? w1 : GS_ROW_HOLE, w2);
                 }
             }
             __builtin_amdgcn_fence(__ATOMIC_RELEASE, "wavefront");
@@ -499,13 +496,14 @@
             if (!active) continue;
         }
         const uint32_t bucket = f2u_sat(wg_min(50.0f * pv[2], 999.0f));
-        const uint32_t word = count ? ((TIGHT ? nslots : count) | (bucket << GS_COUNT_BITS)) : 0u;
+        const uint32_t rslot = TIGHT && count ? s_tgid[tid] : 0u;
+        const uint32_t word = count ? ((TIGHT ? nslots | ((rslot >> 16) << GS_TSLOT_BITS) : count) | (bucket << GS_COUNT_BITS)) : 0u;
         if (TIGHT) {
             const uint32_t off = STATE ? (sid & 0xFFFFu) : sid, uk = off >> 10;
             const uint32_t e = ((bid * (NB / 2) + uk) << 10) + (v - (NB == 2 ? 0u : s_ust[uk]));
             tile_counts[e] = word;
             to.rowptr[e] = rowptr;
-            to.unit_off[e] = (unsigned short)(off & 1023u);
+            to.rec_lo[e] = (unsigned short)(rslot & 0xFFFFu);
         } else tile_counts[i] = word;
         if (count == 0) continue;
 
@@ -565,7 +563,7 @@
     return (float)(lam * (1.0 + 1e-7));
 }
 void gs_preprocess_prepare(GsPreprocessLaunch& L, const GsScene& s, const GsUniforms& u, const GsFrame& f, void* gdata, uint32_t* counts,
-                           bool tight, uint32_t* arena, uint32_t* rowptr, unsigned short* unit_off, uint32_t* unit_n, GsControl* ctl,
+                           bool tight, uint32_t* arena, uint32_t* rowptr, unsigned short* rec_lo, uint32_t* unit_n, GsControl* ctl,
                            uint32_t tight_nb, bool state, GsTint tint) {
     const uint32_t wcols = f.col1 - f.col0;
     uint32_t nb = f.full || wcols * 4u > f.ntx * 3u ? 1u : (wcols * 10u > f.ntx * 3u ? 4u : 8u);
@@ -584,7 +582,7 @@
     }
     L.s = s; L.u = u; L.f = f; L.gdata = gdata; L.counts = counts; L.tint = tint;
     L.w2 = f.full ? 1.0f : gs_view_norm2(u);
-    L.to.arena = arena; L.to.rowptr = rowptr; L.to.unit_off = unit_off; L.to.unit_n = unit_n; L.to.ctl = ctl;
+    L.to.arena = arena; L.to.rowptr = rowptr; L.to.rec_lo = rec_lo; L.to.unit_n = unit_n; L.to.ctl = ctl;
     L.to.rec_shard_cap = ((L.blocks + 15u) / 16u) * (PRE_G * nb);
     L.args[0] = &L.s; L.args[1] = &L.u; L.args[2] = &L.f; L.args[3] = &L.gdata; L.args[4] = &L.counts; L.args[5] = &L.to; L.args[6] = &L.tint; L.args[7] = &L.w2;
 }
diff --git a/gaussian-splatting-wgpu_amd/csrc/k_rows.hip b/gaussian-splatting-wgpu_amd/csrc/k_rows.hip
--- a/gaussian-splatting-wgpu_amd/csrc/k_rows.hip
+++ b/gaussian-splatting-wgpu_amd/csrc/k_rows.hip
@@ -32,11 +32,12 @@
     union {
         uint32_t it[RA_TILE * 3];
         struct {
-            uint32_t goff[RA_TILE + 8], gptr[RA_TILE + 8];
+            uint32_t goff[RA_TILE + 8], gptr[RA_TILE + 8], grs[RA_TILE + 8];
             unsigned short mark[RA_TILE];
         } g;
     } u;
 };
+static_assert(sizeof(RowSortShared) <= 80 * 1024, "two workgroups per CU (67 KB; 59 KB while the arena's items carried the record slot themselves)");
 
 __global__ __launch_bounds__(RA_THREADS) void gs_rows_sort_kernel(const uint32_t* __restrict__ arena, const uint4* __restrict__ grec,
                                                                   const uint32_t* __restrict__ chunk_table, uint32_t* __restrict__ rows_out,
@@ -73,6 +74,7 @@
             const uint4 rec = (g0 + k < nvis) ? grec[g0 + k] : make_uint4(0u, 0u, 0xFFFFFFFFu, 0u);
             sh.u.g.goff[k] = rec.z;
             sh.u.g.gptr[k] = rec.w;
+            sh.u.g.grs[k] = rec.x;
             if (rec.z >= s0 && rec.z < s_end) sh.u.g.mark[rec.z - s0] = (unsigned short)(k + 1u);
         }
         __syncthreads();
@@ -103,9 +105,10 @@
             if (slot < n) {
                 const uint32_t k = m - 1u;
                 const uint32_t src = sh.u.g.gptr[k] + (slot - sh.u.g.goff[k]);
+                const uint32_t rs = sh.u.g.grs[k];
                 if (src < row_cap) {
-                    const gs_item3 v = *reinterpret_cast<const gs_item3*>(arena + (uint64_t)src * 3u);
-                    ix[j] = v.x; iy[j] = v.y; iz[j] = v.z;
+                    const uint2 v = reinterpret_cast<const uint2*>(arena)[src];
+                    ix[j] = v.x == GS_ROW_HOLE ? GS_ROW_HOLE : rs; iy[j] = v.x; iz[j] = v.y;
                 }
             }
         }
```

Result: no change. 1455 frames/s (median of 6 runs) (+0.8%).
